# Genie-Kim/PintheMemory

Measured on AMD Instinct MI355X. Metric: train imgs/sec 768x768 bs=8 R50-DeepLabV3+ +mem, higher is better.
Workload: dtype f32

## Files before the change

include/pinmem_hip.h:

```cpp
#ifndef PINMEM_HIP_H
#define PINMEM_HIP_H
#include <stddef.h>
#include <stdint.h>

#ifdef __cplusplus
extern "C" {
#endif

typedef enum pm_status { PM_OK = 0, PM_EINVAL = -1, PM_EWORKSPACE = -2, PM_ELAUNCH = -3, PM_EUNSUPPORTED = -4 } pm_status;

typedef enum pm_dtype { PM_F32 = 0, PM_BF16 = 1 } pm_dtype;
#define PM_TF_ZERO_PAD64 1

typedef struct pm_tensor {
  void* ptr;
  int32_t n, h, w, c;
  int64_t pitch;
  int32_t dtype;
  int32_t flags;
} pm_tensor;

#define PM_ABI_VERSION 400

typedef struct pm_conv_params {
  int32_t struct_size;
  int32_t kh, kw, stride, pad, dil;
  int32_t prec;
  void* wino_v;
  int64_t wino_v_bytes;
  void* wxf;
  int64_t wxf_bytes;
  int32_t wxf_valid;
} pm_conv_params;

typedef struct pm_conv_epilogue {
  int64_t struct_size;
  const float* bias;
  const float* scale;
  const float* shift;
  const float* residual;
  int64_t residual_pitch;
  int32_t relu;
  float* bn_partials;
  int64_t bn_partials_bytes;
} pm_conv_epilogue;

const char* pm_last_error(void);
int pm_version(void);

size_t pm_conv_workspace(const pm_tensor* x, const pm_tensor* y, const pm_conv_params* p, int which );
size_t pm_conv_winograd_v_bytes(const pm_tensor* x, const pm_tensor* y, const pm_conv_params* p);
size_t pm_conv_wxf_bytes(const pm_tensor* x, const pm_tensor* y, const pm_conv_params* p);
size_t pm_conv_wxf_bytes_dgrad(const pm_tensor* dy, const pm_tensor* dx, const pm_conv_params* p);
typedef struct pm_wxf_job {
  const float* w;
  void* wxf;
  int64_t wxf_bytes;
  int32_t cout, kh, kw, cin;
  int32_t dgrad;
  int32_t reserved;
} pm_wxf_job;
int pm_conv_wxf_refresh_bf16(const pm_wxf_job* jobs, int n, void* stream);
int pm_conv_wxf_refresh_f32(const pm_wxf_job* jobs, int n, void* stream);
size_t pm_conv_bn_partials_bytes(const pm_tensor* x, const pm_tensor* y, const pm_conv_params* p);
int pm_conv_fwd(const pm_tensor* x, const float* w_krsc, const pm_tensor* y, const pm_conv_params* p,
                const pm_conv_epilogue* ep, void* ws, size_t ws_bytes, void* stream);
int pm_conv_bwd_data(const pm_tensor* dy, const float* w_krsc, const pm_tensor* dx, const pm_conv_params* p,
                     const pm_tensor* add, void* ws, size_t ws_bytes, void* stream);
int pm_conv_bwd_data_masked(const pm_tensor* dy, const float* w_krsc, const pm_tensor* dx, const pm_conv_params* p,
                            const pm_tensor* add, const uint8_t* add_mask, void* ws, size_t ws_bytes, void* stream);
int pm_conv_bwd_weight(const pm_tensor* x, const pm_tensor* dy, float* dw_krsc, float* dbias, const pm_conv_params* p,
                       void* ws, size_t ws_bytes, void* stream);

typedef struct pm_routing {
  int32_t struct_size;
  int32_t winograd;
  int32_t winograd_fused;
  int32_t conv16;
  int32_t conv16_wide;
  int32_t conv16_persistent;
  int32_t wgrad16;
  int32_t bf16_wgrad;
  int32_t split;
} pm_routing;
int pm_routing_get(pm_routing* out);
int pm_routing_set(const pm_routing* r);


int pm_set_winograd(int mode);
int pm_set_winograd_fused(int on);
int pm_set_conv16(int on);
int pm_set_bf16_wgrad(int on);
int pm_set_wgrad16(int on);
int pm_set_split(int on);

int pm_profile_enable(int on);
int pm_profile_dump(const char* csv_path);
int pm_profile_read(int mode, int bm, int bn, int km, int nst, double* total_ms, double* total_flops, int64_t* launches, int clear);
int pm_profile_read_prec(int mode, int bm, int bn, int km, int nst, int prec, double* total_ms, double* total_flops, int64_t* launches, int clear);
int pm_profile_read_bytes(int mode, int bm, int bn, int km, int nst, int prec, double* total_bytes);

size_t pm_bn_workspace(const pm_tensor* x);
int pm_bn_stats(const pm_tensor* x, float* moments, void* ws, size_t ws_bytes, void* stream);
int pm_bn_stats_finalize(const pm_tensor* x, float eps, float* mean, float* invstd, float* running_mean , float* running_var ,
                         float momentum, void* ws, size_t ws_bytes, void* stream);
int pm_bn_merge(const float* parts, int world, int c, float* moments, void* stream);
int pm_bn_merge_finalize(const float* parts, int world, int c, float eps, float* mean, float* invstd, float* running_mean ,
                         float* running_var , float momentum, void* stream);
int pm_bn_finalize(const float* moments, int c, float eps, float* mean, float* invstd,
                   float* running_mean, float* running_var, float momentum, void* stream);
int pm_bn_apply(const pm_tensor* x, const float* mean, const float* invstd, const float* gamma, const float* beta,
                const pm_tensor* residual , int relu, const pm_tensor* y, void* stream);
int pm_bn_apply_mask(const pm_tensor* x, const float* mean, const float* invstd, const float* gamma, const float* beta,
                     const pm_tensor* residual , int relu, const pm_tensor* y, uint8_t* mask , void* stream);
int pm_bn_bwd_reduce_mask(const pm_tensor* dy, const uint8_t* mask, const pm_tensor* x, const float* mean, const float* invstd,
                          const pm_tensor* gmask , float* sums, void* ws, size_t ws_bytes, void* stream);
int pm_bn_apply_mask_affine(const pm_tensor* x, const float* mean, const float* invstd, const float* gamma, const float* beta,
                            const pm_tensor* r, const float* r_mean, const float* r_invstd, const float* r_gamma, const float* r_beta,
                            int relu, const pm_tensor* y, uint8_t* mask , void* stream);
int pm_bn_bwd_apply_mask(const pm_tensor* dy, const uint8_t* mask, const pm_tensor* x, const float* mean, const float* invstd, const float* gamma,
                         const float* sums, float count, const pm_tensor* dx, void* stream);
int pm_bn_bwd_reduce(const pm_tensor* dy, const pm_tensor* y , const pm_tensor* x, const float* mean, const float* invstd,
                     const float* gamma , const float* beta , int relu, const pm_tensor* gmask ,
                     float* sums, void* ws, size_t ws_bytes, void* stream);
int pm_bn_bwd_apply(const pm_tensor* dy, const pm_tensor* y , const pm_tensor* x, const float* mean, const float* invstd,
                    const float* gamma, const float* beta , const float* sums, float count, int relu, const pm_tensor* dx,
                    const pm_tensor* dres , void* stream);
int pm_bn_partials_finalize(const float* partials, int64_t pixels, int c, float eps, float* mean, float* invstd, float* running_mean ,
                            float* running_var , float momentum, float* moments , void* stream);
int pm_bn_fold(const float* gamma, const float* beta, const float* running_mean, const float* running_var, const float* conv_bias,
               int c, float eps, float* scale, float* shift, void* stream);
int pm_bn_fold_multi(const void* table, const int* cs, const int* offs, int n, int max_c, int total, float eps, float* arena, void* stream);
int pm_relu_bwd(const pm_tensor* dy, const pm_tensor* y, const pm_tensor* dx, void* stream);
int pm_add(const pm_tensor* a, const pm_tensor* b, const pm_tensor* y, void* stream);
int pm_add_n(const pm_tensor* const* xs, int n, const pm_tensor* y, void* stream);
int pm_copy(const pm_tensor* src, const pm_tensor* dst, void* stream);
int pm_scale_shift_act(const pm_tensor* x, const float* scale, const float* shift, const pm_tensor* residual, int relu,
                       const pm_tensor* y, void* stream);

int pm_cast(const pm_tensor* x, const pm_tensor* y, void* stream);

int pm_maxpool3x3s2_fwd(const pm_tensor* x, const pm_tensor* y, uint8_t* argmax, void* stream);
int pm_maxpool3x3s2_bwd(const pm_tensor* dy, const uint8_t* argmax, const pm_tensor* dx, void* stream);
int pm_maxpool3x3s2_bn_relu_fwd(const pm_tensor* x, const float* mean, const float* invstd, const float* gamma, const float* beta, const pm_tensor* y,
                                uint8_t* argmax, void* stream);
int pm_bn_bwd_reduce_pool(const pm_tensor* dy_pooled, const uint8_t* argmax, const pm_tensor* x, const float* mean, const float* invstd, const float* gamma,
                          const float* beta, float* sums, void* ws, size_t ws_bytes, void* stream);
int pm_bn_bwd_apply_pool(const pm_tensor* dy_pooled, const uint8_t* argmax, const pm_tensor* x, const float* mean, const float* invstd, const float* gamma,
                         const float* beta, const float* sums, float count, const pm_tensor* dx, void* stream);
int pm_global_avgpool_fwd(const pm_tensor* x, const pm_tensor* y , void* stream);
int pm_global_avgpool_bwd(const pm_tensor* dy, const pm_tensor* dx, int accumulate, void* stream);

int pm_resize_bilinear_fwd(const pm_tensor* x, const pm_tensor* y, void* stream);
int pm_resize_bilinear_bwd(const pm_tensor* dy, const pm_tensor* dx, int accumulate, void* stream);
size_t pm_resize_bilinear_bwd_workspace(const pm_tensor* dy, const pm_tensor* dx);
// ... 79 lines not shown
```

pinthememory_amd/csrc/bn.hip:

```cpp
#include "pm_common.h"

namespace {

constexpr int CB = 64;
constexpr int RL = 16;

__device__ __forceinline__ float bn_affine(float v, float mu, float is, float ga, float be) { return pm_bn_affine(v, mu, is, ga, be); }

inline int chunk_rows(long P, int C) {
  const long colblocks = std::max<long>(1, (C + CB - 1) / CB);
  const long want = std::max<long>(512, 2048 / colblocks);
  long r = (P + want - 1) / want;
  r = std::max<long>(r, 64);
  return (int)((r + RL - 1) / RL * RL);
}

__global__ __launch_bounds__(256) void bn_stats_partial(const float* __restrict__ x, long pitch, long P, int C, int rows, float* __restrict__ part) {
  __shared__ float sm[RL][CB][2];
  const int g = threadIdx.x & 15, r = threadIdx.x >> 4;
  const int c = blockIdx.y * CB + g * 4;
  const long p0 = (long)blockIdx.x * rows, p1 = min(P, p0 + rows);
  float s1[4] = {0, 0, 0, 0}, s2[4] = {0, 0, 0, 0};
  if (c < C) {
    const float4 k = PM_LD4(x + c);
// ... 411 lines not shown
  if (int e = check_bn(dy, "bn_bwd_reduce")) return e;
  if (int e = check_bn(x, "bn_bwd_reduce")) return e;
  PM_REQUIRE(pm_same_shape(dy, x) && mean && invstd && sums, PM_EINVAL, "bn_bwd_reduce: bad args");
  PM_REQUIRE(relu >= 0 && relu <= 2, PM_EINVAL, "bn_bwd_reduce: relu mode %d (0 none, 1 mask from y, 2 mask rebuilt from x)", relu);
  PM_REQUIRE(relu != 1 || (y && pm_vec4(y) && pm_same_shape(y, x)), PM_EINVAL, "bn_bwd_reduce: relu mode 1 needs the forward output");
  PM_REQUIRE(relu != 2 || (gamma && beta), PM_EINVAL, "bn_bwd_reduce: relu mode 2 needs gamma and beta");
  PM_REQUIRE(!gmask || (relu != 0 && pm_vec4(gmask) && pm_same_shape(gmask, x)), PM_EINVAL, "bn_bwd_reduce: gmask needs a ReLU mode and the shape of x");
  PM_REQUIRE(ws && ws_bytes >= pm_bn_workspace(x), PM_EWORKSPACE, "bn_bwd_reduce: workspace too small");
  const long P = pm_pixels(x);
  const int rows = chunk_rows(P, x->c), nb = pm_cdiv(P, rows);
  hipStream_t st = (hipStream_t)stream;
  dim3 grid(nb, pm_cdiv(x->c, CB));
  const float *pdy = (const float*)dy->ptr, *py = relu == 1 ? (const float*)y->ptr : nullptr, *px = (const float*)x->ptr;
  const long yp = relu == 1 ? y->pitch : 0;
  float* pg = gmask ? (float*)gmask->ptr : nullptr;
  const long gp = gmask ? gmask->pitch : 0;
#define PM_BN_BWD_PARTIAL(R, G)                                                                                                                         \
  hipLaunchKernelGGL((bn_bwd_partial<R, G>), grid, dim3(256), 0, st, pdy, (long)dy->pitch, py, yp, px, (long)x->pitch, mean, invstd, gamma, beta, pg, gp, P, \
                     x->c, rows, (float*)ws)
  if (relu == 0) PM_BN_BWD_PARTIAL(0, false);
  else if (relu == 1 && gmask) PM_BN_BWD_PARTIAL(1, true);
  else if (relu == 1) PM_BN_BWD_PARTIAL(1, false);
  else if (gmask) PM_BN_BWD_PARTIAL(2, true);
  else PM_BN_BWD_PARTIAL(2, false);
#undef PM_BN_BWD_PARTIAL
  hipLaunchKernelGGL(bn_bwd_final, dim3(pm_cdiv(x->c, FC)), dim3(256), 0, st, (const float*)ws, nb, x->c, sums);
  return pm_check_launch("bn_bwd_reduce");
}

extern "C" int pm_bn_bwd_reduce_mask(const pm_tensor* dy, const uint8_t* mask, const pm_tensor* x, const float* mean, const float* invstd,
                                     const pm_tensor* gmask, float* sums, void* ws, size_t ws_bytes, void* stream) {
  PM_REQUIRE(dy && x && mask, PM_EINVAL, "bn_bwd_reduce_mask: null");
  if (pm_is_bf16(x)) return pm16_bn_bwd_reduce(dy, nullptr, mask, x, mean, invstd, nullptr, nullptr, 3, gmask, sums, ws, ws_bytes, (hipStream_t)stream);
  if (int e = check_bn(dy, "bn_bwd_reduce_mask")) return e;
  if (int e = check_bn(x, "bn_bwd_reduce_mask")) return e;
  PM_REQUIRE(pm_same_shape(dy, x) && mean && invstd && sums && mask, PM_EINVAL, "bn_bwd_reduce_mask: bad args");
  PM_REQUIRE(!gmask || (pm_vec4(gmask) && pm_same_shape(gmask, x)), PM_EINVAL, "bn_bwd_reduce_mask: gmask must have the shape of x");
  PM_REQUIRE(ws && ws_bytes >= pm_bn_workspace(x), PM_EWORKSPACE, "bn_bwd_reduce_mask: workspace too small");
  const long P = pm_pixels(x);
  const int rows = chunk_rows(P, x->c), nb = pm_cdiv(P, rows);
  hipStream_t st = (hipStream_t)stream;
  dim3 grid(nb, pm_cdiv(x->c, CB));
  float* pg = gmask ? (float*)gmask->ptr : nullptr;
  const long gp = gmask ? gmask->pitch : 0;
  if (gmask)
    hipLaunchKernelGGL((bn_bwd_partial<3, true>), grid, dim3(256), 0, st, (const float*)dy->ptr, (long)dy->pitch, reinterpret_cast<const float*>(mask), 0l,
                       (const float*)x->ptr, (long)x->pitch, mean, invstd, (const float*)nullptr, (const float*)nullptr, pg, gp, P, x->c, rows, (float*)ws);
  else
    hipLaunchKernelGGL((bn_bwd_partial<3, false>), grid, dim3(256), 0, st, (const float*)dy->ptr, (long)dy->pitch, reinterpret_cast<const float*>(mask), 0l,
                       (const float*)x->ptr, (long)x->pitch, mean, invstd, (const float*)nullptr, (const float*)nullptr, pg, gp, P, x->c, rows, (float*)ws);
  hipLaunchKernelGGL(bn_bwd_final, dim3(pm_cdiv(x->c, FC)), dim3(256), 0, st, (const float*)ws, nb, x->c, sums);
  return pm_check_launch("bn_bwd_reduce_mask");
}

extern "C" int pm_bn_bwd_apply(const pm_tensor* dy, const pm_tensor* y, const pm_tensor* x, const float* mean, const float* invstd, const float* gamma,
                               const float* beta, const float* sums, float count, int relu, const pm_tensor* dx, const pm_tensor* dres, void* stream) {
  PM_REQUIRE(dy && x && dx, PM_EINVAL, "bn_bwd_apply: null");
  if (pm_is_bf16(x)) return pm16_bn_bwd_apply(dy, y, x, mean, invstd, gamma, beta, sums, count, relu, dx, dres, (hipStream_t)stream);
  if (int e = check_bn(dy, "bn_bwd_apply")) return e;
  if (int e = check_bn(x, "bn_bwd_apply")) return e;
  if (int e = check_bn(dx, "bn_bwd_apply")) return e;
  PM_REQUIRE(pm_same_shape(dy, x) && pm_same_shape(dx, x) && mean && invstd && gamma && sums, PM_EINVAL, "bn_bwd_apply: bad args");
  PM_REQUIRE(relu >= 0 && relu <= 2, PM_EINVAL, "bn_bwd_apply: relu mode %d (0 none, 1 mask from y, 2 mask rebuilt from x)", relu);
  PM_REQUIRE(relu != 1 || (y && pm_vec4(y) && pm_same_shape(y, x)), PM_EINVAL, "bn_bwd_apply: relu mode 1 needs the forward output");
  PM_REQUIRE(relu != 2 || beta, PM_EINVAL, "bn_bwd_apply: relu mode 2 needs beta");
  PM_REQUIRE(!dres || (pm_vec4(dres) && pm_same_shape(dres, x)), PM_EINVAL, "bn_bwd_apply: dres shape mismatch");
  const float *pd = (const float*)dy->ptr, *po = relu == 1 ? (const float*)y->ptr : nullptr, *px = (const float*)x->ptr;
  float *pdx = (float*)dx->ptr, *pdr = dres ? (float*)dres->ptr : nullptr;
  const long a = dy->pitch, b = relu == 1 ? y->pitch : 0, c = x->pitch, d = dx->pitch, e2 = dres ? dres->pitch : 0;
  const bool from_x = relu == 2;
  const int C = x->c;
  const bool dev_count = !(count > 0.f);
  const float host_inv_n = dev_count ? 0.f : 1.f / count;
  return pm_ew_launch(true, pm_pixels(x), C, (hipStream_t)stream, "bn_bwd_apply", [=] __device__(long p, int ch) {
    const float inv_n = dev_count ? 1.f / sums[2 * C] : host_inv_n;
    float4 g = PM_LD4(pd + p * a + ch);
    if (po) {
      const float4 o = PM_LD4(po + p * b + ch);
      g.x = o.x > 0.f ? g.x : 0.f, g.y = o.y > 0.f ? g.y : 0.f, g.z = o.z > 0.f ? g.z : 0.f, g.w = o.w > 0.f ? g.w : 0.f;
    }
    const float4 v = PM_LD4(px + p * c + ch), mu = PM_LD4(mean + ch), is = PM_LD4(invstd + ch), ga = PM_LD4(gamma + ch);
    if (from_x) {
      const float4 be = PM_LD4(beta + ch);
      g.x = bn_affine(v.x, mu.x, is.x, ga.x, be.x) > 0.f ? g.x : 0.f, g.y = bn_affine(v.y, mu.y, is.y, ga.y, be.y) > 0.f ? g.y : 0.f;
      g.z = bn_affine(v.z, mu.z, is.z, ga.z, be.z) > 0.f ? g.z : 0.f, g.w = bn_affine(v.w, mu.w, is.w, ga.w, be.w) > 0.f ? g.w : 0.f;
    }
    if (pdr) PM_ST4(pdr + p * e2 + ch, g);
    const float4 s1 = PM_LD4(sums + ch), s2 = PM_LD4(sums + C + ch);
    float4 r;
    r.x = (g.x - s1.x * inv_n - (v.x - mu.x) * is.x * (s2.x * inv_n)) * (is.x * ga.x);
    r.y = (g.y - s1.y * inv_n - (v.y - mu.y) * is.y * (s2.y * inv_n)) * (is.y * ga.y);
    r.z = (g.z - s1.z * inv_n - (v.z - mu.z) * is.z * (s2.z * inv_n)) * (is.z * ga.z);
    r.w = (g.w - s1.w * inv_n - (v.w - mu.w) * is.w * (s2.w * inv_n)) * (is.w * ga.w);
    PM_ST4(pdx + p * d + ch, r);
  });
}

extern "C" int pm_bn_bwd_apply_mask(const pm_tensor* dy, const uint8_t* mask, const pm_tensor* x, const float* mean, const float* invstd, const float* gamma,
                                    const float* sums, float count, const pm_tensor* dx, void* stream) {
  PM_REQUIRE(dy && x && dx && mask, PM_EINVAL, "bn_bwd_apply_mask: null");
  if (int e = check_bn(dy, "bn_bwd_apply_mask")) return e;
  if (int e = check_bn(x, "bn_bwd_apply_mask")) return e;
  if (int e = check_bn(dx, "bn_bwd_apply_mask")) return e;
  PM_REQUIRE(pm_same_shape(dy, x) && pm_same_shape(dx, x) && mean && invstd && gamma && sums, PM_EINVAL, "bn_bwd_apply_mask: bad args");
  const float *pd = (const float*)dy->ptr, *px = (const float*)x->ptr;
  float* pdx = (float*)dx->ptr;
  const long a = dy->pitch, c = x->pitch, d = dx->pitch;
  const int C = x->c, cq = C >> 2;
  const bool dev_count = !(count > 0.f);
  const float host_inv_n = dev_count ? 0.f : 1.f / count;
  return pm_ew_launch(true, pm_pixels(x), C, (hipStream_t)stream, "bn_bwd_apply_mask", [=] __device__(long p, int ch) {
    const float inv_n = dev_count ? 1.f / sums[2 * C] : host_inv_n;
    float4 g = PM_LD4(pd + p * a + ch);
    const unsigned mb = mask[p * cq + (ch >> 2)];
    g.x = (mb & 1u) ? g.x : 0.f, g.y = (mb & 2u) ? g.y : 0.f, g.z = (mb & 4u) ? g.z : 0.f, g.w = (mb & 8u) ? g.w : 0.f;
    const float4 v = PM_LD4(px + p * c + ch), mu = PM_LD4(mean + ch), is = PM_LD4(invstd + ch), ga = PM_LD4(gamma + ch);
    const float4 s1 = PM_LD4(sums + ch), s2 = PM_LD4(sums + C + ch);
    float4 r;
    r.x = (g.x - s1.x * inv_n - (v.x - mu.x) * is.x * (s2.x * inv_n)) * (is.x * ga.x);
    r.y = (g.y - s1.y * inv_n - (v.y - mu.y) * is.y * (s2.y * inv_n)) * (is.y * ga.y);
    r.z = (g.z - s1.z * inv_n - (v.z - mu.z) * is.z * (s2.z * inv_n)) * (is.z * ga.z);
    r.w = (g.w - s1.w * inv_n - (v.w - mu.w) * is.w * (s2.w * inv_n)) * (is.w * ga.w);
    PM_ST4(pdx + p * d + ch, r);
  });
}

namespace {
int check_pool_bn(const pm_tensor* dyp, const uint8_t* argmax, const pm_tensor* x, const char* who) {
  PM_REQUIRE(dyp && argmax && x, PM_EINVAL, "%s: null", who);
  if (int e = check_bn(dyp, who)) return e;
  if (int e = check_bn(x, who)) return e;
  PM_REQUIRE(dyp->n == x->n && dyp->c == x->c && dyp->h == (x->h + 2 - 3) / 2 + 1 && dyp->w == (x->w + 2 - 3) / 2 + 1, PM_EINVAL,
             "%s: dy is the gradient of the 3x3 / s2 / p1 max pool of a tensor shaped like x", who);
  return PM_OK;
}
}

extern "C" int pm_bn_bwd_reduce_pool(const pm_tensor* dyp, const uint8_t* argmax, const pm_tensor* x, const float* mean, const float* invstd, const float* gamma,
                                     const float* beta, float* sums, void* ws, size_t ws_bytes, void* stream) {
  if (int e = check_pool_bn(dyp, argmax, x, "bn_bwd_reduce_pool")) return e;
  PM_REQUIRE(mean && invstd && gamma && beta && sums, PM_EINVAL, "bn_bwd_reduce_pool: bad args");
  PM_REQUIRE(ws && ws_bytes >= pm_bn_workspace(x), PM_EWORKSPACE, "bn_bwd_reduce_pool: workspace too small");
  const long P = pm_pixels(x);
  const int rows = chunk_rows(P, x->c), nb = pm_cdiv(P, rows);
  hipStream_t st = (hipStream_t)stream;
  hipLaunchKernelGGL(bn_bwd_partial_pool, dim3(nb, pm_cdiv(x->c, CB)), dim3(256), 0, st, (const float*)dyp->ptr, (long)dyp->pitch, dyp->h, dyp->w, argmax, x->h, x->w,
                     (const float*)x->ptr, (long)x->pitch, mean, invstd, gamma, beta, P, x->c, rows, (float*)ws);
  hipLaunchKernelGGL(bn_bwd_final, dim3(pm_cdiv(x->c, FC)), dim3(256), 0, st, (const float*)ws, nb, x->c, sums);
  return pm_check_launch("bn_bwd_reduce_pool");
}

extern "C" int pm_bn_bwd_apply_pool(const pm_tensor* dyp, const uint8_t* argmax, const pm_tensor* x, const float* mean, const float* invstd, const float* gamma,
                                    const float* beta, const float* sums, float count, const pm_tensor* dx, void* stream) {
  if (int e = check_pool_bn(dyp, argmax, x, "bn_bwd_apply_pool")) return e;
  PM_REQUIRE(dx, PM_EINVAL, "bn_bwd_apply_pool: null");
  if (int e = check_bn(dx, "bn_bwd_apply_pool")) return e;
  PM_REQUIRE(pm_same_shape(dx, x) && mean && invstd && gamma && beta && sums, PM_EINVAL, "bn_bwd_apply_pool: bad args");
  const float *pd = (const float*)dyp->ptr, *px = (const float*)x->ptr;
  float* pdx = (float*)dx->ptr;
  const long a = dyp->pitch, c = x->pitch, d = dx->pitch;
  const int C = x->c, H = x->h, W = x->w, Ho = dyp->h, Wo = dyp->w;
  const bool dev_count = !(count > 0.f);
  const float host_inv_n = dev_count ? 0.f : 1.f / count;
  return pm_ew_launch(true, pm_pixels(x), C, (hipStream_t)stream, "bn_bwd_apply_pool", [=] __device__(long p, int ch) {
    const float inv_n = dev_count ? 1.f / sums[2 * C] : host_inv_n;
    float4 g = pm_maxpool_gather4(pd, a, Ho, Wo, argmax, H, W, C, p, ch);
    const float4 v = PM_LD4(px + p * c + ch), mu = PM_LD4(mean + ch), is = PM_LD4(invstd + ch), ga = PM_LD4(gamma + ch), be = PM_LD4(beta + ch);
    g.x = bn_affine(v.x, mu.x, is.x, ga.x, be.x) > 0.f ? g.x : 0.f, g.y = bn_affine(v.y, mu.y, is.y, ga.y, be.y) > 0.f ? g.y : 0.f;
    g.z = bn_affine(v.z, mu.z, is.z, ga.z, be.z) > 0.f ? g.z : 0.f, g.w = bn_affine(v.w, mu.w, is.w, ga.w, be.w) > 0.f ? g.w : 0.f;
    const float4 s1 = PM_LD4(sums + ch), s2 = PM_LD4(sums + C + ch);
    float4 r;
    r.x = (g.x - s1.x * inv_n - (v.x - mu.x) * is.x * (s2.x * inv_n)) * (is.x * ga.x);
    r.y = (g.y - s1.y * inv_n - (v.y - mu.y) * is.y * (s2.y * inv_n)) * (is.y * ga.y);
    r.z = (g.z - s1.z * inv_n - (v.z - mu.z) * is.z * (s2.z * inv_n)) * (is.z * ga.z);
    r.w = (g.w - s1.w * inv_n - (v.w - mu.w) * is.w * (s2.w * inv_n)) * (is.w * ga.w);
    PM_ST4(pdx + p * d + ch, r);
  });
}
```

pinthememory_amd/csrc/conv_igemm.hip:

```cpp
#include <stdlib.h>
#include <algorithm>
#include <type_traits>
#include <vector>

#include "pm_common.h"

#include "conv_igemm_kernel.h"

namespace {

template <int ZL, bool O16 = false>
__global__ __launch_bounds__(256) void splitk_reduce_vec_kernel(const float* __restrict__ ws, int ksplit, long slab, int M, int Nn,
                                                                float* __restrict__ C, long c_pitch, const float* bias,
                                                                const float* scale, const float* shift, const float* residual,
                                                                long res_pitch, int relu, const unsigned char* res_mask) {
  constexpr int GP = 256 / ZL;
  __shared__ float4 red[ZL > 1 ? ZL : 1][GP];
  const int gl = threadIdx.x % GP, zl = threadIdx.x / GP;
  const long groups = (long)M * Nn / 4;
  for (long g0 = (long)blockIdx.x * GP; g0 < groups; g0 += (long)gridDim.x * GP) {
    const long grp = g0 + gl;
    float4 v = make_float4(0.f, 0.f, 0.f, 0.f);
    if (grp < groups)
#pragma unroll 8
// ... 394 lines not shown
  prof.done();
  return pm_check_launch("conv_igemm");
}

int check_common(const pm_tensor* x, const pm_tensor* y, const pm_conv_params* p) {
  PM_REQUIRE(x && y && p && x->ptr && y->ptr, PM_EINVAL, "conv: null tensor");
  PM_REQUIRE(p->struct_size == (int32_t)sizeof(pm_conv_params), PM_EINVAL, "conv: pm_conv_params.struct_size %d != %zu -- caller built against another pinmem_hip.h (library ABI %d)",
             p->struct_size, sizeof(pm_conv_params), PM_ABI_VERSION);
  PM_REQUIRE(p->kh >= 1 && p->kw >= 1 && p->dil >= 1 && p->pad >= 0, PM_EINVAL, "conv: bad geometry");
  PM_REQUIRE(p->stride == 1 || p->stride == 2, PM_EUNSUPPORTED, "conv: stride %d unsupported (1 or 2)", p->stride);
  const int ho = (x->h + 2 * p->pad - p->dil * (p->kh - 1) - 1) / p->stride + 1;
  const int wo = (x->w + 2 * p->pad - p->dil * (p->kw - 1) - 1) / p->stride + 1;
  PM_REQUIRE(ho == y->h && wo == y->w && x->n == y->n, PM_EINVAL, "conv: output %dx%d does not match geometry (%dx%d)", y->h, y->w, ho, wo);
  PM_REQUIRE((x->dtype == PM_F32 || x->dtype == PM_BF16) && (y->dtype == PM_F32 || y->dtype == PM_BF16), PM_EUNSUPPORTED, "conv: dtype %d / %d", x->dtype, y->dtype);
  for (const pm_tensor* t : {x, y}) {
    if (pm_is_bf16(t)) PM_REQUIRE(pm_vec8(t), PM_EINVAL, "conv: bf16 tensors must be 16B aligned with pitch %% 8 == 0 and channels %% 8 == 0");
    else PM_REQUIRE(pm_vec_ok(t), PM_EINVAL, "conv: tensors must be 16B aligned with pitch %% 4 == 0");
  }
  PM_REQUIRE(x->c % 4 == 0, PM_EUNSUPPORTED, "conv: Cin %% 4 != 0 unsupported (pad the input channels)");
  PM_REQUIRE((y->c % 4 == 0) || (p->kh * p->kw == 1), PM_EUNSUPPORTED, "conv: Cout %% 4 != 0 only for 1x1");
  PM_REQUIRE(x->pitch >= x->c && y->pitch >= y->c, PM_EINVAL, "conv: pitch < channels");
  PM_REQUIRE(pm_pixels(x) * x->pitch < (1ll << 29) && pm_pixels(y) * y->pitch < (1ll << 29) && (int64_t)y->c * x->c * p->kh * p->kw < (1ll << 29),
             PM_EUNSUPPORTED, "conv: tensor too large for 32-bit byte offsets (2 GiB per tensor)");
  return PM_OK;
}

void fill_geom(ConvK& k, const pm_tensor* x, const pm_tensor* y, const pm_conv_params* p) {
  k.N = x->n, k.H = x->h, k.W = x->w, k.Cin = x->c, k.x_pitch = x->pitch;
  k.Ho = y->h, k.Wo = y->w, k.Cout = y->c, k.y_pitch = y->pitch;
  k.kh = p->kh, k.kw = p->kw, k.stride = p->stride, k.pad = p->pad, k.dil = p->dil;
  k.sshift = p->stride == 2 ? 1 : 0;
  k.prec = p->prec != 0 ? 1 : 0;
  k.T_eff = p->kh * p->kw, k.tk_w = p->kw, k.ky0 = k.kx0 = 0, k.ksy = k.ksx = 1;
  k.sub = k.sub_cy = k.sub_cx = 0, k.Hc = x->h, k.Wc = x->w;
  k.bias = k.scale = k.shift = k.residual = nullptr;
  k.res_pitch = 0, k.res_mask = nullptr, k.relu = 0, k.stats = nullptr, k.io16 = 0;
  k.stage_ep = 1;
  k.spl_prio = 1;
  k.n_group = 8;
  k.batch_xcd = 0;
  k.a_bs = k.b_bs = k.c_bs = 0;
}

struct WinoPlan {
  bool use;
  pm_wino_geom g;
  int Kp, P;
  size_t v_bytes, m_bytes, u_bytes;
  Plan pl;
};
inline bool wino_wgrad_pays(int cin, int cout) { return (long)cin * cout >= 256 * 256; }
WinoPlan wino_plan(const pm_tensor* xin, int cout, const pm_conv_params* p, bool wgrad = false) {
  WinoPlan wp{};
  if (wgrad && !wino_wgrad_pays(xin->c, cout)) return wp;
  if (pm_route.winograd == 0 || p->kh != 3 || p->kw != 3 || p->stride != 1 || p->pad != p->dil || p->prec != 0) return wp;
  const int cin = xin->c;
  if (cin < 128 || cout < 128 || (cout & 3) || (cin & 3)) return wp;
  int m = 0;
  double best_ratio = 0.6;
  for (int cand = pm_route.winograd; cand >= 2; cand -= 2) {
    const pm_wino_geom g = pm_wino_make_geom(xin->n, xin->h, xin->w, p->dil, cand);
    const double cover = (double)(cand * g.TY * p->dil) * (double)(cand * g.TX * p->dil) / ((double)xin->h * xin->w);
    const double ratio = cover * (cand + 2) * (cand + 2) / (9.0 * cand * cand);
    if (ratio <= best_ratio) best_ratio = ratio, m = cand, wp.g = g;
  }
  if (!m) return wp;
  wp.P = (m + 2) * (m + 2);
  wp.Kp = (cin + BK - 1) / BK * BK;
  if (wp.g.tiles * (long)std::max(wp.Kp, cout) * 4 >= (1ll << 31)) return wp;
  wp.v_bytes = pm_align_up((size_t)wp.P * wp.g.tiles * wp.Kp * sizeof(float), 256);
  wp.m_bytes = pm_align_up((size_t)wp.P * wp.g.tiles * cout * sizeof(float), 256);
  wp.u_bytes = pm_align_up((size_t)wp.P * cout * wp.Kp * sizeof(float), 256);
  wp.pl.bm = 128, wp.pl.bn = 128;
  if (pm_cdiv(cout, 128) * 128 > cout * 1.12 && pm_cdiv(cout, 64) * 64 < pm_cdiv(cout, 128) * 128) wp.pl.bn = 64;
  if (wp.g.tiles <= 4608 && !pm_route.split) wp.pl.bm = 64;
  wp.pl.tiles_m = pm_cdiv(wp.g.tiles, wp.pl.bm), wp.pl.tiles_n = pm_cdiv(cout, wp.pl.bn);
  wp.pl.ksplit = 1, wp.pl.kper = wp.Kp, wp.pl.ws_bytes = 0;
  wp.use = true;
  return wp;
}
inline size_t wino_ws(const WinoPlan& wp) { return wp.v_bytes + wp.m_bytes + wp.u_bytes; }

int wino_conv(const pm_tensor* xin, const float* w, int w_cout, int w_cin, bool dgrad, const pm_tensor* yout, const WinoPlan& wp,
              const pm_conv_epilogue& ep, void* ws, hipStream_t st, float* v_keep = nullptr, float* u_ext = nullptr, bool u_valid = false) {
  float* V = v_keep ? v_keep : (float*)ws;
  float* Mo = (float*)((char*)ws + wp.v_bytes);
  float* U = u_ext ? u_ext : (float*)((char*)ws + wp.v_bytes + wp.m_bytes);
  const int cout = yout->c;
  if (int e = pm_wino_input_xf((const float*)xin->ptr, xin->pitch, xin->c, wp.Kp, wp.g, V, st)) return e;
  if (!(u_ext && u_valid))
    if (int e = pm_wino_filter_xf(w, w_cout, w_cin, wp.Kp, dgrad, wp.g.m, U, st)) return e;
  const pm_tensor xv = {V, 1, 1, (int32_t)wp.g.tiles, wp.Kp, wp.Kp};
  const pm_tensor yv = {Mo, 1, 1, (int32_t)wp.g.tiles, cout, cout};
  const pm_conv_params p1 = {(int32_t)sizeof(pm_conv_params), 1, 1, 1, 0, 1, 0};
  ConvK k;
  fill_geom(k, &xv, &yv, &p1);
  k.A = V, k.B = U, k.C = Mo;
  k.M = (int)wp.g.tiles, k.Nn = cout, k.K = wp.Kp;
  k.a_bytes = (unsigned)(wp.g.tiles * wp.Kp * 4), k.b_bytes = (unsigned)((long)cout * wp.Kp * 4), k.kmode = K_FAST;
  k.c_pitch = cout, k.c_split = 0;
  k.a_bs = wp.g.tiles * wp.Kp, k.b_bs = (long)cout * wp.Kp, k.c_bs = wp.g.tiles * cout;
  if (pm_route.winograd_fused && wp.g.m == 4 && wp.Kp % 16 == 0) {
    ProfScope prof(st, 3, 32, 32, 0, 0, 1, wp.g.tiles, cout, wp.Kp, wp.P, 1, 2.0 * wp.P * (double)wp.g.tiles * cout * xin->c);
    const int e = pm_wino_fused_f4(V, U, cout, wp.Kp, wp.g, (float*)yout->ptr, yout->pitch, ep.bias, ep.scale, ep.shift, ep.residual, ep.residual_pitch, ep.relu, st);
    prof.done();
    return e;
  }
  if (int e = launch<MODE_FWD>(k, wp.pl, st, wp.P, 2.0 * wp.P * (double)wp.g.tiles * cout * xin->c)) return e;
  return pm_wino_output_xf(Mo, cout, wp.g, (float*)yout->ptr, yout->pitch, ep.bias, ep.scale, ep.shift, ep.residual, ep.residual_pitch, ep.relu, st);
}

struct WinoWgradPlan {
  Plan pl;
  size_t slab_bytes;
};
WinoWgradPlan wino_wgrad_plan(const WinoPlan& wp, int cout) {
  WinoWgradPlan q{};
  q.pl.bm = 128, q.pl.bn = 128;
  if (pm_cdiv(wp.Kp, 128) * 128 > wp.Kp * 1.12 && pm_cdiv(wp.Kp, 64) * 64 < pm_cdiv(wp.Kp, 128) * 128) q.pl.bn = 64;
  q.pl.tiles_m = pm_cdiv(cout, 128), q.pl.tiles_n = pm_cdiv(wp.Kp, q.pl.bn);
  const long ksteps = (wp.g.tiles + BK - 1) / BK;
  const long per_split = (long)q.pl.tiles_m * q.pl.tiles_n * wp.P;
  long ks = std::max<long>(1, std::min<long>((768 + per_split / 2) / per_split, ksteps / 8));
  const long steps_per = (ksteps + ks - 1) / ks;
  ks = (ksteps + steps_per - 1) / steps_per;
  q.pl.ksplit = (int)ks, q.pl.kper = (int)(steps_per * BK), q.pl.ws_bytes = 0;
  q.slab_bytes = pm_align_up((size_t)ks * wp.P * cout * wp.Kp * sizeof(float), 256);
  return q;
}
inline size_t wino_wgrad_ws(const WinoPlan& wp, const WinoWgradPlan& q) { return wp.v_bytes + wp.m_bytes + q.slab_bytes; }

int wino_wgrad(const pm_tensor* x, const pm_tensor* dy, float* dw, const WinoPlan& wp, const WinoWgradPlan& q, void* ws, hipStream_t st,
               float* v_kept = nullptr) {
  float* V = v_kept ? v_kept : (float*)ws;
  float* Z = (float*)((char*)ws + wp.v_bytes);
  float* slab = (float*)((char*)ws + wp.v_bytes + wp.m_bytes);
  const int cout = dy->c;
  if (!v_kept)
    if (int e = pm_wino_input_xf((const float*)x->ptr, x->pitch, x->c, wp.Kp, wp.g, V, st)) return e;
  if (int e = pm_wino_dy_xf((const float*)dy->ptr, dy->pitch, cout, wp.g, Z, st)) return e;
  const pm_tensor xv = {V, 1, 1, (int32_t)wp.g.tiles, wp.Kp, wp.Kp};
  const pm_tensor zv = {Z, 1, 1, (int32_t)wp.g.tiles, cout, cout};
  const pm_conv_params p1 = {(int32_t)sizeof(pm_conv_params), 1, 1, 1, 0, 1, 0};
  ConvK k;
  fill_geom(k, &xv, &zv, &p1);
  k.A = Z, k.B = V, k.C = slab;
  k.M = cout, k.Nn = wp.Kp, k.K = (int)wp.g.tiles;
  k.a_bytes = (unsigned)(wp.g.tiles * cout * 4), k.b_bytes = (unsigned)(wp.g.tiles * wp.Kp * 4), k.kmode = K_MID;
  k.c_pitch = wp.Kp, k.c_split = (long)wp.P * cout * wp.Kp;
  k.a_bs = wp.g.tiles * cout, k.b_bs = wp.g.tiles * wp.Kp, k.c_bs = (long)cout * wp.Kp;
  if (int e = launch<MODE_WGRAD>(k, q.pl, st, wp.P, 2.0 * wp.P * (double)wp.g.tiles * cout * x->c)) return e;
  return pm_wino_dw_xf(slab, q.pl.ksplit, cout, x->c, wp.Kp, wp.g.m, dw, st);
}

struct Bf16Plan {
  bool use;
  bool c16;
  pm_conv16 k16;
  bool inplace;
  int Cp;
  long M, Nn, Kf;
  size_t xb_bytes, wb_bytes;
  Plan pl;
};
Bf16Plan bf16_plan(const pm_tensor* xin, const pm_tensor* yout, const pm_conv_params* p) {
  Bf16Plan b{};
  if ((p->prec != 2 && !pm_is_bf16(xin) && !pm_is_bf16(yout)) || xin->c < 32) return b;
  b.Cp = (xin->c + 63) / 64 * 64;
  const long T = (long)p->kh * p->kw;
  b.M = pm_pixels(yout), b.Nn = yout->c, b.Kf = T * b.Cp / 2;
  b.inplace = pm_is_bf16(xin) && (xin->c % 64 == 0 || ((xin->flags & PM_TF_ZERO_PAD64) && xin->pitch >= b.Cp));
  const size_t xb = b.inplace ? (size_t)pm_pixels(xin) * xin->pitch * 2 : (size_t)pm_pixels(xin) * b.Cp * 2, wb = (size_t)yout->c * T * b.Cp * 2;
  if (xb >= (1ull << 31) || wb >= (1ull << 31)) return b;
  b.xb_bytes = b.inplace ? 0 : pm_align_up(xb, 256), b.wb_bytes = pm_align_up(wb, 256);
  b.pl = make_plan(MODE_FWD, b.M, b.Nn, b.Kf, true);
  if (b.pl.bn < 64) return b;
  b.use = true;
  constexpr long C16_MIN_M = 256;
  b.c16 = false;
  if (pm_route.conv16 && b.M >= C16_MIN_M && p->stride >= 1) {
    pm_conv16& k = b.k16;
    k = pm_conv16{};
    k.N = xin->n, k.H = xin->h, k.W = xin->w, k.Ho = yout->h, k.Wo = yout->w;
    k.a_pitch = b.inplace ? xin->pitch : b.Cp, k.Cp = b.Cp;
    k.kh = p->kh, k.kw = p->kw, k.stride = p->stride, k.pad = p->pad, k.dil = p->dil;
    k.M = (int)b.M, k.Nn = (int)b.Nn, k.K = (int)(T * b.Cp), k.ksteps = k.K / 64;
    k.c_pitch = yout->pitch, k.c_f32 = pm_is_bf16(yout) ? 0 : 1;
    pm_conv16_plan(&k);
    b.c16 = pm_route.conv16 == 2 || k.wide || k.bm == 64 || k.ksteps_per == 1 || (b.pl.bm == 64 && k.ksteps >= 16);
  }
  return b;
}
inline size_t bf16_ws(const Bf16Plan& b) {
  return b.xb_bytes + b.wb_bytes + std::max(pm_align_up(b.pl.ws_bytes, 256), b.c16 ? pm_conv16_slab_bytes(&b.k16) : (size_t)0);
}

int conv_bf16(const pm_tensor* xin, const float* w, int w_cout, int w_cin, bool rotate, const pm_tensor* yout, const pm_conv_params* pe, const Bf16Plan& b,
              const pm_conv_epilogue& e0, void* ws, hipStream_t st, char* wb_ext = nullptr, bool wb_valid = false) {
  char* xb = b.inplace ? (char*)xin->ptr : (char*)ws;
  char* wb = wb_ext ? wb_ext : (char*)ws + b.xb_bytes;
  float* slab = (float*)((char*)ws + b.xb_bytes + b.wb_bytes);
  const int T = pe->kh * pe->kw;
  if (!b.inplace) {
    if (pm_is_bf16(xin)) {
      if (int e = pm16_pad_rows((const pm_bf16*)xin->ptr, xin->pitch, xin->c, b.Cp, pm_pixels(xin), (pm_bf16*)xb, st)) return e;
    } else if (int e = pm_bf16_cast_rows((const float*)xin->ptr, xin->pitch, xin->c, b.Cp, pm_pixels(xin), xb, st)) return e;
  }
  if (!(wb_ext && wb_valid))
    if (int e = pm_bf16_cast_weights(w, w_cout, T, w_cin, b.Cp, rotate, wb, st)) return e;
  const long xpitch16 = b.inplace ? xin->pitch : b.Cp;
  if (b.c16) {
    const bool o16 = pm_is_bf16(yout);
    const bool ok = (!e0.bn_partials || o16) &&
                    (o16 ? ((yout->c | yout->pitch | (e0.residual ? e0.residual_pitch : 0)) & 7) == 0 && pm_aligned16(yout->ptr) && pm_aligned16(e0.residual)
                         : !(e0.scale || e0.residual || e0.relu));
    if (ok) {
      pm_conv16 k = b.k16;
      k.A = (const pm_bf16*)xb, k.B = (const pm_bf16*)wb;
      const double fl = 2.0 * (double)b.M * (double)b.Nn * (double)T * (double)xin->c * (g_prof_on ? pm_conv16_executed_fraction(&k) : 1.0);
      ProfScope prof(st, k.wide ? 5 : 4, k.bm, k.bn, pm_conv16w_persistent(&k), 5, k.wide ? 3 : (k.ksteps_per == 1 ? 1 : 2), k.M, k.Nn, k.K / 2, 1, k.ksplit, fl);
      int e;
      if (k.ksplit > 1) {
        k.C = slab;
// ... 165 lines not shown
  const long T = (long)p->kh * p->kw;
  if (which == MODE_FWD) M = pm_pixels(y), Nn = y->c, K = T * x->c;
  else if (which == MODE_DGRAD) M = pm_pixels(x), Nn = x->c, K = T * y->c;
  else M = y->c, Nn = T * x->c, K = pm_pixels(y);
}

struct S2ParityPlan {
  S2Class c[4];
  Plan pl[4];
  bool valid[4];
  size_t tmp_bytes, slab_bytes;
};
S2ParityPlan s2_parity_plan(const pm_tensor* dy, const pm_tensor* dx, const pm_conv_params* p) {
  S2ParityPlan s{};
  for (int cls = 0; cls < 4; ++cls) {
    const S2Class& c = s.c[cls] = s2_class(cls, dx, p);
    s.tmp_bytes = std::max(s.tmp_bytes, (size_t)c.M * dx->c * sizeof(float));
    s.valid[cls] = c.M > 0 && c.nky * c.nkx > 0;
    if (!s.valid[cls]) continue;
    s.pl[cls] = make_plan(MODE_DGRAD, c.M, dx->c, (long)c.nky * c.nkx * dy->c, p->prec != 0);
    s.slab_bytes = std::max(s.slab_bytes, s.pl[cls].ws_bytes);
  }
  s.tmp_bytes = pm_align_up(s.tmp_bytes, 256);
  return s;
}

struct W16Plan {
  bool use;
  pm_wgrad16 k;
};
W16Plan wgrad16_plan(const pm_tensor* x, const pm_tensor* dy, const pm_conv_params* p, long M, long Nn, long K, int max_ksplit) {
  W16Plan q{};
  pm_wgrad16& w16 = q.k;
  w16.X = (const pm_bf16*)x->ptr, w16.DY = (const pm_bf16*)dy->ptr;
  w16.N = x->n, w16.H = x->h, w16.W = x->w, w16.Ho = dy->h, w16.Wo = dy->w;
  w16.x_pitch = x->pitch, w16.dy_pitch = dy->pitch, w16.Cin = x->c, w16.Cout = dy->c;
  w16.kh = p->kh, w16.kw = p->kw, w16.stride = p->stride, w16.pad = p->pad, w16.dil = p->dil;
  w16.M = (int)M, w16.Nn = (int)Nn, w16.P = (int)K, w16.kper = 64, w16.c_split = M * Nn;
  q.use = K < (1l << 30) && pm_wgrad16_plan(&w16);
  if (!q.use) return q;
  const long tiles = (long)w16.tiles_m * w16.tiles_n, steps = (K + 63) / 64;
  int best_ks = 1;
  double best = 1e30;
  for (int ks = 1; ks <= max_ksplit; ++ks) {
    const long per = (steps + ks - 1) / ks, kse = (steps + per - 1) / per;
    const long rounds = (tiles * kse + 255) / 256;
    const double cost = (double)rounds * (per + 6) + (kse > 1 ? (double)kse * M * Nn * 8.0 / 4e12 / 1.0e-6 : 0.0);
    if (cost < best) best = cost, best_ks = (int)kse;
  }
  const long per = (steps + best_ks - 1) / best_ks;
  w16.kper = (int)per * 64, w16.ksplit = (int)((steps + per - 1) / per);
  return q;
}

enum RouteKind {
  R_DIRECT,
  R_WINO,
  R_BF16,
  R_S2_NATIVE,
  R_S2_PARITY,
  R_WINO_WGRAD,
  R_BF16_WGRAD,
  R_DIRECT_WGRAD,
};
struct ConvRoute {
  RouteKind kind;
  Plan pl;
  WinoPlan wino;
  WinoWgradPlan wino_w;
  Bf16Plan b16;
  pm_conv_params pe;
  S2Native s2n;
  S2ParityPlan s2p;
  Bf16WgradPlan b16w;
  W16Plan w16;
  bool native16;
  size_t ws_bytes;
  size_t class_off, slab_off;
  size_t bias_off;
  size_t x32_off, dy32_off;
  size_t v_keep_bytes;
  size_t wxf_bytes;
  size_t bn_bytes;
};

ConvRoute route_conv(int which, const pm_tensor* x, const pm_tensor* y, const pm_conv_params* p) {
  ConvRoute r{};
  long M, Nn, K;
  gemm_dims(which, x, y, p, M, Nn, K);
  if (which == MODE_FWD) {
    if ((r.wino = wino_plan(x, y->c, p)).use) {
      r.kind = R_WINO, r.ws_bytes = wino_ws(r.wino), r.wxf_bytes = r.wino.u_bytes;
      r.v_keep_bytes = wino_wgrad_pays(x->c, y->c) ? r.wino.v_bytes : 0;
    } else if (p->prec == 2 && (r.b16 = bf16_plan(x, y, p)).use) {
      r.kind = R_BF16, r.pe = *p, r.ws_bytes = bf16_ws(r.b16), r.wxf_bytes = r.b16.wb_bytes;
    } else {
      r.kind = R_DIRECT, r.pl = make_plan(MODE_FWD, M, Nn, K, p->prec != 0), r.ws_bytes = pm_align_up(r.pl.ws_bytes, 256);
    }
    bool bn;
    if (pm_is_bf16(y)) bn = pm_vec8(y) && r.kind == R_BF16 && (r.b16.c16 ? (r.b16.k16.ksplit == 1 && !r.b16.k16.wide) : r.b16.pl.ksplit == 1);
    else if (pm_is_bf16(x) || (y->c & 3) || (y->pitch & 3) || !pm_aligned16(y->ptr)) bn = false;
    else bn = r.kind == R_BF16 ? r.b16.pl.ksplit == 1 : (r.kind == R_DIRECT && p->prec == 0 && r.pl.ksplit == 1 && r.pl.bn >= 64);
    r.bn_bytes = bn ? pm_align_up((size_t)pm_cdiv(pm_pixels(y), 32) * y->c * 2 * sizeof(float), 256) : 0;
  } else if (which == MODE_DGRAD) {
    if (p->stride == 2) {
      if ((r.s2n = s2_native_plan(y, x, p)).ok) {
        r.kind = R_S2_NATIVE, r.ws_bytes = r.s2n.total;
      } else {
        r.kind = R_S2_PARITY, r.s2p = s2_parity_plan(y, x, p);
        r.class_off = 0, r.slab_off = 4 * r.s2p.tmp_bytes;
        r.dy32_off = pm_align_up(r.slab_off + r.s2p.slab_bytes + 256, 256);
        r.ws_bytes = r.dy32_off + upcast_bytes(y);
      }
    } else if (dgrad_bf16_ok(p) && (r.pe = dgrad_as_fwd(p), r.b16 = bf16_plan(y, x, &r.pe)).use) {
      r.kind = R_BF16, r.ws_bytes = bf16_ws(r.b16), r.wxf_bytes = r.b16.wb_bytes;
    } else if ((r.wino = wino_plan(y, x->c, p)).use) {
      r.kind = R_WINO, r.ws_bytes = wino_ws(r.wino);
    } else {
      r.kind = R_DIRECT, r.pl = make_plan(MODE_DGRAD, M, Nn, K, p->prec != 0), r.ws_bytes = pm_align_up(r.pl.ws_bytes, 256);
    }
  } else {
    const bool tier = pm_is_bf16(x) || pm_is_bf16(y);
    r.native16 = pm_is_bf16(x) && pm_is_bf16(y) && y->c >= 32;
    size_t own;
    if (!tier && (r.b16w = bf16_wgrad_plan(x, y, p)).use) {
      r.kind = R_BF16_WGRAD, own = bf16_wgrad_ws(r.b16w);
    } else if (!tier && (r.wino = wino_plan(x, y->c, p, true)).use) {
      r.kind = R_WINO_WGRAD, r.wino_w = wino_wgrad_plan(r.wino, y->c), own = wino_wgrad_ws(r.wino, r.wino_w);
    } else {
      r.kind = R_DIRECT_WGRAD, r.pl = make_plan(MODE_WGRAD, M, Nn, K, p->prec != 0), own = r.pl.ws_bytes;
      if (r.native16) {
        r.pl.kper = (r.pl.kper + 63) / 64 * 64;
        r.pl.ksplit = (int)((K + r.pl.kper - 1) / r.pl.kper);
        r.w16 = wgrad16_plan(x, y, p, M, Nn, K, r.pl.ksplit);
      }
    }
    r.bias_off = pm_align_up(own, 256);
    r.ws_bytes = r.bias_off + pm_align_up((size_t)pm_cdiv(pm_pixels(y), colsum_rows(pm_pixels(y), y->c)) * y->c * sizeof(float), 256) + upcast_bytes(x) + upcast_bytes(y);
    r.x32_off = r.dy32_off = r.ws_bytes;
    if (!r.native16) r.x32_off -= upcast_bytes(x);
    r.dy32_off = r.x32_off - upcast_bytes(y);
  }
  return r;
}

int dgrad_s2_parity(const pm_tensor* dy0, const float* w, const pm_tensor* dx, const pm_conv_params* p, const pm_tensor* add, const ConvRoute& r, void* ws, hipStream_t st) {
  pm_tensor dy32;
  if (int e = upcast(dy0, (char*)ws + r.dy32_off, &dy32, st)) return e;
  const pm_tensor* dy = &dy32;
  float* tmp = (float*)((char*)ws + r.class_off);
  float* slab = (float*)((char*)ws + r.slab_off);
  for (int cls = 0; cls < 4; ++cls) {
    if (!r.s2p.valid[cls]) continue;
    const S2Class& c = r.s2p.c[cls];
    const Plan& pl = r.s2p.pl[cls];
    ConvK k;
    fill_geom(k, dx, dy, p);
    k.A = (const float*)dy->ptr, k.B = w;
    k.M = (int)c.M, k.Nn = dx->c, k.K = c.nky * c.nkx * dy->c;
    k.a_bytes = (unsigned)(pm_pixels(dy) * dy->pitch * 4), k.b_bytes = (unsigned)((long)dy->c * p->kh * p->kw * dx->c * 4);
    k.kmode = dy->c >= BK ? K_MID : K_SMALL;
    k.T_eff = c.nky * c.nkx, k.tk_w = c.nkx, k.ky0 = c.ky0, k.kx0 = c.kx0, k.ksy = c.ksy, k.ksx = c.ksx;
    k.sub = 1, k.sub_cy = c.cy, k.sub_cx = c.cx, k.Hc = c.Hc, k.Wc = c.Wc;
    float* out = (float*)((char*)tmp + cls * r.s2p.tmp_bytes);
    if (pl.ksplit > 1) {
      k.C = slab, k.c_pitch = dx->c, k.c_split = c.M * dx->c;
      if (int e = launch<MODE_DGRAD>(k, pl, st)) return e;
      if (int e = splitk_reduce(slab, pl.ksplit, c.M, dx->c, out, (long)dx->c, nullptr, nullptr, nullptr, nullptr, 0l, 0, st)) return e;
    } else {
      k.C = out, k.c_pitch = dx->c, k.c_split = 0;
      if (int e = launch<MODE_DGRAD>(k, pl, st)) return e;
    }
  }
  return s2_interleave(tmp, (long)(r.s2p.tmp_bytes / sizeof(float)), r.s2p.valid, dx, add, st, "dgrad_s2_interleave");
}

template <int MODE>
int conv_direct(const pm_tensor* x, const pm_tensor* y, const float* w, const pm_conv_params* p, const Plan& pl, const pm_conv_epilogue& e, void* ws, hipStream_t st,
                const unsigned char* res_mask = nullptr) {
  const pm_tensor *xin = MODE == MODE_FWD ? x : y, *out = MODE == MODE_FWD ? y : x;
  long M, Nn, K;
  gemm_dims(MODE, x, y, p, M, Nn, K);
  ConvK k;
  fill_geom(k, x, y, p);
  k.io16 = pm_is_bf16(out) ? 1 : 0;
  k.A = (const float*)xin->ptr, k.B = w;
  k.M = (int)M, k.Nn = (int)Nn, k.K = (int)K;
  k.a_bytes = (unsigned)(pm_pixels(xin) * xin->pitch * 4), k.b_bytes = (unsigned)((long)y->c * p->kh * p->kw * x->c * 4);
  k.kmode = (xin->c % BK == 0 && (MODE == MODE_FWD || p->stride == 1)) ? 0 : (xin->c >= BK ? 1 : 2);
  if (pl.ksplit > 1) {
    k.C = (float*)ws, k.c_pitch = Nn, k.c_split = M * Nn;
    if (int err = launch<MODE>(k, pl, st)) return err;
    return splitk_reduce((const float*)ws, pl.ksplit, M, Nn, (float*)out->ptr, (long)out->pitch, e.bias, e.scale, e.shift, e.residual, (long)e.residual_pitch, e.relu, st, k.io16 != 0,
                         res_mask);
  }
  k.C = (float*)out->ptr, k.c_pitch = out->pitch, k.c_split = 0;
  k.bias = e.bias, k.scale = e.scale, k.shift = e.shift, k.residual = e.residual, k.res_pitch = e.residual_pitch, k.res_mask = res_mask, k.relu = e.relu;
  k.stats = e.bn_partials;
  return launch<MODE>(k, pl, st);
}

int conv_wgrad_direct(const pm_tensor* x, const pm_tensor* dy, float* dw, const pm_conv_params* p, const ConvRoute& r, void* ws, hipStream_t st) {
  long M, Nn, K;
  gemm_dims(MODE_WGRAD, x, dy, p, M, Nn, K);
  if (r.w16.use) {
    pm_wgrad16 w16 = r.w16.k;
    w16.C = w16.ksplit > 1 ? (float*)ws : dw;
    ProfScope prof(st, MODE_WGRAD, w16.bm, w16.bn, 2, 4, 3, M, Nn, K, 1, w16.ksplit, 2.0 * (double)M * (double)Nn * (double)K);
    const int e = pm_wgrad16_launch(&w16, st);
    prof.done();
    if (e || w16.ksplit == 1) return e;
// ... 146 lines not shown
  if (!x || !y || !p0) return 0;
  const pm_conv_params tp = tier_params(p0, x, y);
  return route_conv(MODE_FWD, x, y, &tp).wxf_bytes;
}
extern "C" size_t pm_conv_wxf_bytes_dgrad(const pm_tensor* dy, const pm_tensor* dx, const pm_conv_params* p0) {
  if (!dy || !dx || !p0) return 0;
  const pm_conv_params tp = tier_params(p0, dy, dx);
  return route_conv(MODE_DGRAD, dx, dy, &tp).wxf_bytes;
}
extern "C" size_t pm_conv_bn_partials_bytes(const pm_tensor* x, const pm_tensor* y, const pm_conv_params* p0) {
  if (!x || !y || !p0 || check_common(x, y, p0) != PM_OK) return 0;
  const pm_conv_params tp = tier_params(p0, x, y);
  return route_conv(MODE_FWD, x, y, &tp).bn_bytes;
}

extern "C" int pm_conv_wxf_refresh_f32(const pm_wxf_job* jobs, int n, void* stream) {
  PM_REQUIRE(n >= 0 && (jobs || n == 0), PM_EINVAL, "conv_wxf_refresh_f32: bad job table");
  std::vector<const float*> w(n);
  std::vector<float*> U(n);
  std::vector<int> cout(n), cin(n), kp(n), m(n);
  for (int i = 0; i < n; ++i) {
    const pm_wxf_job& q = jobs[i];
    PM_REQUIRE(q.w && q.wxf && q.cout > 0 && q.cin > 0 && q.kh == 3 && q.kw == 3 && q.dgrad == 0, PM_EINVAL,
               "conv_wxf_refresh_f32: job %d: forward transforms of 3x3 filters only", i);
    PM_REQUIRE(pm_aligned16(q.wxf), PM_EINVAL, "conv_wxf_refresh_f32: job %d: buffer must be 16-byte aligned", i);
    const int Kp = (q.cin + BK - 1) / BK * BK;
    const size_t u4 = pm_align_up((size_t)36 * q.cout * Kp * sizeof(float), 256), u2 = pm_align_up((size_t)16 * q.cout * Kp * sizeof(float), 256);
    PM_REQUIRE((size_t)q.wxf_bytes == u4 || (size_t)q.wxf_bytes == u2, PM_EINVAL, "conv_wxf_refresh_f32: job %d: %ld bytes is neither the F(4x4) nor the F(2x2) transform of %d x %d",
               i, (long)q.wxf_bytes, q.cout, q.cin);
    w[i] = q.w, U[i] = (float*)q.wxf, cout[i] = q.cout, cin[i] = q.cin, kp[i] = Kp, m[i] = (size_t)q.wxf_bytes == u4 ? 4 : 2;
  }
  return pm_wino_filter_xf_multi(w.data(), U.data(), cout.data(), cin.data(), kp.data(), m.data(), n, (hipStream_t)stream);
}

extern "C" int pm_conv_fwd(const pm_tensor* x, const float* w, const pm_tensor* y, const pm_conv_params* p0,
                           const pm_conv_epilogue* ep, void* ws, size_t ws_bytes, void* stream) {
  if (int e = check_common(x, y, p0)) return e;
  const pm_conv_params tp = tier_params(p0, x, y);
  const pm_conv_params* p = &tp;
  PM_REQUIRE(!ep || ep->struct_size == (int64_t)sizeof(pm_conv_epilogue), PM_EINVAL,
             "conv_fwd: pm_conv_epilogue.struct_size %ld != %zu -- caller built against another pinmem_hip.h (library ABI %d)", ep ? (long)ep->struct_size : 0l,
             sizeof(pm_conv_epilogue), PM_ABI_VERSION);
  PM_REQUIRE(w && pm_aligned16(w), PM_EINVAL, "conv_fwd: weight null or unaligned");
  pm_conv_epilogue e0 = {(int64_t)sizeof(pm_conv_epilogue), nullptr, nullptr, nullptr, nullptr, 0, 0};
  if (ep) e0 = *ep;
  PM_REQUIRE((e0.scale == nullptr) == (e0.shift == nullptr), PM_EINVAL, "conv_fwd: scale and shift go together");
  const ConvRoute r = route_conv(MODE_FWD, x, y, p);
  if (e0.bn_partials) {
    PM_REQUIRE(!e0.relu && !e0.residual, PM_EINVAL, "conv_fwd: bn_partials are the statistics of the convolution output (no residual / ReLU)");
    PM_REQUIRE(r.bn_bytes != 0 && (size_t)e0.bn_partials_bytes >= r.bn_bytes, PM_EINVAL, "conv_fwd: this call cannot emit bn_partials (ask pm_conv_bn_partials_bytes): %zu needed", r.bn_bytes);
  }
  PM_REQUIRE(ws_bytes >= r.ws_bytes && (ws || r.ws_bytes == 0), PM_EWORKSPACE, "conv_fwd: workspace %zu < %zu", ws_bytes, r.ws_bytes);
  hipStream_t st = (hipStream_t)stream;
  switch (r.kind) {
    case R_WINO: {
      float* keep = (p->wino_v && (size_t)p->wino_v_bytes >= r.wino.v_bytes) ? (float*)p->wino_v : nullptr;
      float* uext = (p->wxf && (size_t)p->wxf_bytes >= r.wino.u_bytes) ? (float*)p->wxf : nullptr;
      return wino_conv(x, w, y->c, x->c, false, y, r.wino, e0, ws, st, keep, uext, p->wxf_valid != 0);
    }
    case R_BF16: {
      char* wext = (p->wxf && (size_t)p->wxf_bytes >= r.b16.wb_bytes) ? (char*)p->wxf : nullptr;
      return conv_bf16(x, w, y->c, x->c, false, y, &r.pe, r.b16, e0, ws, st, wext, p->wxf_valid != 0);
    }
    default:
      PM_REQUIRE(pm_is_f32(x), PM_EUNSUPPORTED, "conv_fwd: a bf16 input needs at least 32 channels (got %d)", x->c);
      return conv_direct<MODE_FWD>(x, y, w, p, r.pl, e0, ws, st);
  }
}

extern "C" int pm_conv_bwd_data(const pm_tensor* dy, const float* w, const pm_tensor* dx, const pm_conv_params* p0, const pm_tensor* add,
                                void* ws, size_t ws_bytes, void* stream) {
  return pm_conv_bwd_data_masked(dy, w, dx, p0, add, nullptr, ws, ws_bytes, stream);
}

extern "C" int pm_conv_bwd_data_masked(const pm_tensor* dy, const float* w, const pm_tensor* dx, const pm_conv_params* p0, const pm_tensor* add,
                                       const uint8_t* add_mask, void* ws, size_t ws_bytes, void* stream) {
  if (int e = check_common(dx, dy, p0)) return e;
  const pm_conv_params tp = tier_params(p0, dy, dx);
  const pm_conv_params* p = &tp;
  PM_REQUIRE(!add || (add->ptr && pm_same_shape(add, dx) && add->dtype == dx->dtype), PM_EINVAL, "conv_bwd_data: `add` must match dx (shape and dtype)");
  PM_REQUIRE(!add || !pm_is_bf16(add) || pm_vec8(add), PM_EINVAL, "conv_bwd_data: bf16 `add` must be 16B aligned with pitch %% 8 == 0");
  PM_REQUIRE(w && pm_aligned16(w), PM_EINVAL, "conv_bwd_data: weight null or unaligned");
  const ConvRoute r = route_conv(MODE_DGRAD, dx, dy, p);
  PM_REQUIRE(ws_bytes >= r.ws_bytes && (ws || r.ws_bytes == 0), PM_EWORKSPACE, "conv_bwd_data: workspace %zu < %zu", ws_bytes, r.ws_bytes);
  if (add_mask) {
    PM_REQUIRE(add && pm_is_f32(add) && pm_is_f32(dy) && pm_vec4(add) && pm_vec4(dx), PM_EINVAL, "conv_bwd_data: a masked `add` is an fp32 tensor with 16-byte rows and c %% 4 == 0");
    PM_REQUIRE(r.kind == R_DIRECT, PM_EUNSUPPORTED,
               "conv_bwd_data: a masked `add` is served by the fp32 implicit-GEMM route only (this call routes to %s)",
               r.kind == R_WINO ? "Winograd" : (r.kind == R_BF16 ? "the bf16 kernels" : "the stride-2 class kernels"));
  }
  hipStream_t st = (hipStream_t)stream;
  const pm_conv_epilogue e1 = {(int64_t)sizeof(pm_conv_epilogue), nullptr, nullptr, nullptr, add ? (const float*)add->ptr : nullptr, add ? add->pitch : 0, 0};
  switch (r.kind) {
    case R_S2_NATIVE: return dgrad_s2_bf16(dy, w, dx, p, add, r.s2n, ws, st);
    case R_S2_PARITY: return dgrad_s2_parity(dy, w, dx, p, add, r, ws, st);
    case R_BF16: {
      char* wext = (p->wxf && (size_t)p->wxf_bytes >= r.b16.wb_bytes) ? (char*)p->wxf : nullptr;
      return conv_bf16(dy, w, dy->c, dx->c, true, dx, &r.pe, r.b16, e1, ws, st, wext, p->wxf_valid != 0);
    }
    case R_WINO: return wino_conv(dy, w, dy->c, dx->c, true, dx, r.wino, e1, ws, st);
    default:
      PM_REQUIRE(pm_is_f32(dy), PM_EUNSUPPORTED, "conv_bwd_data: a bf16 dy needs at least 32 channels and a stride-1 geometry the forward form covers");
      return conv_direct<MODE_DGRAD>(dx, dy, w, p, r.pl, e1, ws, st, add_mask);
  }
}

extern "C" int pm_conv_bwd_weight(const pm_tensor* x0, const pm_tensor* dy0, float* dw, float* dbias, const pm_conv_params* p0, void* ws,
                                  size_t ws_bytes, void* stream) {
  if (int e = check_common(x0, dy0, p0)) return e;
  const pm_conv_params tp = tier_params(p0, x0, dy0);
  const pm_conv_params* p = &tp;
  PM_REQUIRE(dw && pm_aligned16(dw), PM_EINVAL, "conv_bwd_weight: dw null or unaligned");
  const ConvRoute r = route_conv(MODE_WGRAD, x0, dy0, p);
  PM_REQUIRE(ws && ws_bytes >= r.ws_bytes, PM_EWORKSPACE, "conv_bwd_weight: workspace %zu < %zu", ws_bytes, r.ws_bytes);
  hipStream_t st = (hipStream_t)stream;
  const pm_tensor *x = x0, *dy = dy0;
  pm_tensor x32, dy32;
  if (!r.native16 && pm_is_bf16(x0)) {
    if (int e = upcast(x0, (char*)ws + r.x32_off, &x32, st)) return e;
    x = &x32;
  }
  if (pm_is_bf16(dy0) && (!r.native16 || dbias)) {
    if (int e = upcast(dy0, (char*)ws + r.dy32_off, &dy32, st)) return e;
    if (!r.native16) dy = &dy32;
  }
  int e;
  switch (r.kind) {
    case R_BF16_WGRAD: e = conv_wgrad_bf16(x, dy, dw, p, r.b16w, ws, st); break;
    case R_WINO_WGRAD: e = wino_wgrad(x, dy, dw, r.wino, r.wino_w, ws, st, (p->wino_v && (size_t)p->wino_v_bytes >= r.wino.v_bytes) ? (float*)p->wino_v : nullptr); break;
    default: e = conv_wgrad_direct(x, dy, dw, p, r, ws, st);
  }
  if (e || !dbias) return e;
  const pm_tensor* dyb = pm_is_bf16(dy0) ? &dy32 : dy0;
  const long P = pm_pixels(dyb);
  const int rpb = colsum_rows(P, dyb->c), nb = pm_cdiv(P, rpb);
  float* part = (float*)((char*)ws + r.bias_off);
  if (dyb->pitch == ((dyb->c + 3) & ~3) && dyb->pitch <= 64 && pm_aligned16(dyb->ptr))
    hipLaunchKernelGGL(colsum_partial_narrow_kernel, dim3(nb), dim3(256), 0, st, (const float*)dyb->ptr, (int)(dyb->pitch / 4), P, dyb->c, rpb, part);
  else
    hipLaunchKernelGGL(colsum_partial_kernel, dim3(nb, pm_cdiv(dyb->c, 64)), dim3(256), 0, st, (const float*)dyb->ptr, (long)dyb->pitch, P, dyb->c, rpb, part);
  hipLaunchKernelGGL(colsum_final_kernel, dim3(pm_cdiv(dyb->c, 64)), dim3(1024), 0, st, (const float*)part, nb, dyb->c, dbias);
  return pm_check_launch("conv_bias_grad");
}
```

pinthememory_amd/csrc/pm_common.h:

```cpp
#pragma once
#include <hip/hip_runtime.h>
#include <algorithm>
#include <atomic>
#include <stdarg.h>
#include <stdint.h>
#include <stdio.h>

#include "../../include/pinmem_hip.h"

void pm_set_error(const char* fmt, ...);

#define PM_REQUIRE(cond, code, ...)      \
  do {                                   \
    if (!(cond)) {                       \
      pm_set_error(__VA_ARGS__);         \
      return (code);                     \
    }                                    \
  } while (0)

static inline int pm_check_launch(const char* what) {
  hipError_t e = hipGetLastError();
  if (e != hipSuccess) {
    pm_set_error("%s: launch failed: %s", what, hipGetErrorString(e));
    return PM_ELAUNCH;
  }
  return PM_OK;
}

static inline bool pm_aligned16(const void* p) { return (reinterpret_cast<uintptr_t>(p) & 15u) == 0; }
static inline int64_t pm_pixels(const pm_tensor* t) { return (int64_t)t->n * t->h * t->w; }
static inline int pm_cdiv(int64_t a, int64_t b) { return (int)((a + b - 1) / b); }
static inline size_t pm_align_up(size_t v, size_t a) { return (v + a - 1) / a * a; }

static inline bool pm_vec_ok(const pm_tensor* t) { return pm_aligned16(t->ptr) && (t->pitch % 4) == 0; }
static inline bool pm_is_f32(const pm_tensor* t) { return t->dtype == PM_F32; }
static inline bool pm_is_bf16(const pm_tensor* t) { return t->dtype == PM_BF16; }
#define PM_REQUIRE_F32(t, who) PM_REQUIRE(!(t) || pm_is_f32(t), PM_EUNSUPPORTED, "%s: fp32 tensors only (got dtype %d)", who, (t)->dtype)
static inline bool pm_vec8(const pm_tensor* t) { return pm_is_bf16(t) && pm_aligned16(t->ptr) && (t->pitch % 8) == 0 && (t->c % 8) == 0; }

struct pm_wino_geom {
  int N, H, W, d, m, TY, TX;
  long tiles;
};
pm_wino_geom pm_wino_make_geom(int n, int h, int w, int d, int m);
int pm_wino_input_xf(const float* x, long pitch, int C, int Kp, const pm_wino_geom& g, float* V, hipStream_t st);
int pm_wino_filter_xf(const float* w, int Cout, int Cin, int Kp, bool dgrad, int m, float* U, hipStream_t st);
int pm_wino_filter_xf_multi(const float* const* w, float* const* U, const int* cout, const int* cin, const int* kp, const int* m, int n, hipStream_t st);
int pm_wino_output_xf(const float* M, int Cout, const pm_wino_geom& g, float* y, long ypitch, const float* bias, const float* scale, const float* shift,
                      const float* residual, long res_pitch, int relu, hipStream_t st);
int pm_wino_fused_f4(const float* V, const float* U, int Cout, int Kp, const pm_wino_geom& g, float* y, long ypitch, const float* bias, const float* scale,
                     const float* shift, const float* residual, long res_pitch, int relu, hipStream_t st);
int pm_wino_dy_xf(const float* dy, long pitch, int Cout, const pm_wino_geom& g, float* Z, hipStream_t st);
int pm_wino_dw_xf(const float* slab, int ks, int Cout, int Cin, int Kp, int m, float* dw, hipStream_t st);

int pm_bf16_cast_rows(const float* x, long pitch, int C, int Cp, long P, void* out, hipStream_t st);
int pm_bf16_cast_weights(const float* w, int Cout, int T, int Cin, int Cp, bool rotate, void* out, hipStream_t st);
struct PmS2Classes {
  int ky0[4], nky[4], kx0[4], nkx[4];
  void* out[4];
};
int pm_bf16_cast_weights_s2(const float* w, int Cout, int kh, int kw, int Cin, int Cp, const PmS2Classes* cl, hipStream_t st);
int pm_bf16_transpose_taps(const float* x, long pitch, int C, int N, int H, int W, int Ho, int Wo, int kh, int kw, int stride, int pad, int dil, void* out,
                           hipStream_t st);

typedef unsigned short pm_bf16;
int pm16_bn_stats(const pm_tensor* x, float* moments, float eps, float* mean, float* invstd, float* running_mean, float* running_var, float momentum, void* ws,
                  size_t ws_bytes, hipStream_t st);
size_t pm16_bn_workspace(const pm_tensor* x);
int pm16_bn_apply_mask(const pm_tensor* x, const float* mean, const float* invstd, const float* gamma, const float* beta, const pm_tensor* res, int relu,
                       const pm_tensor* y, uint8_t* mask, hipStream_t st);
int pm16_bn_bwd_reduce(const pm_tensor* dy, const pm_tensor* y, const uint8_t* mask, const pm_tensor* x, const float* mean, const float* invstd, const float* gamma,
                       const float* beta, int relu, const pm_tensor* gmask, float* sums, void* ws, size_t ws_bytes, hipStream_t st);
int pm16_bn_bwd_apply(const pm_tensor* dy, const pm_tensor* y, const pm_tensor* x, const float* mean, const float* invstd, const float* gamma, const float* beta,
                      const float* sums, float count, int relu, const pm_tensor* dx, const pm_tensor* dres, hipStream_t st);
int pm16_add_n(const pm_tensor* const* xs, int n, const pm_tensor* y, hipStream_t st);
int pm16_copy(const pm_tensor* x, const pm_tensor* y, hipStream_t st);
int pm16_maxpool_fwd(const pm_tensor* x, const pm_tensor* y, uint8_t* argmax, hipStream_t st);
int pm16_maxpool_bwd(const pm_tensor* dy, const uint8_t* argmax, const pm_tensor* dx, hipStream_t st);
int pm16_gap_fwd(const pm_tensor* x, const pm_tensor* y, hipStream_t st);
int pm16_gap_bwd(const pm_tensor* dy, const pm_tensor* dx, int accumulate, hipStream_t st);
int pm16_resize_fwd(const pm_tensor* x, const pm_tensor* y, hipStream_t st);
int pm16_resize_bwd(const pm_tensor* dy, const pm_tensor* dx, int accumulate, hipStream_t st);
size_t pm16_resize_bwd_workspace(const pm_tensor* dy, const pm_tensor* dx);
int pm16_resize_bwd_separable(const pm_tensor* dy, const pm_tensor* dx, int accumulate, void* ws, size_t ws_bytes, hipStream_t st);
int pm16_to_f32(const pm_bf16* x, long pitch, int C, long P, float* out, long out_pitch, hipStream_t st);
int pm16_pad_rows(const pm_bf16* x, long pitch, int C, int Cp, long P, pm_bf16* out, hipStream_t st);

struct pm_conv16 {
  const pm_bf16* A;
  const pm_bf16* B;
  void* C;
  int N, H, W, Ho, Wo;
  long a_pitch;
  int Cp;
  int kh, kw, stride, pad, dil;
  int M, Nn, K, ksteps;
  long c_pitch;
  int c_f32;
  const float *bias, *scale, *shift;
  const void* residual;
  long res_pitch;
  int relu;
  float* stats;
  int bm, bn, tiles_m, tiles_n, ksplit, ksteps_per;
  long c_split;
  int wide;
};
void pm_conv16_plan(pm_conv16* k);
int pm_conv16w_launch(const pm_conv16* k, hipStream_t st);
int pm_conv16w_persistent(const pm_conv16* k);
size_t pm_conv16_slab_bytes(const pm_conv16* k);
double pm_conv16_executed_fraction(const pm_conv16* k);
int pm_conv16_launch(const pm_conv16* k, hipStream_t st);

struct pm_wgrad16 {
  const pm_bf16* X;
  const pm_bf16* DY;
  float* C;
  int N, H, W, Ho, Wo;
  long x_pitch, dy_pitch;
  int Cin, Cout, kh, kw, stride, pad, dil;
  int M, Nn, P;
  int kper, ksplit;
  long c_split;
  int bm, bn, tiles_m, tiles_n;
};
bool pm_wgrad16_plan(pm_wgrad16* k);
int pm_wgrad16_launch(const pm_wgrad16* k, hipStream_t st);

struct pm_gemm_pw {
  const float* A;
  const float* B;
  float* C;
  const float *bias, *scale, *shift, *residual;
  const unsigned char* res_mask;
  long a_pitch, c_pitch, res_pitch;
// ... 23 lines not shown
    if (!keep || !done[dev].load(std::memory_order_acquire)) {
      if (hipFuncSetAttribute(kernel, hipFuncAttributeMaxDynamicSharedMemorySize, lds_bytes) != hipSuccess) (void)hipGetLastError();
      else if (keep) done[dev].store(true, std::memory_order_release);
    }
    return pm_device_cus(dev);
  }
};

extern pm_routing pm_route;


__device__ __forceinline__ void pm_ld8(const pm_bf16* p, float* v) {
  const uint4 q = *reinterpret_cast<const uint4*>(p);
  v[0] = __uint_as_float(q.x << 16), v[1] = __uint_as_float(q.x & 0xffff0000u), v[2] = __uint_as_float(q.y << 16), v[3] = __uint_as_float(q.y & 0xffff0000u);
  v[4] = __uint_as_float(q.z << 16), v[5] = __uint_as_float(q.z & 0xffff0000u), v[6] = __uint_as_float(q.w << 16), v[7] = __uint_as_float(q.w & 0xffff0000u);
}
__device__ __forceinline__ unsigned pm_pack_bf16(float a, float b) {
  typedef __bf16 bf16x2_t __attribute__((ext_vector_type(2)));
  bf16x2_t o;
  o[0] = (__bf16)a, o[1] = (__bf16)b;
  return __builtin_bit_cast(unsigned, o);
}
__device__ __forceinline__ void pm_st8(pm_bf16* p, const float* v) {
  uint4 q;
  q.x = pm_pack_bf16(v[0], v[1]), q.y = pm_pack_bf16(v[2], v[3]), q.z = pm_pack_bf16(v[4], v[5]), q.w = pm_pack_bf16(v[6], v[7]);
  *reinterpret_cast<uint4*>(p) = q;
}
__device__ __forceinline__ float pm_bf16_to_f32(pm_bf16 h) { return __uint_as_float((unsigned)h << 16); }
__device__ __forceinline__ pm_bf16 pm_f32_to_bf16(float f) { return __builtin_bit_cast(unsigned short, (__bf16)f); }

template <int LDC, int LPR, int RPI>
__device__ __forceinline__ void pm_slab_stats16(const float* Ws, int rr0, int cc, long slab_row0, long M, long Nn, int col, bool cok, const float* bi, const float* sc,
                                                const float* sh, float* stats) {
  const float cnt = (float)max(0l, min(32l, M - slab_row0));
  float s1[8], mu[8], m2[8];
#pragma unroll
  for (int e = 0; e < 8; ++e) s1[e] = 0.f, m2[e] = 0.f;
  auto slab_row = [&](int r0, float* v) {
    const float4 v0 = *reinterpret_cast<const float4*>(Ws + (r0 + rr0) * LDC + cc), v1 = *reinterpret_cast<const float4*>(Ws + (r0 + rr0) * LDC + cc + 4);
    const float t[8] = {v0.x, v0.y, v0.z, v0.w, v1.x, v1.y, v1.z, v1.w};
#pragma unroll
    for (int e = 0; e < 8; ++e) v[e] = pm_bf16_to_f32(pm_f32_to_bf16((t[e] + bi[e]) * sc[e] + sh[e]));
    return slab_row0 + r0 + rr0 < M;
  };
#pragma unroll
  for (int r0 = 0; r0 < 32; r0 += RPI) {
    float v[8];
    const bool rok = slab_row(r0, v);
#pragma unroll
    for (int e = 0; e < 8; ++e) s1[e] += rok ? v[e] : 0.f;
  }
#pragma unroll
  for (int o = LPR; o < 64; o <<= 1)
#pragma unroll
    for (int e = 0; e < 8; ++e) s1[e] += __shfl_xor(s1[e], o, 64);
#pragma unroll
  for (int e = 0; e < 8; ++e) mu[e] = cnt > 0.f ? s1[e] / cnt : 0.f;
#pragma unroll
  for (int r0 = 0; r0 < 32; r0 += RPI) {
    float v[8];
    const bool rok = slab_row(r0, v);
#pragma unroll
    for (int e = 0; e < 8; ++e) {
      const float d = v[e] - mu[e];
      m2[e] += rok ? d * d : 0.f;
    }
  }
#pragma unroll
  for (int o = LPR; o < 64; o <<= 1)
#pragma unroll
    for (int e = 0; e < 8; ++e) m2[e] += __shfl_xor(m2[e], o, 64);
  if (rr0 == 0 && cok && cnt > 0.f) {
    float* dst = stats + ((slab_row0 >> 5) * Nn + col) * 2;
#pragma unroll
    for (int e = 0; e < 8; e += 2) *reinterpret_cast<float4*>(dst + 2 * e) = make_float4(mu[e], m2[e], mu[e + 1], m2[e + 1]);
  }
}

__device__ __forceinline__ float pm_bn_affine(float v, float mu, float is, float ga, float be) {
  const float s = is * ga;
  return fmaf(v, s, fmaf(-mu, s, be));
}

__device__ __forceinline__ float4 pm_maxpool_gather4(const float* __restrict__ dy, long dp, int Ho, int Wo, const uint8_t* __restrict__ arg, int H, int W, int C, long ip,
                                                     int ch) {
  const int ix = (int)(ip % W), iy = (int)((ip / W) % H), n = (int)(ip / ((long)W * H));
  float4 g = make_float4(0.f, 0.f, 0.f, 0.f);
  const int oy_hi = min((iy + 1) >> 1, Ho - 1), ox_hi = min((ix + 1) >> 1, Wo - 1);
  for (int oy = iy >> 1; oy <= oy_hi; ++oy) {
    const int ky = iy + 1 - 2 * oy;
    if (ky < 0 || ky > 2) continue;
    for (int ox = ix >> 1; ox <= ox_hi; ++ox) {
      const int kx = ix + 1 - 2 * ox;
      if (kx < 0 || kx > 2) continue;
      const long op = (long)(n * Ho + oy) * Wo + ox;
      const unsigned a = *reinterpret_cast<const unsigned*>(arg + op * C + ch), want = (unsigned)(ky * 3 + kx);
      const float4 d = *reinterpret_cast<const float4*>(dy + op * dp + ch);
      g.x += (a & 255u) == want ? d.x : 0.f;
      g.y += ((a >> 8) & 255u) == want ? d.y : 0.f;
      g.z += ((a >> 16) & 255u) == want ? d.z : 0.f;
      g.w += (a >> 24) == want ? d.w : 0.f;
    }
  }
  return g;
}

__device__ __forceinline__ float pm_wave_sum(float v) {
#pragma unroll
  for (int o = 32; o > 0; o >>= 1) v += __shfl_xor(v, o, 64);
  return v;
}
__device__ __forceinline__ float pm_wave_max(float v) {
#pragma unroll
  for (int o = 32; o > 0; o >>= 1) v = fmaxf(v, __shfl_xor(v, o, 64));
  return v;
}

struct pm_lerp {
  int i0, i1;
  float w0, w1;
};
__host__ __device__ __forceinline__ float pm_ac_scale(int in, int out) {
  return out > 1 ? (float)(in - 1) / (float)(out - 1) : 0.f;
}
__device__ __forceinline__ pm_lerp pm_ac_lerp(float scale, int dst, int in) {
  float src = scale * (float)dst;
  int i0 = (int)src;
  if (i0 > in - 1) i0 = in - 1;
  int i1 = i0 + (i0 < in - 1 ? 1 : 0);
  float l1 = src - (float)i0;
  if (l1 < 0.f) l1 = 0.f;
  if (l1 > 1.f) l1 = 1.f;
  pm_lerp r;
  r.i0 = i0;
  r.i1 = i1;
  r.w1 = l1;
  r.w0 = 1.f - l1;
  return r;
}

template <bool VEC, typename F>
__global__ __launch_bounds__(256) void pm_ew_kernel(long pixels, int c, F f) {
  const int cg = VEC ? c / 4 : c;
  const long total = pixels * cg;
  for (long i = (long)blockIdx.x * 256 + threadIdx.x; i < total; i += (long)gridDim.x * 256) {
    const long p = i / cg;
    const int ch = (int)(i - p * cg) * (VEC ? 4 : 1);
    f(p, ch);
  }
}
static inline int pm_ew_grid(long work) { return (int)std::min<long>((work + 255) / 256, 256 * 16); }
template <typename F>
static inline int pm_ew_launch(bool vec, long pixels, int c, hipStream_t st, const char* name, F f) {
  if (pixels * c == 0) return PM_OK;
  if (vec) hipLaunchKernelGGL((pm_ew_kernel<true, F>), dim3(pm_ew_grid(pixels * c / 4)), dim3(256), 0, st, pixels, c, f);
  else hipLaunchKernelGGL((pm_ew_kernel<false, F>), dim3(pm_ew_grid(pixels * c)), dim3(256), 0, st, pixels, c, f);
  return pm_check_launch(name);
}
static inline bool pm_same_shape(const pm_tensor* a, const pm_tensor* b) { return a->n == b->n && a->h == b->h && a->w == b->w && a->c == b->c; }
static inline bool pm_vec4(const pm_tensor* t) { return pm_vec_ok(t) && t->c % 4 == 0; }
#define PM_LD4(ptr) (*reinterpret_cast<const float4*>(ptr))
#define PM_ST4(ptr, v) (*reinterpret_cast<float4*>(ptr) = (v))
```

pinthememory_amd/csrc/winograd.hip:

```cpp
#include "pm_common.h"

namespace {

enum { W_BT = 0, W_AT = 1, W_G = 2, W_A = 3, W_GT = 4 };

template <int MT>
__host__ __device__ constexpr float wino_bt(int i, int j) {
  if (MT == 2) {
    constexpr float t[4][4] = {{1, 0, -1, 0}, {0, 1, 1, 0}, {0, -1, 1, 0}, {0, 1, 0, -1}};
    return t[i & 3][j & 3];
  }
  constexpr float t[6][6] = {{4, 0, -5, 0, 1, 0}, {0, -4, -4, 1, 1, 0}, {0, 4, -4, -1, 1, 0}, {0, -2, -1, 2, 1, 0}, {0, 2, -1, -2, 1, 0}, {0, 4, 0, -5, 0, 1}};
  return t[i][j];
}
template <int MT>
__host__ __device__ constexpr float wino_at(int i, int j) {
  if (MT == 2) {
    constexpr float t[2][4] = {{1, 1, 1, 0}, {0, 1, -1, -1}};
    return t[i & 1][j & 3];
  }
  constexpr float t[4][6] = {{1, 1, 1, 1, 1, 0}, {0, 1, -1, 2, -2, 0}, {0, 1, 1, 4, 4, 0}, {0, 1, -1, 8, -8, 1}};
  return t[i][j];
}
template <int MT>
// ... 205 lines not shown
    Vec<4> col[3], o[A];
#pragma unroll
    for (int ky = 0; ky < 3; ++ky)
#pragma unroll
      for (int e = 0; e < 4; ++e) col[ky].v[e] = DGRAD ? sg[(2 - ky) * 3 + (2 - kx)][4 * q + e][j] : sg[ky * 3 + kx][j][4 * q + e];
    mat_apply<MT, W_G>(col, o);
#pragma unroll
    for (int a = 0; a < A; ++a) gg[a][kx] = o[a];
  }
  float* out = U + (long)row * Kp + k;
#pragma unroll
  for (int a = 0; a < A; ++a) {
    Vec<4> o[A];
    mat_apply<MT, W_G>(gg[a], o);
#pragma unroll
    for (int b = 0; b < A; ++b) {
#pragma unroll
      for (int e = 0; e < 4; ++e)
        if (k + e >= Kr) o[b].v[e] = 0.f;
      vstore<4>(out + (a * A + b) * plane, o[b]);
    }
  }
}
template <int MT, bool DGRAD>
__global__ __launch_bounds__(256) void wino_filter_kernel(const float* __restrict__ w, int Cout, int Cin, int Kp, float* __restrict__ U) {
  __shared__ float sg[9][32][33];
  wino_filter_block<MT, DGRAD>(w, Cout, Cin, Kp, U, blockIdx.x, blockIdx.y, sg);
}

constexpr int WR_BATCH = 48;
struct WinoRefreshJobs {
  const float* w[WR_BATCH];
  float* U[WR_BATCH];
  int cout[WR_BATCH], cin[WR_BATCH], kp[WR_BATCH], m[WR_BATCH];
  int start[WR_BATCH + 1];
  int n;
};
__global__ __launch_bounds__(256) void wino_filter_multi_kernel(const WinoRefreshJobs t) {
  __shared__ float sg[9][32][33];
  int j = 0;
  while (j + 1 < t.n && (int)blockIdx.x >= t.start[j + 1]) ++j;
  const int local = (int)blockIdx.x - t.start[j];
  const int nbx = t.kp[j] / 32;
  const int bx = local % nbx, by = local / nbx;
  if (t.m[j] == 4) wino_filter_block<4, false>(t.w[j], t.cout[j], t.cin[j], t.kp[j], t.U[j], bx, by, sg);
  else wino_filter_block<2, false>(t.w[j], t.cout[j], t.cin[j], t.kp[j], t.U[j], bx, by, sg);
}

template <int MT, int W>
__global__ __launch_bounds__(256) void wino_dy_kernel(const float* __restrict__ dy, long yp, int Cout, const pm_wino_geom g, float* __restrict__ Z) {
  constexpr int A = MT + 2;
  const unsigned cg = Cout / W;
  const unsigned total = (unsigned)g.tiles * cg;
  const long plane = g.tiles * (long)Cout;
  for (unsigned i = blockIdx.x * 256u + threadIdx.x; i < total; i += gridDim.x * 256u) {
    const unsigned tile = i / cg;
    const int c = (int)(i - tile * cg) * W;
    const TileId t = decode_tile(tile, g);
    Vec<W> r[A][MT];
#pragma unroll
    for (int b = 0; b < MT; ++b) {
      const int xx = t.rx + g.d * (MT * t.tx + b);
      Vec<W> col[MT], o[A];
#pragma unroll
      for (int a = 0; a < MT; ++a) {
        const int yy = t.ry + g.d * (MT * t.ty + a);
        col[a] = (yy < g.H && xx < g.W) ? vload<W>(dy + ((long)(t.n * g.H + yy) * g.W + xx) * yp + c) : vzero<W>();
      }
      mat_apply<MT, W_A>(col, o);
#pragma unroll
      for (int a = 0; a < A; ++a) r[a][b] = o[a];
    }
    float* out = Z + (long)tile * Cout + c;
#pragma unroll
    for (int a = 0; a < A; ++a) {
      Vec<W> o[A];
      mat_apply<MT, W_A>(r[a], o);
#pragma unroll
      for (int b = 0; b < A; ++b) vstore<W>(out + (a * A + b) * plane, o[b]);
    }
  }
}

template <int MT>
__global__ __launch_bounds__(256) void wino_dw_kernel(const float* __restrict__ slab, int ks, int Cout, int Cin, int Kp, float* __restrict__ dw) {
  constexpr int A = MT + 2, P = A * A;
  const long total = (long)Cout * Cin, plane = (long)Cout * Kp;
  for (long i = (long)blockIdx.x * 256 + threadIdx.x; i < total; i += (long)gridDim.x * 256) {
    const int co = (int)(i / Cin), ci = (int)(i - (long)co * Cin);
    const float* in = slab + (long)co * Kp + ci;
    float du[P];
#pragma unroll
    for (int q = 0; q < P; ++q) du[q] = 0.f;
    for (int z = 0; z < ks; ++z) {
      float ld[P];
#pragma unroll
      for (int q = 0; q < P; ++q) ld[q] = in[((long)z * P + q) * plane];
#pragma unroll
      for (int q = 0; q < P; ++q) du[q] += ld[q];
    }
    Vec<1> h[3][A];
#pragma unroll
    for (int b = 0; b < A; ++b) {
      Vec<1> col[A], o[3];
#pragma unroll
      for (int a = 0; a < A; ++a) col[a].v[0] = du[a * A + b];
      mat_apply<MT, W_GT>(col, o);
#pragma unroll
      for (int k = 0; k < 3; ++k) h[k][b] = o[k];
    }
    float* out = dw + (long)co * 9 * Cin + ci;
#pragma unroll
    for (int k = 0; k < 3; ++k) {
      Vec<1> o[3];
      mat_apply<MT, W_GT>(h[k], o);
#pragma unroll
      for (int l = 0; l < 3; ++l) out[(k * 3 + l) * (long)Cin] = o[l].v[0];
    }
  }
}

typedef float f32x16 __attribute__((ext_vector_type(16)));

struct WinoFusedArgs {
  const float* V;
  const float* U;
  float* y;
  long yp;
  int Cout, Kp;
  pm_wino_geom g;
  const float* bias;
  const float* scale;
  const float* shift;
  const float* residual;
  long rp;
  int relu;
  int ncb;
};

constexpr int WF_THREADS = 768, WF_TB = 32, WF_CB = 32, WF_BK = 16, WF_P = 36;
constexpr size_t WF_LDS = (size_t)WF_P * WF_TB * (WF_CB + 1) * sizeof(float);

__device__ __forceinline__ int wf_xcd_remap(int bid, int nwg) {
  const int q = nwg >> 3, r = nwg & 7, xcd = bid & 7, idx = bid >> 3;
  const int base = xcd < r ? xcd * (q + 1) : r * (q + 1) + (xcd - r) * q;
  return base + idx;
}

__global__ __launch_bounds__(WF_THREADS) void wino_fused_f4_kernel(const WinoFusedArgs a) {
  extern __shared__ __align__(16) float4 lds4[];
  const int tid = threadIdx.x, lane = tid & 63, wave = tid >> 6;
  const int lid = wf_xcd_remap(blockIdx.x, gridDim.x);
  const int tb = lid / a.ncb, cb = lid - tb * a.ncb;
  const long tile0 = (long)tb * WF_TB;
  const int co0 = cb * WF_CB;

  const int rem = tid & 255, row = rem >> 2, chunk = rem & 3, pgrp = tid >> 8;
  const bool is_a = row < WF_TB;
  bool valid;
  const float* gp;
  long plane;
  if (is_a) {
    const long tile = tile0 + row;
    valid = tile < a.g.tiles;
    gp = a.V + (valid ? tile : 0) * a.Kp + chunk * 4;
    plane = a.g.tiles * (long)a.Kp;
// ... 88 lines not shown
      mat_apply<MT, W_AT>(sv[aa], o);
#pragma unroll
      for (int b = 0; b < MT; ++b) {
        const int xx = ti.rx + a.g.d * (MT * ti.tx + b);
        if (yy >= a.g.H || xx >= a.g.W) continue;
        const long pix = (long)(ti.n * a.g.H + yy) * a.g.W + xx;
        float v = o[b].v[0];
        if (a.bias) v += bi;
        if (a.scale) v = v * sc + sh;
        if (a.residual) v += a.residual[pix * a.rp + co];
        if (a.relu) v = fmaxf(v, 0.f);
        a.y[pix * a.yp + co] = v;
      }
    }
  }
}

inline unsigned nblocks(long total) { return (unsigned)std::min<long>((total + 255) / 256, 1 << 20); }

}

pm_wino_geom pm_wino_make_geom(int n, int h, int w, int d, int m) {
  pm_wino_geom g;
  g.N = n, g.H = h, g.W = w, g.d = d, g.m = m;
  g.TY = (pm_cdiv(h, d) + m - 1) / m, g.TX = (pm_cdiv(w, d) + m - 1) / m;
  g.tiles = (long)n * d * d * g.TY * g.TX;
  return g;
}

int pm_wino_input_xf(const float* x, long pitch, int C, int Kp, const pm_wino_geom& g, float* V, hipStream_t st) {
  if (g.m == 4) hipLaunchKernelGGL((wino_input_kernel<4, 2>), dim3(nblocks(g.tiles * (Kp / 2))), dim3(256), 0, st, x, pitch, C, Kp, g, V);
  else hipLaunchKernelGGL((wino_input_kernel<2, 4>), dim3(nblocks(g.tiles * (Kp / 4))), dim3(256), 0, st, x, pitch, C, Kp, g, V);
  return pm_check_launch("wino_input");
}

int pm_wino_filter_xf(const float* w, int Cout, int Cin, int Kp, bool dgrad, int m, float* U, hipStream_t st) {
  const int R = dgrad ? Cin : Cout;
  dim3 grid(Kp / 32, pm_cdiv(R, 32));
  if (m == 4) {
    if (dgrad) hipLaunchKernelGGL((wino_filter_kernel<4, true>), grid, dim3(256), 0, st, w, Cout, Cin, Kp, U);
    else hipLaunchKernelGGL((wino_filter_kernel<4, false>), grid, dim3(256), 0, st, w, Cout, Cin, Kp, U);
  } else {
    if (dgrad) hipLaunchKernelGGL((wino_filter_kernel<2, true>), grid, dim3(256), 0, st, w, Cout, Cin, Kp, U);
    else hipLaunchKernelGGL((wino_filter_kernel<2, false>), grid, dim3(256), 0, st, w, Cout, Cin, Kp, U);
  }
  return pm_check_launch("wino_filter");
}

int pm_wino_filter_xf_multi(const float* const* w, float* const* U, const int* cout, const int* cin, const int* kp, const int* m, int n, hipStream_t st) {
  for (int i0 = 0; i0 < n; i0 += WR_BATCH) {
    WinoRefreshJobs t;
    t.n = std::min(WR_BATCH, n - i0);
    long blocks = 0;
    for (int i = 0; i < t.n; ++i) {
      t.w[i] = w[i0 + i], t.U[i] = U[i0 + i], t.cout[i] = cout[i0 + i], t.cin[i] = cin[i0 + i], t.kp[i] = kp[i0 + i], t.m[i] = m[i0 + i];
      t.start[i] = (int)blocks;
      blocks += (long)(kp[i0 + i] / 32) * pm_cdiv(cout[i0 + i], 32);
    }
    t.start[t.n] = (int)blocks;
    if (blocks == 0) continue;
    hipLaunchKernelGGL(wino_filter_multi_kernel, dim3((unsigned)blocks), dim3(256), 0, st, t);
    if (int e = pm_check_launch("wino_filter_multi")) return e;
  }
  return PM_OK;
}

int pm_wino_output_xf(const float* M, int Cout, const pm_wino_geom& g, float* y, long ypitch, const float* bias, const float* scale, const float* shift,
                      const float* residual, long res_pitch, int relu, hipStream_t st) {
  if (g.m == 4)
    hipLaunchKernelGGL((wino_output_kernel<4, 2>), dim3(nblocks(g.tiles * (Cout / 2))), dim3(256), 0, st, M, Cout, g, y, ypitch, bias, scale, shift, residual,
                       res_pitch, relu);
  else
    hipLaunchKernelGGL((wino_output_kernel<2, 4>), dim3(nblocks(g.tiles * (Cout / 4))), dim3(256), 0, st, M, Cout, g, y, ypitch, bias, scale, shift, residual,
                       res_pitch, relu);
  return pm_check_launch("wino_output");
}

int pm_wino_dy_xf(const float* dy, long pitch, int Cout, const pm_wino_geom& g, float* Z, hipStream_t st) {
  if (g.m == 4) hipLaunchKernelGGL((wino_dy_kernel<4, 2>), dim3(nblocks(g.tiles * (Cout / 2))), dim3(256), 0, st, dy, pitch, Cout, g, Z);
  else hipLaunchKernelGGL((wino_dy_kernel<2, 4>), dim3(nblocks(g.tiles * (Cout / 4))), dim3(256), 0, st, dy, pitch, Cout, g, Z);
  return pm_check_launch("wino_dy");
}

int pm_wino_dw_xf(const float* slab, int ks, int Cout, int Cin, int Kp, int m, float* dw, hipStream_t st) {
  const unsigned nb = (unsigned)std::min<long>(((long)Cout * Cin + 255) / 256, 1 << 16);
  if (m == 4) hipLaunchKernelGGL(wino_dw_kernel<4>, dim3(nb), dim3(256), 0, st, slab, ks, Cout, Cin, Kp, dw);
  else hipLaunchKernelGGL(wino_dw_kernel<2>, dim3(nb), dim3(256), 0, st, slab, ks, Cout, Cin, Kp, dw);
  return pm_check_launch("wino_dw");
}

int pm_wino_fused_f4(const float* V, const float* U, int Cout, int Kp, const pm_wino_geom& g, float* y, long ypitch, const float* bias, const float* scale,
                     const float* shift, const float* residual, long res_pitch, int relu, hipStream_t st) {
  static pm_lds_optin optin;
  (void)optin(reinterpret_cast<const void*>(&wino_fused_f4_kernel), (int)WF_LDS);
  WinoFusedArgs a;
  a.V = V, a.U = U, a.y = y, a.yp = ypitch, a.Cout = Cout, a.Kp = Kp, a.g = g;
  a.bias = bias, a.scale = scale, a.shift = shift, a.residual = residual, a.rp = res_pitch, a.relu = relu;
  a.ncb = (Cout + WF_CB - 1) / WF_CB;
  const long ntb = (g.tiles + WF_TB - 1) / WF_TB;
  hipLaunchKernelGGL(wino_fused_f4_kernel, dim3((unsigned)(ntb * a.ncb)), dim3(WF_THREADS), WF_LDS, st, a);
  return pm_check_launch("wino_fused_f4");
}
```

pinthememory_amd/hip/kernels.py:

```python
import ctypes
from ctypes import byref

import os

import torch

from . import lib as L
from .lib import PmConvEpilogue, PmConvParams, check, ptr, stream, tdesc, workspace


def _lib():
    return L.load()


CONV_PREC = 0
ACT_DTYPE = torch.float32


def set_conv_precision(name):
    global CONV_PREC, ACT_DTYPE
    CONV_PREC = {'f32': 0, 'fp32': 0, 'bf16': 2, 'bf16_operands': 2, 'bf16_staged': 1}[name]
    ACT_DTYPE = torch.bfloat16 if name == 'bf16' else torch.float32


# ... 146 lines not shown
    for j, (key, ent, owner) in zip(jobs, todo):
        cout, kh, kw, cin = key[1]
        j.w, j.wxf, j.wxf_bytes, j.cout, j.kh, j.kw, j.cin, j.dgrad = key[0], ent[2].data_ptr(), key[2], cout, kh, kw, cin, 1 if key[5] else 0
        ent[1] = -1
    check(_lib().pm_conv_wxf_refresh_bf16(jobs, len(todo), stream()), 'pm_conv_wxf_refresh_bf16')
    cur = L.stream_obj()
    raw = cur.cuda_stream
    if raw not in _U_STREAMS:
        _U_STREAMS[raw] = cur
    ev = cur.record_event()
    for key, ent, owner in todo:
        ent[1], ent[3], ent[4] = owner._version, ev, raw
    return len(todo)


_SIZES = {}
_GEN = [0]


def _sizes(key, fn):
    v = _SIZES.get(key)
    if v is None:
        if len(_SIZES) > 8192:
            _SIZES.clear()
        v = _SIZES[key] = fn()
    return v


_XFORM_COUNT = [0, False]


def filter_transform_count(enable=None):
    if enable is not None:
        _XFORM_COUNT[1] = bool(enable)
    return _XFORM_COUNT[0]


def conv_fwd(x, w_krsc, stride, pad, dil, bias=None, scale=None, shift=None, residual=None, relu=False, out=None, keep_v=None, bn_partials=None, out_dtype=None):
    cout, kh, kw, cin = w_krsc.shape
    n, h, w_, c = x.shape
    assert c == cin, 'conv: Cin mismatch %d vs %d' % (c, cin)
    ho, wo = conv_out_hw(h, w_, kh, stride, pad, dil)
    y = out if out is not None else new((n, ho, wo, cout), x, pitch_pad=True, dtype=out_dtype if out_dtype is not None else ACT_DTYPE)
    assert residual is None or residual.dtype == y.dtype, 'conv_fwd: the fused residual has the dtype of the output'
    xd, yd = tdesc(x), tdesc(y)
    p = L.conv_params(kh, kw, stride, pad, dil, CONV_PREC)
    lib = _lib()
    nbv, nbu, nb, npb = _sizes(('f', x.shape, x.stride(), x.dtype, xd.flags, w_krsc.shape, y.stride(), y.dtype, stride, pad, dil, CONV_PREC, _GEN[0]),
                               lambda: (lib.pm_conv_winograd_v_bytes(byref(xd), byref(yd), byref(p)), lib.pm_conv_wxf_bytes(byref(xd), byref(yd), byref(p)),
                                        lib.pm_conv_workspace(byref(xd), byref(yd), byref(p), 0), lib.pm_conv_bn_partials_bytes(byref(xd), byref(yd), byref(p))))
    if keep_v is not None:
        nbv = nbv if KEEP_WINOGRAD_V else 0
        v = torch.empty(nbv // 4, dtype=torch.float32, device=x.device) if nbv else None
        keep_v.append(v)
        if v is not None:
            p.wino_v, p.wino_v_bytes = v.data_ptr(), nbv
    u_ent = None
    if (kh == 3 and CONV_PREC == 0) or CONV_PREC == 2:
        u_ent = _wino_u(p, w_krsc, nbu)
    if _XFORM_COUNT[1] and p.wxf_valid == 0 and nbu:
        _XFORM_COUNT[0] += 1
    ws = workspace(nb, x.device) if nb else None
    part = None
    if bn_partials is not None:
        ep16 = BN_EPILOGUE16 or (BN_EP16_MIN_BYTES > 0 and y.numel() * 2 >= BN_EP16_MIN_BYTES)
        ep32 = BN_EPILOGUE or (BN_EP_MIN_BYTES > 0 and y.numel() * 4 >= BN_EP_MIN_BYTES)
        npb = npb if ((ep16 if y.dtype == torch.bfloat16 else ep32) and residual is None and not relu and scale is None) else 0
        part = torch.empty(npb // 4, dtype=torch.float32, device=x.device) if npb else None
        bn_partials.append(part)
    ep = None
    if bias is not None or scale is not None or residual is not None or relu or part is not None:
        rd = tdesc(residual) if residual is not None else None
        ep = L.conv_epilogue(ptr(bias), ptr(scale), ptr(shift), rd.ptr if rd else None, rd.pitch if rd else 0, 1 if relu else 0, ptr(part),
                            part.numel() * 4 if part is not None else 0)
    check(lib.pm_conv_fwd(byref(xd), w_krsc.data_ptr(), byref(yd), byref(p), byref(ep) if ep else None, ptr(ws), nb, stream()), 'pm_conv_fwd')
    if u_ent is not None:
        ent, version = u_ent
        cur = L.stream_obj()
        ent[3], ent[4] = cur.record_event(), cur.cuda_stream
        ent[1] = version
    return y


def conv_bwd_data(dy, w_krsc, x_shape, stride, pad, dil, add=None, dtype=None, add_mask=None):
    cout, kh, kw, cin = w_krsc.shape
    dx = new(x_shape, dy, dtype=dtype)
    dyd, dxd = tdesc(dy), tdesc(dx)
    p = L.conv_params(kh, kw, stride, pad, dil, CONV_PREC)
    lib = _lib()
    nb, nbu = _sizes(('d', dy.shape, dy.stride(), dy.dtype, dyd.flags, w_krsc.shape, dx.shape, dx.stride(), dx.dtype, stride, pad, dil, CONV_PREC, _GEN[0]),
                     lambda: (lib.pm_conv_workspace(byref(dxd), byref(dyd), byref(p), 1), lib.pm_conv_wxf_bytes_dgrad(byref(dyd), byref(dxd), byref(p))))
    ws = workspace(nb, dy.device) if nb else None
    ad = tdesc(add) if add is not None else None
    u_ent = _wino_u(p, w_krsc, nbu, dgrad=True) if CONV_PREC == 2 else None
    if add_mask is not None:
        check(lib.pm_conv_bwd_data_masked(byref(dyd), w_krsc.data_ptr(), byref(dxd), byref(p), byref(ad), add_mask.data_ptr(), ptr(ws), nb, stream()), 'pm_conv_bwd_data_masked')
    else:
        check(lib.pm_conv_bwd_data(byref(dyd), w_krsc.data_ptr(), byref(dxd), byref(p), byref(ad) if ad else None, ptr(ws), nb, stream()), 'pm_conv_bwd_data')
    if u_ent is not None:
        ent, version = u_ent
        cur = L.stream_obj()
        ent[3], ent[4] = cur.record_event(), cur.cuda_stream
        ent[1] = version
    return dx


def conv_bwd_weight(x, dy, w_shape_krsc, stride, pad, dil, want_bias=False, wino_v=None, on_stream=None):
    cout, kh, kw, cin = w_shape_krsc
    dw = torch.empty(w_shape_krsc, dtype=torch.float32, device=x.device)
    db = torch.empty(cout, dtype=torch.float32, device=x.device) if want_bias else None
    xd, dyd = tdesc(x), tdesc(dy)
    p = L.conv_params(kh, kw, stride, pad, dil, CONV_PREC)
    if wino_v is not None:
        p.wino_v, p.wino_v_bytes = wino_v.data_ptr(), wino_v.numel() * 4
    lib = _lib()
    nb = _sizes(('w', x.shape, x.stride(), x.dtype, dy.shape, dy.stride(), dy.dtype, w_shape_krsc, stride, pad, dil, CONV_PREC, wino_v is not None, _GEN[0]),
                lambda: lib.pm_conv_workspace(byref(xd), byref(dyd), byref(p), 2))
    raw = stream() if on_stream is None else on_stream.cuda_stream
    ws = workspace(nb, x.device, on_stream)
    check(lib.pm_conv_bwd_weight(byref(xd), byref(dyd), dw.data_ptr(), ptr(db), byref(p), ptr(ws), nb, raw), 'pm_conv_bwd_weight')
    return dw, db


def bn_stats(x):
    c = x.shape[3]
    mom = torch.empty(3 * c, dtype=torch.float32, device=x.device)
    xd = tdesc(x)
    lib = _lib()
    nb = _sizes(('bn', x.shape, x.dtype), lambda: lib.pm_bn_workspace(byref(xd)))
    ws = workspace(nb, x.device)
    check(lib.pm_bn_stats(byref(xd), mom.data_ptr(), ptr(ws), nb, stream()), 'pm_bn_stats')
    return mom


def bn_stats_finalize(x, eps, running_mean=None, running_var=None, momentum=0.1):
    c = x.shape[3]
    mean = torch.empty(c, dtype=torch.float32, device=x.device)
    invstd = torch.empty_like(mean)
    xd = tdesc(x)
    lib = _lib()
    nb = _sizes(('bn', x.shape, x.dtype), lambda: lib.pm_bn_workspace(byref(xd)))
    ws = workspace(nb, x.device)
    check(lib.pm_bn_stats_finalize(byref(xd), eps, mean.data_ptr(), invstd.data_ptr(), ptr(running_mean), ptr(running_var), momentum, ptr(ws), nb, stream()),
          'pm_bn_stats_finalize')
    return mean, invstd


def bn_partials_finalize(part, pixels, c, eps, running_mean=None, running_var=None, momentum=0.1):
    mean = torch.empty(c, dtype=torch.float32, device=part.device)
    invstd = torch.empty_like(mean)
    check(_lib().pm_bn_partials_finalize(part.data_ptr(), pixels, c, eps, mean.data_ptr(), invstd.data_ptr(), ptr(running_mean), ptr(running_var), momentum, None,
                                         stream()), 'pm_bn_partials_finalize')
    return mean, invstd


def bn_partials_moments(part, pixels, c):
    mom = torch.empty(3 * c, dtype=torch.float32, device=part.device)
    check(_lib().pm_bn_partials_finalize(part.data_ptr(), pixels, c, 0.0, None, None, None, None, 0.0, mom.data_ptr(), stream()), 'pm_bn_partials_finalize')
    return mom


def bn_merge(parts, world, c):
    out = torch.empty(3 * c, dtype=torch.float32, device=parts.device)
    check(_lib().pm_bn_merge(parts.data_ptr(), world, c, out.data_ptr(), stream()), 'pm_bn_merge')
    return out


def bn_merge_finalize(parts, world, c, eps, running_mean=None, running_var=None, momentum=0.1):
    mean = torch.empty(c, dtype=torch.float32, device=parts.device)
    invstd = torch.empty_like(mean)
    check(_lib().pm_bn_merge_finalize(parts.data_ptr(), world, c, eps, mean.data_ptr(), invstd.data_ptr(), ptr(running_mean), ptr(running_var), momentum,
                                      stream()), 'pm_bn_merge_finalize')
    return mean, invstd


def bn_finalize(moments, c, eps, running_mean=None, running_var=None, momentum=0.1):
    mean = torch.empty(c, dtype=torch.float32, device=moments.device)
    invstd = torch.empty_like(mean)
    check(_lib().pm_bn_finalize(moments.data_ptr(), c, eps, mean.data_ptr(), invstd.data_ptr(), ptr(running_mean), ptr(running_var), momentum, stream()),
          'pm_bn_finalize')
    return mean, invstd


def bn_fold_multi(table, cs, offs, n, max_c, total, eps):
    arena = torch.empty(2 * total, dtype=torch.float32, device=table.device)
    check(_lib().pm_bn_fold_multi(table.data_ptr(), cs.data_ptr(), offs.data_ptr(), n, max_c, total, eps, arena.data_ptr(), stream()), 'pm_bn_fold_multi')
    return arena


def bn_fold(gamma, beta, running_mean, running_var, eps, conv_bias=None):
    c = gamma.numel()
    scale = torch.empty(c, dtype=torch.float32, device=gamma.device)
    shift = torch.empty_like(scale)
    check(_lib().pm_bn_fold(gamma.data_ptr(), beta.data_ptr(), running_mean.data_ptr(), running_var.data_ptr(), ptr(conv_bias), c, eps, scale.data_ptr(),
                            shift.data_ptr(), stream()), 'pm_bn_fold')
    return scale, shift


def bn_apply(x, mean, invstd, gamma, beta, residual=None, relu=False, out=None, want_mask=False):
    y = out if out is not None else torch.empty_like(x, memory_format=torch.contiguous_format)
    rd = tdesc(residual) if residual is not None else None
    grp = 8 if x.dtype == torch.bfloat16 else 4
    mask = torch.empty((x.shape[0] * x.shape[1] * x.shape[2], x.shape[3] // grp), dtype=torch.uint8, device=x.device) if want_mask else None
    check(_lib().pm_bn_apply_mask(byref(tdesc(x)), mean.data_ptr(), invstd.data_ptr(), gamma.data_ptr(), beta.data_ptr(), byref(rd) if rd else None,
# ... 560 lines not shown
```

pinthememory_amd/hip/lib.py:

```python
import ctypes
import os
from ctypes import POINTER, byref, c_char_p, c_float, c_int, c_int32, c_int64, c_size_t, c_void_p

import torch

_HERE = os.path.dirname(os.path.dirname(os.path.abspath(__file__)))
LIB_PATH = os.environ.get('PM_LIB') or os.path.join(_HERE, 'libpinmem_hip.so')


class PmTensor(ctypes.Structure):
    _fields_ = [('ptr', c_void_p), ('n', c_int32), ('h', c_int32), ('w', c_int32), ('c', c_int32), ('pitch', c_int64), ('dtype', c_int32), ('flags', c_int32)]


PM_F32, PM_BF16 = 0, 1
PM_TF_ZERO_PAD64 = 1


class PmSgdEntry(ctypes.Structure):
    _fields_ = [('param', c_void_p), ('grad', c_void_p), ('momentum_buffer', c_void_p), ('numel', c_int64)]


class PmWxfJob(ctypes.Structure):
    _fields_ = [('w', c_void_p), ('wxf', c_void_p), ('wxf_bytes', c_int64), ('cout', c_int32), ('kh', c_int32), ('kw', c_int32), ('cin', c_int32),
                ('dgrad', c_int32), ('reserved', c_int32)]


class PmConvParams(ctypes.Structure):
    _fields_ = [('struct_size', c_int32), ('kh', c_int32), ('kw', c_int32), ('stride', c_int32), ('pad', c_int32), ('dil', c_int32), ('prec', c_int32),
                ('wino_v', c_void_p), ('wino_v_bytes', c_int64),
                ('wxf', c_void_p), ('wxf_bytes', c_int64), ('wxf_valid', c_int32)]


class PmRouting(ctypes.Structure):
    _fields_ = [('struct_size', c_int32), ('winograd', c_int32), ('winograd_fused', c_int32), ('conv16', c_int32), ('conv16_wide', c_int32),
                ('conv16_persistent', c_int32), ('wgrad16', c_int32), ('bf16_wgrad', c_int32), ('split', c_int32)]


class PmConvEpilogue(ctypes.Structure):
    _fields_ = [('struct_size', c_int64), ('bias', c_void_p), ('scale', c_void_p), ('shift', c_void_p), ('residual', c_void_p),
                ('residual_pitch', c_int64), ('relu', c_int32), ('bn_partials', c_void_p), ('bn_partials_bytes', c_int64)]


def conv_params(kh, kw, stride, pad, dil, prec=0):
    return PmConvParams(ctypes.sizeof(PmConvParams), kh, kw, stride, pad, dil, prec)


def conv_epilogue(*fields):
    return PmConvEpilogue(ctypes.sizeof(PmConvEpilogue), *fields)


ABI_VERSION = 400


class PinmemError(RuntimeError):
    pass


_T, _P, _E = POINTER(PmTensor), POINTER(PmConvParams), POINTER(PmConvEpilogue)
_vp, _sz, _i, _f, _i64 = c_void_p, c_size_t, c_int, c_float, c_int64

SIGNATURES = {
    'pm_last_error': (c_char_p, []),
    'pm_version': (c_int, []),
    'pm_conv_winograd_v_bytes': (_sz, [_T, _T, _P]),
    'pm_conv_wxf_bytes': (_sz, [_T, _T, _P]),
    'pm_conv_wxf_bytes_dgrad': (_sz, [_T, _T, _P]),
    'pm_conv_wxf_refresh_bf16': (_i, [_vp, _i, _vp]),
    'pm_conv_wxf_refresh_f32': (_i, [_vp, _i, _vp]),
    'pm_conv_workspace': (_sz, [_T, _T, _P, _i]),
    'pm_conv_fwd': (_i, [_T, _vp, _T, _P, _E, _vp, _sz, _vp]),
    'pm_conv_bwd_data': (_i, [_T, _vp, _T, _P, _T, _vp, _sz, _vp]),
    'pm_conv_bwd_data_masked': (_i, [_T, _vp, _T, _P, _T, _vp, _vp, _sz, _vp]),
    'pm_conv_bwd_weight': (_i, [_T, _T, _vp, _vp, _P, _vp, _sz, _vp]),
    'pm_set_winograd': (_i, [_i]),
    'pm_set_winograd_fused': (_i, [_i]),
    'pm_set_conv16': (_i, [_i]),
    'pm_profile_enable': (_i, [_i]),
    'pm_profile_dump': (_i, [ctypes.c_char_p]),
    'pm_profile_read': (_i, [_i, _i, _i, _i, _i, POINTER(ctypes.c_double), POINTER(ctypes.c_double), POINTER(c_int64), _i]),
    'pm_profile_read_prec': (_i, [_i, _i, _i, _i, _i, _i, POINTER(ctypes.c_double), POINTER(ctypes.c_double), POINTER(c_int64), _i]),
    'pm_profile_read_bytes': (_i, [_i, _i, _i, _i, _i, _i, POINTER(ctypes.c_double)]),
    'pm_bn_workspace': (_sz, [_T]),
    'pm_bn_stats': (_i, [_T, _vp, _vp, _sz, _vp]),
    'pm_bn_merge': (_i, [_vp, _i, _i, _vp, _vp]),
    'pm_bn_merge_finalize': (_i, [_vp, _i, _i, _f, _vp, _vp, _vp, _vp, _f, _vp]),
    'pm_bn_finalize': (_i, [_vp, _i, _f, _vp, _vp, _vp, _vp, _f, _vp]),
    'pm_bn_stats_finalize': (_i, [_T, _f, _vp, _vp, _vp, _vp, _f, _vp, _sz, _vp]),
    'pm_bn_fold': (_i, [_vp, _vp, _vp, _vp, _vp, _i, _f, _vp, _vp, _vp]),
    'pm_bn_fold_multi': (_i, [_vp, _vp, _vp, _i, _i, _i, _f, _vp, _vp]),
    'pm_bn_apply': (_i, [_T, _vp, _vp, _vp, _vp, _T, _i, _T, _vp]),
    'pm_bn_apply_mask': (_i, [_T, _vp, _vp, _vp, _vp, _T, _i, _T, _vp, _vp]),
    'pm_bn_bwd_reduce_mask': (_i, [_T, _vp, _T, _vp, _vp, _T, _vp, _vp, _sz, _vp]),
    'pm_bn_apply_mask_affine': (_i, [_T, _vp, _vp, _vp, _vp, _T, _vp, _vp, _vp, _vp, _i, _T, _vp, _vp]),
    'pm_bn_bwd_apply_mask': (_i, [_T, _vp, _T, _vp, _vp, _vp, _vp, _f, _T, _vp]),
    'pm_bn_bwd_reduce': (_i, [_T, _T, _T, _vp, _vp, _vp, _vp, _i, _T, _vp, _vp, _sz, _vp]),
    'pm_bn_bwd_apply': (_i, [_T, _T, _T, _vp, _vp, _vp, _vp, _vp, _f, _i, _T, _T, _vp]),
    'pm_relu_bwd': (_i, [_T, _T, _T, _vp]),
    'pm_add': (_i, [_T, _T, _T, _vp]),
    'pm_add_n': (_i, [POINTER(_T), _i, _T, _vp]),
    'pm_copy': (_i, [_T, _T, _vp]),
    'pm_scale_shift_act': (_i, [_T, _vp, _vp, _T, _i, _T, _vp]),
    'pm_maxpool3x3s2_fwd': (_i, [_T, _T, _vp, _vp]),
    'pm_maxpool3x3s2_bwd': (_i, [_T, _vp, _T, _vp]),
    'pm_maxpool3x3s2_bn_relu_fwd': (_i, [_T, _vp, _vp, _vp, _vp, _T, _vp, _vp]),
    'pm_bn_bwd_reduce_pool': (_i, [_T, _vp, _T, _vp, _vp, _vp, _vp, _vp, _vp, _sz, _vp]),
    'pm_bn_bwd_apply_pool': (_i, [_T, _vp, _T, _vp, _vp, _vp, _vp, _vp, _f, _T, _vp]),
    'pm_global_avgpool_fwd': (_i, [_T, _T, _vp]),
    'pm_global_avgpool_bwd': (_i, [_T, _T, _i, _vp]),
    'pm_resize_bilinear_fwd': (_i, [_T, _T, _vp]),
    'pm_resize_bilinear_bwd': (_i, [_T, _T, _i, _vp]),
    'pm_resize_bilinear_bwd_workspace': (_sz, [_T, _T]),
    'pm_resize_bilinear_bwd_separable': (_i, [_T, _T, _i, _vp, _sz, _vp]),
    'pm_resize_bilinear_hp_fwd': (_i, [_T, _T, _i, _vp]),
    'pm_softmax_mean_update': (_i, [_T, _vp, _i, _vp]),
    'pm_sliding_stitch': (_i, [_T, _vp, _i, _i, _i, _i, _vp, _i, _vp]),
    'pm_argmax_f64': (_i, [_vp, _i, _i, _i, _i, _vp, _vp, _vp]),
    'pm_image_u8_to_nhwc4': (_i, [_vp, _i64, POINTER(c_float), POINTER(c_float), _vp, _vp]),
    'pm_labels_u8_to_i64': (_i, [_vp, _i64, _vp, _vp]),
    'pm_nchw_to_nhwc': (_i, [_vp, _i, _T, _vp]),
    'pm_nhwc_to_nchw': (_i, [_T, _vp, _vp]),
    'pm_label_nearest': (_i, [_vp, _i, _i, _i, _vp, _i, _i, _vp]),
    'pm_upsample_ce_workspace': (_sz, [_i, _i, _i]),
    'pm_upsample_ce_fwd': (_i, [_T, _f, _vp, _i, _i, _vp, _vp, _sz, _vp]),
    'pm_upsample_ce_bwd_workspace': (_sz, [_T, _i, _i]),
    'pm_upsample_ce_bwd': (_i, [_T, _f, _vp, _i, _i, _vp, _vp, _T, _vp, _sz, _vp]),
    'pm_upsample_ce_field_bytes': (_sz, [_T, _i, _i]),
    'pm_upsample_ce_fwd_field': (_i, [_T, _f, _vp, _i, _i, _vp, _vp, _vp, _sz, _vp]),
    'pm_upsample_ce_bwd_field': (_i, [_T, _f, _i, _i, _vp, _vp, _vp, _T, _vp]),
    'pm_upsample_wce_loss_floats': (_sz, [_i]),
    'pm_upsample_wce_workspace': (_sz, [_i, _i, _i]),
    'pm_upsample_wce_fwd': (_i, [_T, _f, _vp, _i, _i, _vp, _i64, _i, _vp, _vp, _sz, _vp]),
    'pm_upsample_wce_fwd_field': (_i, [_T, _f, _vp, _i, _i, _vp, _i64, _i, _vp, _vp, _vp, _sz, _vp]),
    'pm_upsample_wce_bwd_field': (_i, [_T, _f, _i, _i, _i, _vp, _vp, _vp, _T, _vp]),
    'pm_label_class_weights_workspace': (_sz, [_i]),
    'pm_label_class_weights': (_i, [_vp, _i, _i, _i, _i, ctypes.c_double, _i, _i, _vp, _vp, _sz, _vp]),
    'pm_mem_read_fwd': (_i, [_T, _vp, _i, _vp, _T, _vp, _vp, _vp]),
    'pm_mem_read_fwd_pq_workspace': (_sz, [_i64, _i]),
    'pm_mem_read_fwd_pq': (_i, [_T, _vp, _i, _vp, _vp, _T, _vp, _vp, _vp, _vp, _sz, _vp]),
    'pm_mem_colsoftmax_workspace': (_sz, [_i64, _i]),
    'pm_mem_colsoftmax': (_i, [_vp, _vp, _i64, _i, _vp, _vp, _sz, _vp]),
    'pm_mem_read_bwd_workspace': (_sz, [_i64, _i, _i]),
    'pm_mem_read_bwd': (_i, [_T, _vp, _i, _vp, _T, _vp, _T, _vp, _vp, _sz, _vp]),
    'pm_mem_write_accum_workspace': (_sz, [_T, _i]),
    'pm_mem_write_accum': (_i, [_T, _vp, _i, _i, _i, _i, _vp, _vp, _sz, _vp]),
    'pm_mem_write_accum_bwd': (_i, [_T, _vp, _i, _i, _i, _i, _vp, _T, _vp]),
    'pm_mem_write_update': (_i, [_vp, _vp, _i, _i, _f, _vp, _vp, _vp]),
    'pm_mem_write_update_bwd': (_i, [_vp, _vp, _i, _i, _f, _vp, _vp, _vp, _vp]),
    'pm_sgd_momentum': (_i, [_vp, _vp, _vp, _i64, _f, _f, _f, _i, _vp]),
    'pm_set_bf16_wgrad': (_i, [_i]),
    'pm_set_wgrad16': (_i, [_i]),
    'pm_set_split': (_i, [_i]),
    'pm_routing_get': (_i, [POINTER(PmRouting)]),
    'pm_routing_set': (_i, [POINTER(PmRouting)]),
    'pm_conv_bn_partials_bytes': (_sz, [_T, _T, POINTER(PmConvParams)]),
    'pm_bn_partials_finalize': (_i, [_vp, _i64, _i, _f, _vp, _vp, _vp, _vp, _f, _vp, _vp]),
    'pm_sgd_momentum_multi': (_i, [_vp, _i, _f, _f, _f, _vp]),
    'pm_sgd_momentum_multi_dev': (_i, [_vp, _i, _f, _vp, _f, _f, _vp]),
    'pm_cast': (_i, [_T, _T, _vp]),
}

_lib = None


def load():
    global _lib
    if _lib is not None:
        return _lib
    if not os.environ.get('PM_LIB'):
        from .. import build as _build
        _build.build()
    lib = ctypes.CDLL(LIB_PATH)
    for name, (res, args) in SIGNATURES.items():
        fn = getattr(lib, name)
        fn.restype, fn.argtypes = res, args
    if lib.pm_version() != ABI_VERSION:
        raise PinmemError('%s reports ABI %d, this binding is written against %d (include/pinmem_hip.h)' % (LIB_PATH, lib.pm_version(), ABI_VERSION))
    _lib = lib
    return lib


def check(code, what=''):
    if code != 0:
        raise PinmemError('%s failed (%d): %s' % (what, code, load().pm_last_error().decode()))


_raw_stream = torch._C._cuda_getCurrentRawStream
_cur_device = torch._C._cuda_getDevice


def stream():
    return _raw_stream(_cur_device())


_ZERO_PAD = {}


def register_zero_pad(base, c, pitch):
    import weakref
    if len(_ZERO_PAD) > 64:
        for k in [k for k, v in _ZERO_PAD.items() if v[0]() is None]:
            del _ZERO_PAD[k]
    _ZERO_PAD[base.data_ptr()] = (weakref.ref(base), c, pitch)


_TD = {}


def tdesc(t):
    key = (t.shape, t.stride(), t.dtype)
    m = _TD.get(key)
    if m is None:
        assert t.dim() == 4 and t.dtype in (torch.float32, torch.bfloat16) and t.is_cuda, 'expected a CUDA fp32 / bf16 NHWC tensor, got %s %s' % (tuple(t.shape), t.dtype)
        n, h, w, c = t.shape
        sn, sh, sw, sc = t.stride()
        pitch = sw if w > 1 else (sh if h > 1 else (sn if n > 1 else c))
        assert (sc == 1 or c == 1) and pitch >= c, 'channels must be innermost: shape %s stride %s' % (tuple(t.shape), t.stride())
        assert (h == 1 or w == 1 or sh == w * pitch) and (n == 1 or h * w == 1 or sn == h * w * pitch), \
            'not an NHWC view: shape %s stride %s' % (tuple(t.shape), t.stride())
        if len(_TD) > 4096:
            _TD.clear()
        m = _TD[key] = (n, h, w, c, pitch, PM_F32 if t.dtype == torch.float32 else PM_BF16)
    assert t.is_cuda
    if m[5] == PM_F32 or m[3] % 64 == 0:
        return PmTensor(t.data_ptr(), m[0], m[1], m[2], m[3], m[4], m[5], 0)
    flags = 0
    z = _ZERO_PAD.get(t.data_ptr())
    if z is not None and z[0]() is not None and z[1] == m[3] and z[2] == m[4]:
        flags = PM_TF_ZERO_PAD64
    return PmTensor(t.data_ptr(), m[0], m[1], m[2], m[3], m[4], m[5], flags)


_ws = {}


def workspace(nbytes, device, on_stream=None):
    key = (device.index, stream() if on_stream is None else on_stream.cuda_stream)
    buf = _ws.get(key)
    if buf is None or buf.numel() < nbytes:
        buf = torch.empty(max(int(nbytes), 1 << 20), dtype=torch.uint8, device=device)
        if on_stream is not None:
            buf.record_stream(on_stream)
# ... 18 lines not shown
```

pinthememory_amd/hip/ops.py:

```python
import os as _os

import torch

from . import kernels as K
from . import lib as L
from .. import dist as D


def nhwc(t):
    v = t.permute(0, 2, 3, 1)
    n, h, w, c = v.shape
    sn, sh, sw, sc = v.stride()
    pitch = sw if w > 1 else (sh if h > 1 else (sn if n > 1 else c))
    ok = (sc == 1 or c == 1) and pitch >= c and (h == 1 or w == 1 or sh == w * pitch) and (n == 1 or h * w == 1 or sn == h * w * pitch)
    if ok and v.dtype == torch.float32:
        return v
    if v.dtype == torch.bfloat16:
        if ok and pitch % 8 == 0 and c % 8 == 0 and v.data_ptr() % 16 == 0:
            return v
        return v.contiguous()
    if h * w == 1:
        return v.contiguous().float()
    return K.nchw_to_nhwc(t.float())

# ... 24 lines not shown


_nbt_pending = []


def flush_bn_counters():
    if _nbt_pending:
        torch._foreach_add_(_nbt_pending, 1)
        _nbt_pending.clear()


_OVERLAP_ENV = _os.environ.get('PM_OVERLAP_WGRAD')
OVERLAP_WGRAD = True if _OVERLAP_ENV is None else _OVERLAP_ENV == '1'


def overlap_wgrad():
    if not OVERLAP_WGRAD:
        return False
    return not (_OVERLAP_ENV is None and K.CONV_PREC == 2 and K.ACT_DTYPE == torch.bfloat16)


_side = {}
_proxy = {}


def masked_stream(n_cus, device=None, first=0):
    import ctypes
    dev = torch.cuda.current_device() if device is None else device
    total = torch.cuda.get_device_properties(dev).multi_processor_count
    n_cus = max(1, min(int(n_cus), total))
    words = (total + 31) // 32
    mask = (ctypes.c_uint32 * words)()
    picked = {(first + (i * total) // n_cus) % total for i in range(n_cus)}
    for cu in picked:
        mask[cu // 32] |= 1 << (cu % 32)
    hip = ctypes.CDLL('libamdhip64.so')
    st = ctypes.c_void_p()
    with torch.cuda.device(dev):
        err = hip.hipExtStreamCreateWithCUMask(ctypes.byref(st), ctypes.c_uint32(words), mask)
    if err != 0 or not st.value:
        raise RuntimeError('hipExtStreamCreateWithCUMask(%d CUs) failed: %d' % (n_cus, err))
    return torch.cuda.ExternalStream(st.value, device=dev)


WGRAD_CUS = int(_os.environ.get('PM_WGRAD_CUS', '0'))


def _side_stream():
    dev = torch.cuda.current_device()
    if dev not in _side:
        _side[dev] = masked_stream(WGRAD_CUS, dev) if WGRAD_CUS > 0 else torch.cuda.Stream(device=dev)
    return _side[dev]


class _Defer(torch.autograd.Function):
    @staticmethod
    def forward(ctx, w):
        return w.view_as(w)

    @staticmethod
    def backward(ctx, g):
        L.stream_obj().wait_stream(_side_stream())
        return g


def begin_forward():
    flush_bn_counters()
    _proxy.clear()


def defer_weights(module):
    if not (overlap_wgrad() and torch.is_grad_enabled()):
        return
    for m in module.modules():
        if isinstance(m, torch.nn.Conv2d) and m.bias is None and m.weight.requires_grad and id(m.weight) not in _proxy:
            _proxy[id(m.weight)] = _Defer.apply(m.weight)


def _w(weight):
    p = _proxy.get(id(weight))
    return (p, True) if p is not None else (weight, False)


def _wgrad(x, dy, wshape, geom, want_bias=False, deferred=False, wino_v=None):
    if not deferred:
        return K.conv_bwd_weight(x, dy, wshape, *geom, want_bias=want_bias, wino_v=wino_v)
    side, main = _side_stream(), L.stream_obj()
    ev = torch.cuda.Event()
    ev.record(main)
    side.wait_event(ev)
    out = K.conv_bwd_weight(x, dy, wshape, *geom, want_bias=want_bias, wino_v=wino_v, on_stream=side)
    if wino_v is not None:
        wino_v.record_stream(side)
    x.record_stream(side)
    dy.record_stream(side)
    for t in out:
        if t is not None:
            t.record_stream(side)
    return out


commit_done = {}


def wait_commit():
    if not commit_done or not torch.cuda.is_available():
        return
    ev = commit_done.pop(torch.cuda.current_device(), None)
    if ev is not None:
        torch.cuda.current_stream().wait_event(ev)


BN_FUSED_FINALIZE = _os.environ.get('PM_BN_FUSED', '1') == '1'


RELU_MASK_BYTES = _os.environ.get('PM_BN_MASK', '1') == '1'


MERGE_SYNCBN = _os.environ.get('PM_MERGE_SYNCBN', '1') == '1'


def _bn_train_stats_multi(ys, bns, partials):
    c = ys[0].shape[3]
    moms = []
    for y, part in zip(ys, partials):
        pixels = y.shape[0] * y.shape[1] * y.shape[2]
        moms.append(K.bn_partials_moments(part, pixels, c) if part is not None else K.bn_stats(y))
    n = len(ys)
    flat, world = D.gather_moments(torch.cat(moms), bns[0].group)
    parts = flat.view(world, n, 3 * c)
    return [K.bn_merge_finalize(parts[:, i].contiguous().view(-1), world, c, bn.eps, bn.running_mean, bn.running_var, bn.momentum) for i, bn in enumerate(bns)]


def _mergeable(bns, ys):
    return (MERGE_SYNCBN and BN_FUSED_FINALIZE and D.is_dist() and len(bns) > 1 and all(b.group is not None and b.group is bns[0].group for b in bns)
            and len({y.shape[3] for y in ys}) == 1)


def _bn_train_stats(y, bn, partials=None):
    c = y.shape[3]
    pixels = y.shape[0] * y.shape[1] * y.shape[2]
    if bn.group is None and BN_FUSED_FINALIZE:
        if partials is not None:
            mean, invstd = K.bn_partials_finalize(partials, pixels, c, bn.eps, bn.running_mean, bn.running_var, bn.momentum)
        else:
            mean, invstd = K.bn_stats_finalize(y, bn.eps, bn.running_mean, bn.running_var, bn.momentum)
    elif bn.group is not None and D.is_dist() and BN_FUSED_FINALIZE:
        mom = K.bn_partials_moments(partials, pixels, c) if partials is not None else K.bn_stats(y)
        flat, world = D.gather_moments(mom, bn.group)
        mean, invstd = K.bn_merge_finalize(flat, world, c, bn.eps, bn.running_mean, bn.running_var, bn.momentum)
    else:
        mom = K.bn_partials_moments(partials, pixels, c) if partials is not None else K.bn_stats(y)
        if bn.group is not None:
            mom = D.merge_moments(mom, c, bn.group)
        mean, invstd = K.bn_finalize(mom, c, bn.eps, bn.running_mean, bn.running_var, bn.momentum)
    return mean, invstd


def _bn_train_fwd(y, gamma, beta, bn, residual, relu, out=None, partials=None, want_mask=False):
    mean, invstd = _bn_train_stats(y, bn, partials)
    if want_mask:
        o, mask = K.bn_apply(y, mean, invstd, gamma, beta, residual=residual, relu=relu, out=out, want_mask=True)
        return o, mean, invstd, mask
    return K.bn_apply(y, mean, invstd, gamma, beta, residual=residual, relu=relu, out=out), mean, invstd


def _bn_train_bwd(dv, o, y, mean, invstd, gamma, beta, relu, group, want_dres, has_res, mask=None):
    c = y.shape[3]
    mode = 0 if not relu else (1 if has_res else 2)
    hand_over = mode == 1 and want_dres
    if hand_over and mask is not None:
        sums, gm = K.bn_bwd_reduce_mask(dv, mask, y, mean, invstd, want_gmask=True, with_count=group is not None)
    else:
        sums, gm = K.bn_bwd_reduce(dv, o, y, mean, invstd, mode, gamma, beta, want_gmask=hand_over, with_count=group is not None)
    local = sums
    if group is not None:
        sums = D.all_reduce_sum_copy(local, group)
    count = float(y.shape[0] * y.shape[1] * y.shape[2]) if group is None else -1.0
    if hand_over:
        dy, _ = K.bn_bwd_apply(gm, None, y, mean, invstd, gamma, sums, count, 0, False)
        dres = gm
    else:
        dy, dres = K.bn_bwd_apply(dv, o, y, mean, invstd, gamma, sums, count, mode, want_dres, beta)
    return dy, dres, local[c:2 * c], local[:c]


def _bn_bwd_masked(dv, mask, y, mean, invstd, gamma, group):
    c = y.shape[3]
    local, _ = K.bn_bwd_reduce_mask(dv, mask, y, mean, invstd, want_gmask=False, with_count=group is not None)
    sums = local if group is None else D.all_reduce_sum_copy(local, group)
    count = float(y.shape[0] * y.shape[1] * y.shape[2]) if group is None else -1.0
    return K.bn_bwd_apply_mask(dv, mask, y, mean, invstd, gamma, sums, count), local[c:2 * c], local[:c]


class _Bottleneck(torch.autograd.Function):

    @staticmethod
    def forward(ctx, x, w1, g1, b1, w2, g2, b2, w3, g3, b3, wd, gd, bd, geoms, bns, deferred):
        xv = nhwc(x)
        k1, k2, k3 = K.krsc(w1), K.krsc(w2), K.krsc(w3)
        ps = []
        y1 = K.conv_fwd(xv, k1, *geoms[0], bn_partials=ps)
        o1, m1, i1 = _bn_train_fwd(y1, g1, b1, bns[0], None, True, partials=ps[0])
        kv = []
        y2 = K.conv_fwd(o1, k2, *geoms[1], keep_v=kv, bn_partials=ps)
        o2, m2, i2 = _bn_train_fwd(y2, g2, b2, bns[1], None, True, partials=ps[1])
        y3 = K.conv_fwd(o2, k3, *geoms[2], bn_partials=ps)
        merged = False
        if wd is not None:
            kd = K.krsc(wd)
            yd = K.conv_fwd(xv, kd, *geoms[3], bn_partials=ps)
            merged = _mergeable([bns[3], bns[2]], [yd, y3])
            fold = y3.dtype == torch.float32 and yd.dtype == torch.float32
            if merged:
                (md, idd), (m3, i3) = _bn_train_stats_multi([yd, y3], [bns[3], bns[2]], [ps[3], ps[2]])
                res = None if fold else K.bn_apply(yd, md, idd, gd, bd, residual=None, relu=False)
            elif fold:
                md, idd = _bn_train_stats(yd, bns[3], ps[3])
                m3, i3 = _bn_train_stats(y3, bns[2], ps[2])
                res = None
            else:
                res, md, idd = _bn_train_fwd(yd, gd, bd, bns[3], None, False, partials=ps[3])
        else:
            kd = yd = md = idd = None
            res = xv
        if res is None:
            out, mask3 = K.bn_apply_res_affine(y3, m3, i3, g3, b3, yd, md, idd, gd, bd, relu=True, want_mask=True)
            if not RELU_MASK_BYTES:
                mask3 = None
        elif merged:
            out, mask3 = K.bn_apply(y3, m3, i3, g3, b3, residual=res, relu=True, want_mask=True) if RELU_MASK_BYTES else (K.bn_apply(y3, m3, i3, g3, b3, residual=res, relu=True), None)
        elif RELU_MASK_BYTES:
            out, m3, i3, mask3 = _bn_train_fwd(y3, g3, b3, bns[2], res, True, partials=ps[2], want_mask=True)
        else:
            (out, m3, i3), mask3 = _bn_train_fwd(y3, g3, b3, bns[2], res, True, partials=ps[2]), None
        ctx.geoms, ctx.groups, ctx.has_ds, ctx.deferred = geoms, [b.group for b in bns], wd is not None, deferred
        ctx.save_for_backward(xv, k1, k2, k3, kd, y1, o1, y2, o2, y3, yd, out, m1, i1, m2, i2, m3, i3, md, idd, g1, g2, g3, gd, b1, b2, b3, kv[0], mask3)
        return nchw(out)

    @staticmethod
    def backward(ctx, dout):
        xv, k1, k2, k3, kd, y1, o1, y2, o2, y3, yd, out, m1, i1, m2, i2, m3, i3, md, idd, g1, g2, g3, gd, b1, b2, b3, v2, mask3 = ctx.saved_tensors
        ge, gr, df = ctx.geoms, ctx.groups, ctx.deferred
        dv = _grad_view(dout)
        pair = None
        if ctx.has_ds and MERGE_SYNCBN and D.is_dist() and gr[2] is not None and gr[3] is gr[2] and y3.shape[3] == yd.shape[3]:
            c3 = y3.shape[3]
            if mask3 is not None:
                s3, gm = K.bn_bwd_reduce_mask(dv, mask3, y3, m3, i3, want_gmask=True, with_count=True)
            else:
                s3, gm = K.bn_bwd_reduce(dv, out, y3, m3, i3, 1, g3, b3, want_gmask=True, with_count=True)
            sd, _ = K.bn_bwd_reduce(gm, None, yd, md, idd, 0, gd, None, want_gmask=False, with_count=True)
            both = D.all_reduce_sum_copy(torch.cat([s3, sd]), gr[2])
            g3sum, gdsum = both[:s3.numel()], both[s3.numel():]
            dy3, _ = K.bn_bwd_apply(gm, None, y3, m3, i3, g3, g3sum, -1.0, 0, False)
            dres, dg3, db3 = gm, s3[c3:2 * c3], s3[:c3]
            dyd, _ = K.bn_bwd_apply(gm, None, yd, md, idd, gd, gdsum, -1.0, 0, False, None)
            pair = (dyd, sd[c3:2 * c3], sd[:c3])
        elif mask3 is not None and dv.dtype == torch.float32 and K.CONV_PREC != 2:
            dy3, dg3, db3 = _bn_bwd_masked(dv, mask3, y3, m3, i3, g3, gr[2])
            dres = None
        else:
            dy3, dres, dg3, db3 = _bn_train_bwd(dv, out, y3, m3, i3, g3, b3, True, gr[2], True, True, mask=mask3)
        dw3, _ = _wgrad(o2, dy3, tuple(k3.shape), ge[2], deferred=df[2])
        do2 = K.conv_bwd_data(dy3, k3, tuple(o2.shape), *ge[2])
        dy2, _, dg2, db2 = _bn_train_bwd(do2, o2, y2, m2, i2, g2, b2, True, gr[1], False, False)
        dw2, _ = _wgrad(o1, dy2, tuple(k2.shape), ge[1], deferred=df[1], wino_v=v2)
        do1 = K.conv_bwd_data(dy2, k2, tuple(o1.shape), *ge[1])
        dy1, _, dg1, db1 = _bn_train_bwd(do1, o1, y1, m1, i1, g1, b1, True, gr[0], False, False)
        dw1, _ = _wgrad(xv, dy1, tuple(k1.shape), ge[0], deferred=df[0])
        dwd = dgd = dbd = None
        skip, skip_mask = (dres, None) if dres is not None else (dv, mask3)
        if ctx.has_ds:
            if pair is not None:
                dyd, dgd, dbd = pair
            elif dres is None:
                dyd, dgd, dbd = _bn_bwd_masked(dv, mask3, yd, md, idd, gd, gr[3])
            else:
                dyd, _, dgd, dbd = _bn_train_bwd(dres, None, yd, md, idd, gd, None, False, gr[3], False, False)
            dwdk, _ = _wgrad(xv, dyd, tuple(kd.shape), ge[3], deferred=df[3])
            dwd = dwdk.permute(0, 3, 1, 2)
            skip, skip_mask = (K.conv_bwd_data(dyd, kd, tuple(xv.shape), *ge[3]) if ctx.needs_input_grad[0] else None), None
        dx = nchw(K.conv_bwd_data(dy1, k1, tuple(xv.shape), *ge[0], add=skip, add_mask=skip_mask)) if ctx.needs_input_grad[0] else None
        p = lambda d: d.permute(0, 3, 1, 2)
        return dx, p(dw1), dg1, db1, p(dw2), dg2, db2, p(dw3), dg3, db3, dwd, dgd, dbd, None, None, None


FOLD_BATCH = _os.environ.get('PM_FOLD_BATCH', '1') == '1'
_fold_cache = None
fold_misses = 0
last_prefold_event = None


class prefold:
    def __init__(self, model):
        self.model, self.active = model, False

    def __enter__(self):
        global _fold_cache, last_prefold_event
        last_prefold_event = None
        m = self.model
        if not FOLD_BATCH or m.training or torch.is_grad_enabled() or _fold_cache is not None:
            return self
        bns = getattr(m, '_pm_bn_list', None)
        if bns is None:
            bns = [b for b in m.modules() if isinstance(b, torch.nn.modules.batchnorm._BatchNorm)]
            m.__dict__['_pm_bn_list'] = bns
        bns = [b for b in bns if b.running_mean is not None and b.weight is not None and b.running_mean.is_cuda and not b.training]
        if not bns or len({b.eps for b in bns}) != 1:
            return self
        ptrs = tuple(t.data_ptr() for b in bns for t in (b.weight, b.bias, b.running_mean, b.running_var))
        plan = m.__dict__.get('_pm_fold_plan')
        if plan is None or plan[0] != ptrs:
            dev = bns[0].running_mean.device
            cs = [b.num_features for b in bns]
            offs, tot = [], 0
            for c in cs:
                offs.append(tot)
                tot += (c + 3) // 4 * 4
            as_i64 = [p - (1 << 64) if p >= (1 << 63) else p for p in ptrs]
            plan = (ptrs, torch.tensor(as_i64, dtype=torch.int64, device=dev), torch.tensor(cs, dtype=torch.int32, device=dev),
                    torch.tensor(offs, dtype=torch.int32, device=dev), cs, offs, tot)
            m.__dict__['_pm_fold_plan'] = plan
        _, table, dcs, doffs, cs, offs, tot = plan
        arena = K.bn_fold_multi(table, dcs, doffs, len(cs), max(cs), tot, bns[0].eps)
        _fold_cache = {b.running_mean.data_ptr(): (arena[o:o + c], arena[tot + o:tot + o + c]) for b, c, o in zip(bns, cs, offs)}
        self.active = True
        last_prefold_event = torch.cuda.current_stream().record_event() if len(bns) == len(m.__dict__['_pm_bn_list']) else None
        return self

    def __exit__(self, *exc):
        global _fold_cache
        if self.active:
            _fold_cache = None
        return False


class _ConvBnAct(torch.autograd.Function):

    @staticmethod
    def forward(ctx, x, w, bias, gamma, beta, residual, geom, bn, relu, out, deferred=False):
        stride, pad, dil = geom
        xv, wk = nhwc(x), K.krsc(w)
        rv = nhwc(residual) if residual is not None else None
        ov = nhwc(out) if out is not None else None
        ctx.geom, ctx.relu, ctx.train, ctx.deferred = geom, relu, bn.training, deferred and bias is None
        needs_grad = bn.grad_enabled and any(ctx.needs_input_grad[:6])
        if not bn.training and not needs_grad:
            hit = _fold_cache.get(bn.running_mean.data_ptr()) if (_fold_cache is not None and bias is None) else None
            if hit is None:
                global fold_misses
                fold_misses += 1
            scale, shift = hit if hit is not None else K.bn_fold(gamma, beta, bn.running_mean, bn.running_var, bn.eps, bias)
            o = K.conv_fwd(xv, wk, stride, pad, dil, scale=scale, shift=shift, residual=rv, relu=relu, out=ov)
            return nchw(o)
        kv, ps = [], []
        y = K.conv_fwd(xv, wk, stride, pad, dil, bias=bias, keep_v=kv if ctx.needs_input_grad[1] else None, bn_partials=ps if bn.training else None)
        if bn.training:
            o, mean, invstd = _bn_train_fwd(y, gamma, beta, bn, rv, relu, ov, partials=ps[0])
        else:
            mean, invstd = bn.running_mean, torch.rsqrt(bn.running_var + bn.eps)
            o = K.bn_apply(y, mean, invstd, gamma, beta, residual=rv, relu=relu, out=ov)
        ctx.group, ctx.has_bias, ctx.has_res = bn.group, bias is not None, residual is not None
        ctx.save_for_backward(xv, wk, y, o, mean, invstd, gamma, beta, kv[0] if kv else None)
        return nchw(o)

    @staticmethod
    def backward(ctx, dout):
        xv, wk, y, o, mean, invstd, gamma, beta, vk = ctx.saved_tensors
        stride, pad, dil = ctx.geom
        dv = _grad_view(dout)
        want_dres = ctx.has_res and ctx.needs_input_grad[5]
        if ctx.train:
            dy, dres, dgamma, dbeta = _bn_train_bwd(dv, o, y, mean, invstd, gamma, beta, ctx.relu, ctx.group, want_dres, ctx.has_res)
        else:
            c = y.shape[3]
            mode = 0 if not ctx.relu else (1 if ctx.has_res else 2)
            sums, g = K.bn_bwd_reduce(dv, o, y, mean, invstd, mode, gamma, beta, want_gmask=mode != 0)
            g = dv if g is None else g
            dy = K.scale_shift_act(g, gamma * invstd, torch.zeros_like(gamma))
            dres, dgamma, dbeta = (g if want_dres else None), sums[c:], sums[:c]
        dx = nchw(K.conv_bwd_data(dy, wk, tuple(xv.shape), stride, pad, dil, dtype=xv.dtype)) if ctx.needs_input_grad[0] else None
        dw = db = None
        if ctx.needs_input_grad[1] or (ctx.has_bias and ctx.needs_input_grad[2]):
            dwk, db = _wgrad(xv, dy, tuple(wk.shape), (stride, pad, dil), want_bias=ctx.has_bias, deferred=ctx.deferred, wino_v=vk)
            dw = dwk.permute(0, 3, 1, 2)
        return dx, dw, db, dgamma, dbeta, (nchw(dres) if dres is not None else None), None, None, None, None, None


class _Stem(torch.autograd.Function):

    @staticmethod
    def forward(ctx, x, w, gamma, beta, geom, bn):
        xv, wk = nhwc(x), K.krsc(w)
        kv, ps = [], []
        y = K.conv_fwd(xv, wk, *geom, keep_v=kv if ctx.needs_input_grad[1] else None, bn_partials=ps)
        mean, invstd = _bn_train_stats(y, bn, ps[0])
        out, arg = K.maxpool_bn_relu_fwd(y, mean, invstd, gamma, beta)
        ctx.geom, ctx.group = geom, bn.group
        ctx.save_for_backward(xv, wk, y, mean, invstd, gamma, beta, arg, kv[0] if kv else None)
        return nchw(out)

    @staticmethod
    def backward(ctx, dout):
        xv, wk, y, mean, invstd, gamma, beta, arg, vk = ctx.saved_tensors
        c = y.shape[3]
        grp = ctx.group
        dy, local = K.bn_relu_bwd_pool(_grad_view(dout), arg, y, mean, invstd, gamma, beta, with_count=grp is not None,
                                       reduce_sums=(lambda s: D.all_reduce_sum_copy(s, grp)) if grp is not None else None)
        dx = nchw(K.conv_bwd_data(dy, wk, tuple(xv.shape), *ctx.geom, dtype=xv.dtype)) if ctx.needs_input_grad[0] else None
        dw = None
        if ctx.needs_input_grad[1]:
            dwk, _ = _wgrad(xv, dy, tuple(wk.shape), ctx.geom, wino_v=vk)
            dw = dwk.permute(0, 3, 1, 2)
        return dx, dw, local[c:2 * c], local[:c], None, None


def stem_tail(x, w, conv, bn):
    st = BNState(bn)
    if st.training and torch.is_grad_enabled() and K.ACT_DTYPE == torch.float32 and x.dtype == torch.float32 and w.shape[0] % 4 == 0:
        return _Stem.apply(x, w, bn.weight, bn.bias, _geom(conv), st)
    return maxpool3x3s2(_ConvBnAct.apply(x, w, None, bn.weight, bn.bias, None, _geom(conv), st, True, None))


class _ConvBnActN(torch.autograd.Function):

    @staticmethod
    def forward(ctx, n, geoms, bns, outs, deferreds, *ts):
        xs, ws, gammas, betas = ts[0:n], ts[n:2 * n], ts[2 * n:3 * n], ts[3 * n:4 * n]
        xvs, wks = [nhwc(x) for x in xs], [K.krsc(w) for w in ws]
        ys, kvs, parts = [], [], []
        for i in range(n):
            kv, ps = [], []
            ys.append(K.conv_fwd(xvs[i], wks[i], *geoms[i], keep_v=kv if ctx.needs_input_grad[5 + n + i] else None, bn_partials=ps))
            kvs.append(kv[0] if kv else None)
            parts.append(ps[0])
        stats = _bn_train_stats_multi(ys, bns, parts)
        os_ = [K.bn_apply(ys[i], stats[i][0], stats[i][1], gammas[i], betas[i], residual=None, relu=True, out=nhwc(outs[i]) if outs[i] is not None else None) for i in range(n)]
        ctx.n, ctx.geoms, ctx.group, ctx.deferreds = n, geoms, bns[0].group, deferreds
        ctx.save_for_backward(*xvs, *wks, *ys, *os_, *[st[0] for st in stats], *[st[1] for st in stats], *gammas, *betas, *kvs)
        return tuple(nchw(o) for o in os_)

    @staticmethod
    def backward(ctx, *douts):
        n = ctx.n
        sv = ctx.saved_tensors
        xvs, wks, ys, os_, means, invs, gammas, betas, kvs = (sv[i * n:(i + 1) * n] for i in range(9))
        c = ys[0].shape[3]
        red = [K.bn_bwd_reduce(_grad_view(douts[i]), os_[i], ys[i], means[i], invs[i], 2, gammas[i], betas[i], want_gmask=False, with_count=True) for i in range(n)]
        tot = D.all_reduce_sum_copy(torch.cat([r[0] for r in red]), ctx.group)
        ln = red[0][0].numel()
        dxs, dws, dgs, dbs = [], [], [], []
        for i in range(n):
            dy, _ = K.bn_bwd_apply(_grad_view(douts[i]), os_[i], ys[i], means[i], invs[i], gammas[i], tot[i * ln:(i + 1) * ln], -1.0, 2, False, betas[i])
            dxs.append(nchw(K.conv_bwd_data(dy, wks[i], tuple(xvs[i].shape), *ctx.geoms[i], dtype=xvs[i].dtype)) if ctx.needs_input_grad[5 + i] else None)
            dwk, _ = _wgrad(xvs[i], dy, tuple(wks[i].shape), ctx.geoms[i], deferred=ctx.deferreds[i], wino_v=kvs[i])
            dws.append(dwk.permute(0, 3, 1, 2))
            dgs.append(red[i][0][c:2 * c]), dbs.append(red[i][0][:c])
        return (None, None, None, None, None, *dxs, *dws, *dgs, *dbs)


def conv_bn_act_n(xs, seqs, outs):
    convs, bns_m = [q[0] for q in seqs], [q[1] for q in seqs]
    ok = MERGE_SYNCBN and BN_FUSED_FINALIZE and D.is_dist() and torch.is_grad_enabled() and all(b.training for b in bns_m) and all(cv.bias is None for cv in convs)
    if ok:
        groups = [D.bn_group(b) for b in bns_m]
        ok = all(g is not None and g is groups[0] for g in groups) and len({cv.out_channels for cv in convs}) == 1
# ... 347 lines not shown
```

Baseline: 153.7.

## Fuse BN-backward apply into Winograd dy/input transforms for dgrad and wgrad

Adds a kernel that applies the batch-norm backward (ReLU gate and dx formula) and writes the Winograd-domain tensors for both the data-gradient input transform and the weight-gradient dy transform in a single pass. Downstream Winograd dgrad and wgrad accept a pre-transformed dy via a new tensor flag, which skips their own transforms and the intermediate dy tensor. This removes a full read/write of the BN-backward output plus two separate transform passes for 3x3 convs where both gradients take the Winograd route. It adds two transformed buffers held at once, more routing checks, and only applies for plain BN+ReLU layers without groups, bias or residual.

```diff
diff --git a/include/pinmem_hip.h b/include/pinmem_hip.h
--- a/include/pinmem_hip.h
+++ b/include/pinmem_hip.h
@@ -11,6 +11,7 @@
 
 typedef enum pm_dtype { PM_F32 = 0, PM_BF16 = 1 } pm_dtype;
 #define PM_TF_ZERO_PAD64 1
+#define PM_TF_WINO_XF 2
 
 typedef struct pm_tensor {
   void* ptr;
@@ -71,6 +72,10 @@
                             const pm_tensor* add, const uint8_t* add_mask, void* ws, size_t ws_bytes, void* stream);
 int pm_conv_bwd_weight(const pm_tensor* x, const pm_tensor* dy, float* dw_krsc, float* dbias, const pm_conv_params* p,
                        void* ws, size_t ws_bytes, void* stream);
+size_t pm_conv_bn_bwd_winograd_bytes(const pm_tensor* x, const pm_tensor* y, const pm_conv_params* p, int which );
+int pm_conv_bn_bwd_winograd(const pm_tensor* dout, const pm_tensor* y, const pm_tensor* x, const pm_conv_params* p, const float* mean, const float* invstd,
+                            const float* gamma, const float* beta, const float* sums, float count, float* vdy, size_t vdy_bytes, float* z, size_t z_bytes,
+                            void* stream);
 
 typedef struct pm_routing {
   int32_t struct_size;
diff --git a/pinthememory_amd/csrc/bn.hip b/pinthememory_amd/csrc/bn.hip
--- a/pinthememory_amd/csrc/bn.hip
+++ b/pinthememory_amd/csrc/bn.hip
@@ -517,16 +517,14 @@
     const float4 v = PM_LD4(px + p * c + ch), mu = PM_LD4(mean + ch), is = PM_LD4(invstd + ch), ga = PM_LD4(gamma + ch);
     if (from_x) {
       const float4 be = PM_LD4(beta + ch);
-      g.x = bn_affine(v.x, mu.x, is.x, ga.x, be.x) > 0.f ? g.x : 0.f, g.y = bn_affine(v.y, mu.y, is.y, ga.y, be.y) > 0.f ? g.y : 0.f;
-      g.z = bn_affine(v.z, mu.z, is.z, ga.z, be.z) > 0.f ? g.z : 0.f, g.w = bn_affine(v.w, mu.w, is.w, ga.w, be.w) > 0.f ? g.w : 0.f;
+      g.x = pm_bn_relu_gate(g.x, v.x, mu.x, is.x, ga.x, be.x), g.y = pm_bn_relu_gate(g.y, v.y, mu.y, is.y, ga.y, be.y);
+      g.z = pm_bn_relu_gate(g.z, v.z, mu.z, is.z, ga.z, be.z), g.w = pm_bn_relu_gate(g.w, v.w, mu.w, is.w, ga.w, be.w);
     }
     if (pdr) PM_ST4(pdr + p * e2 + ch, g);
     const float4 s1 = PM_LD4(sums + ch), s2 = PM_LD4(sums + C + ch);
     float4 r;
-    r.x = (g.x - s1.x * inv_n - (v.x - mu.x) * is.x * (s2.x * inv_n)) * (is.x * ga.x);
-    r.y = (g.y - s1.y * inv_n - (v.y - mu.y) * is.y * (s2.y * inv_n)) * (is.y * ga.y);
-    r.z = (g.z - s1.z * inv_n - (v.z - mu.z) * is.z * (s2.z * inv_n)) * (is.z * ga.z);
-    r.w = (g.w - s1.w * inv_n - (v.w - mu.w) * is.w * (s2.w * inv_n)) * (is.w * ga.w);
+    r.x = pm_bn_bwd_dx(g.x, v.x, mu.x, is.x, ga.x, s1.x, s2.x, inv_n), r.y = pm_bn_bwd_dx(g.y, v.y, mu.y, is.y, ga.y, s1.y, s2.y, inv_n);
+    r.z = pm_bn_bwd_dx(g.z, v.z, mu.z, is.z, ga.z, s1.z, s2.z, inv_n), r.w = pm_bn_bwd_dx(g.w, v.w, mu.w, is.w, ga.w, s1.w, s2.w, inv_n);
     PM_ST4(pdx + p * d + ch, r);
   });
 }
@@ -552,10 +550,8 @@
     const float4 v = PM_LD4(px + p * c + ch), mu = PM_LD4(mean + ch), is = PM_LD4(invstd + ch), ga = PM_LD4(gamma + ch);
     const float4 s1 = PM_LD4(sums + ch), s2 = PM_LD4(sums + C + ch);
     float4 r;
-    r.x = (g.x - s1.x * inv_n - (v.x - mu.x) * is.x * (s2.x * inv_n)) * (is.x * ga.x);
-    r.y = (g.y - s1.y * inv_n - (v.y - mu.y) * is.y * (s2.y * inv_n)) * (is.y * ga.y);
-    r.z = (g.z - s1.z * inv_n - (v.z - mu.z) * is.z * (s2.z * inv_n)) * (is.z * ga.z);
-    r.w = (g.w - s1.w * inv_n - (v.w - mu.w) * is.w * (s2.w * inv_n)) * (is.w * ga.w);
+    r.x = pm_bn_bwd_dx(g.x, v.x, mu.x, is.x, ga.x, s1.x, s2.x, inv_n), r.y = pm_bn_bwd_dx(g.y, v.y, mu.y, is.y, ga.y, s1.y, s2.y, inv_n);
+    r.z = pm_bn_bwd_dx(g.z, v.z, mu.z, is.z, ga.z, s1.z, s2.z, inv_n), r.w = pm_bn_bwd_dx(g.w, v.w, mu.w, is.w, ga.w, s1.w, s2.w, inv_n);
     PM_ST4(pdx + p * d + ch, r);
   });
 }
@@ -605,10 +601,8 @@
     g.z = bn_affine(v.z, mu.z, is.z, ga.z, be.z) > 0.f ? g.z : 0.f, g.w = bn_affine(v.w, mu.w, is.w, ga.w, be.w) > 0.f ? g.w : 0.f;
     const float4 s1 = PM_LD4(sums + ch), s2 = PM_LD4(sums + C + ch);
     float4 r;
-    r.x = (g.x - s1.x * inv_n - (v.x - mu.x) * is.x * (s2.x * inv_n)) * (is.x * ga.x);
-    r.y = (g.y - s1.y * inv_n - (v.y - mu.y) * is.y * (s2.y * inv_n)) * (is.y * ga.y);
-    r.z = (g.z - s1.z * inv_n - (v.z - mu.z) * is.z * (s2.z * inv_n)) * (is.z * ga.z);
-    r.w = (g.w - s1.w * inv_n - (v.w - mu.w) * is.w * (s2.w * inv_n)) * (is.w * ga.w);
+    r.x = pm_bn_bwd_dx(g.x, v.x, mu.x, is.x, ga.x, s1.x, s2.x, inv_n), r.y = pm_bn_bwd_dx(g.y, v.y, mu.y, is.y, ga.y, s1.y, s2.y, inv_n);
+    r.z = pm_bn_bwd_dx(g.z, v.z, mu.z, is.z, ga.z, s1.z, s2.z, inv_n), r.w = pm_bn_bwd_dx(g.w, v.w, mu.w, is.w, ga.w, s1.w, s2.w, inv_n);
     PM_ST4(pdx + p * d + ch, r);
   });
 }
diff --git a/pinthememory_amd/csrc/conv_igemm.hip b/pinthememory_amd/csrc/conv_igemm.hip
--- a/pinthememory_amd/csrc/conv_igemm.hip
+++ b/pinthememory_amd/csrc/conv_igemm.hip
@@ -500,12 +500,14 @@
 inline size_t wino_ws(const WinoPlan& wp) { return wp.v_bytes + wp.m_bytes + wp.u_bytes; }
 
 int wino_conv(const pm_tensor* xin, const float* w, int w_cout, int w_cin, bool dgrad, const pm_tensor* yout, const WinoPlan& wp,
-              const pm_conv_epilogue& ep, void* ws, hipStream_t st, float* v_keep = nullptr, float* u_ext = nullptr, bool u_valid = false) {
-  float* V = v_keep ? v_keep : (float*)ws;
-  float* Mo = (float*)((char*)ws + wp.v_bytes);
-  float* U = u_ext ? u_ext : (float*)((char*)ws + wp.v_bytes + wp.m_bytes);
+              const pm_conv_epilogue& ep, void* ws, hipStream_t st, float* v_keep = nullptr, float* u_ext = nullptr, bool u_valid = false, bool v_given = false) {
+  float* V = v_given ? (float*)xin->ptr : (v_keep ? v_keep : (float*)ws);
+  const size_t v_own = v_given ? 0 : wp.v_bytes;
+  float* Mo = (float*)((char*)ws + v_own);
+  float* U = u_ext ? u_ext : (float*)((char*)ws + v_own + wp.m_bytes);
   const int cout = yout->c;
-  if (int e = pm_wino_input_xf((const float*)xin->ptr, xin->pitch, xin->c, wp.Kp, wp.g, V, st)) return e;
+  if (!v_given)
+    if (int e = pm_wino_input_xf((const float*)xin->ptr, xin->pitch, xin->c, wp.Kp, wp.g, V, st)) return e;
   if (!(u_ext && u_valid))
     if (int e = pm_wino_filter_xf(w, w_cout, w_cin, wp.Kp, dgrad, wp.g.m, U, st)) return e;
   const pm_tensor xv = {V, 1, 1, (int32_t)wp.g.tiles, wp.Kp, wp.Kp};
@@ -549,14 +551,15 @@
 inline size_t wino_wgrad_ws(const WinoPlan& wp, const WinoWgradPlan& q) { return wp.v_bytes + wp.m_bytes + q.slab_bytes; }
 
 int wino_wgrad(const pm_tensor* x, const pm_tensor* dy, float* dw, const WinoPlan& wp, const WinoWgradPlan& q, void* ws, hipStream_t st,
-               float* v_kept = nullptr) {
+               float* v_kept = nullptr, bool z_given = false) {
   float* V = v_kept ? v_kept : (float*)ws;
-  float* Z = (float*)((char*)ws + wp.v_bytes);
-  float* slab = (float*)((char*)ws + wp.v_bytes + wp.m_bytes);
+  float* Z = z_given ? (float*)dy->ptr : (float*)((char*)ws + wp.v_bytes);
+  float* slab = (float*)((char*)ws + wp.v_bytes + (z_given ? 0 : wp.m_bytes));
   const int cout = dy->c;
   if (!v_kept)
     if (int e = pm_wino_input_xf((const float*)x->ptr, x->pitch, x->c, wp.Kp, wp.g, V, st)) return e;
-  if (int e = pm_wino_dy_xf((const float*)dy->ptr, dy->pitch, cout, wp.g, Z, st)) return e;
+  if (!z_given)
+    if (int e = pm_wino_dy_xf((const float*)dy->ptr, dy->pitch, cout, wp.g, Z, st)) return e;
   const pm_tensor xv = {V, 1, 1, (int32_t)wp.g.tiles, wp.Kp, wp.Kp};
   const pm_tensor zv = {Z, 1, 1, (int32_t)wp.g.tiles, cout, cout};
   const pm_conv_params p1 = {(int32_t)sizeof(pm_conv_params), 1, 1, 1, 0, 1, 0};
@@ -888,12 +891,14 @@
   size_t v_keep_bytes;
   size_t wxf_bytes;
   size_t bn_bytes;
+  bool pre;
 };
 
 ConvRoute route_conv(int which, const pm_tensor* x, const pm_tensor* y, const pm_conv_params* p) {
   ConvRoute r{};
   long M, Nn, K;
   gemm_dims(which, x, y, p, M, Nn, K);
+  r.pre = which != MODE_FWD && (y->flags & PM_TF_WINO_XF) != 0;
   if (which == MODE_FWD) {
     if ((r.wino = wino_plan(x, y->c, p)).use) {
       r.kind = R_WINO, r.ws_bytes = wino_ws(r.wino), r.wxf_bytes = r.wino.u_bytes;
@@ -921,7 +926,7 @@
     } else if (dgrad_bf16_ok(p) && (r.pe = dgrad_as_fwd(p), r.b16 = bf16_plan(y, x, &r.pe)).use) {
       r.kind = R_BF16, r.ws_bytes = bf16_ws(r.b16), r.wxf_bytes = r.b16.wb_bytes;
     } else if ((r.wino = wino_plan(y, x->c, p)).use) {
-      r.kind = R_WINO, r.ws_bytes = wino_ws(r.wino);
+      r.kind = R_WINO, r.ws_bytes = wino_ws(r.wino) - (r.pre ? r.wino.v_bytes : 0);
     } else {
       r.kind = R_DIRECT, r.pl = make_plan(MODE_DGRAD, M, Nn, K, p->prec != 0), r.ws_bytes = pm_align_up(r.pl.ws_bytes, 256);
     }
@@ -932,7 +937,7 @@
     if (!tier && (r.b16w = bf16_wgrad_plan(x, y, p)).use) {
       r.kind = R_BF16_WGRAD, own = bf16_wgrad_ws(r.b16w);
     } else if (!tier && (r.wino = wino_plan(x, y->c, p, true)).use) {
-      r.kind = R_WINO_WGRAD, r.wino_w = wino_wgrad_plan(r.wino, y->c), own = wino_wgrad_ws(r.wino, r.wino_w);
+      r.kind = R_WINO_WGRAD, r.wino_w = wino_wgrad_plan(r.wino, y->c), own = wino_wgrad_ws(r.wino, r.wino_w) - (r.pre ? r.wino.m_bytes : 0);
     } else {
       r.kind = R_DIRECT_WGRAD, r.pl = make_plan(MODE_WGRAD, M, Nn, K, p->prec != 0), own = r.pl.ws_bytes;
       if (r.native16) {
@@ -1245,6 +1250,7 @@
   PM_REQUIRE(!add || !pm_is_bf16(add) || pm_vec8(add), PM_EINVAL, "conv_bwd_data: bf16 `add` must be 16B aligned with pitch %% 8 == 0");
   PM_REQUIRE(w && pm_aligned16(w), PM_EINVAL, "conv_bwd_data: weight null or unaligned");
   const ConvRoute r = route_conv(MODE_DGRAD, dx, dy, p);
+  PM_REQUIRE(!r.pre || r.kind == R_WINO, PM_EUNSUPPORTED, "conv_bwd_data: a Winograd-transformed dy (PM_TF_WINO_XF) is served by the Winograd route only; this call routes elsewhere");
   PM_REQUIRE(ws_bytes >= r.ws_bytes && (ws || r.ws_bytes == 0), PM_EWORKSPACE, "conv_bwd_data: workspace %zu < %zu", ws_bytes, r.ws_bytes);
   if (add_mask) {
     PM_REQUIRE(add && pm_is_f32(add) && pm_is_f32(dy) && pm_vec4(add) && pm_vec4(dx), PM_EINVAL, "conv_bwd_data: a masked `add` is an fp32 tensor with 16-byte rows and c %% 4 == 0");
@@ -1261,11 +1267,57 @@
       char* wext = (p->wxf && (size_t)p->wxf_bytes >= r.b16.wb_bytes) ? (char*)p->wxf : nullptr;
       return conv_bf16(dy, w, dy->c, dx->c, true, dx, &r.pe, r.b16, e1, ws, st, wext, p->wxf_valid != 0);
     }
-    case R_WINO: return wino_conv(dy, w, dy->c, dx->c, true, dx, r.wino, e1, ws, st);
+    case R_WINO: return wino_conv(dy, w, dy->c, dx->c, true, dx, r.wino, e1, ws, st, nullptr, nullptr, false, r.pre);
     default:
       PM_REQUIRE(pm_is_f32(dy), PM_EUNSUPPORTED, "conv_bwd_data: a bf16 dy needs at least 32 channels and a stride-1 geometry the forward form covers");
       return conv_direct<MODE_DGRAD>(dx, dy, w, p, r.pl, e1, ws, st, add_mask);
   }
+}
+
+namespace {
+struct WinoBnBwdRoute {
+  bool ok;
+  WinoPlan d, w;
+};
+WinoBnBwdRoute wino_bn_bwd_route(const pm_tensor* x, const pm_tensor* y, const pm_conv_params* p0) {
+  WinoBnBwdRoute q{};
+  if (!x || !y || !p0 || !pm_is_f32(x) || !pm_is_f32(y) || check_common(x, y, p0) != PM_OK) return q;
+  const pm_conv_params tp = tier_params(p0, x, y);
+  pm_tensor yy = *y;
+  yy.flags &= ~PM_TF_WINO_XF;
+  const ConvRoute rd = route_conv(MODE_DGRAD, x, &yy, &tp), rw = route_conv(MODE_WGRAD, x, &yy, &tp);
+  if (rd.kind != R_WINO || rw.kind != R_WINO_WGRAD) return q;
+  q.d = rd.wino, q.w = rw.wino;
+  q.ok = q.d.g.m == q.w.g.m && q.d.g.tiles == q.w.g.tiles && q.d.g.TY == q.w.g.TY && q.d.g.TX == q.w.g.TX && q.d.g.d == q.w.g.d;
+  return q;
+}
+}
+
+extern "C" size_t pm_conv_bn_bwd_winograd_bytes(const pm_tensor* x, const pm_tensor* y, const pm_conv_params* p0, int which) {
+  const WinoBnBwdRoute q = wino_bn_bwd_route(x, y, p0);
+  if (!q.ok || which < 0 || which > 1) return 0;
+  return which == 0 ? q.d.v_bytes : q.w.m_bytes;
+}
+
+extern "C" int pm_conv_bn_bwd_winograd(const pm_tensor* dout, const pm_tensor* y, const pm_tensor* x, const pm_conv_params* p0, const float* mean, const float* invstd,
+                                       const float* gamma, const float* beta, const float* sums, float count, float* vdy, size_t vdy_bytes, float* z, size_t z_bytes,
+                                       void* stream) {
+  PM_REQUIRE(dout && y && x && p0 && dout->ptr && y->ptr, PM_EINVAL, "conv_bn_bwd_winograd: null tensor");
+  PM_REQUIRE_F32(dout, "conv_bn_bwd_winograd");
+  PM_REQUIRE_F32(y, "conv_bn_bwd_winograd");
+  PM_REQUIRE_F32(x, "conv_bn_bwd_winograd");
+  PM_REQUIRE(pm_same_shape(dout, y) && pm_vec4(dout) && pm_vec4(y) && dout->pitch >= dout->c && y->pitch >= y->c, PM_EINVAL,
+             "conv_bn_bwd_winograd: dout and y are fp32 tensors of one shape with 16-byte rows and c %% 4 == 0");
+  PM_REQUIRE(mean && invstd && gamma && beta && sums, PM_EINVAL, "conv_bn_bwd_winograd: statistics, parameters and sums are required");
+  pm_tensor xs = *x;
+  if (!xs.ptr) xs.ptr = y->ptr;
+  if (int e = check_common(&xs, y, p0)) return e;
+  const WinoBnBwdRoute q = wino_bn_bwd_route(&xs, y, p0);
+  PM_REQUIRE(q.ok, PM_EUNSUPPORTED, "conv_bn_bwd_winograd: the data and the weight gradient of this convolution do not both take the Winograd route (pm_conv_bn_bwd_winograd_bytes answers 0)");
+  PM_REQUIRE(vdy && z && pm_aligned16(vdy) && pm_aligned16(z) && vdy_bytes >= q.d.v_bytes && z_bytes >= q.w.m_bytes, PM_EWORKSPACE,
+             "conv_bn_bwd_winograd: vdy %zu < %zu or z %zu < %zu bytes (or null / unaligned)", vdy_bytes, q.d.v_bytes, z_bytes, q.w.m_bytes);
+  return pm_wino_bn_bwd_xf((const float*)dout->ptr, dout->pitch, (const float*)y->ptr, y->pitch, mean, invstd, gamma, beta, sums, count, y->c, q.d.Kp, q.d.g, vdy, z,
+                           (hipStream_t)stream);
 }
 
 extern "C" int pm_conv_bwd_weight(const pm_tensor* x0, const pm_tensor* dy0, float* dw, float* dbias, const pm_conv_params* p0, void* ws,
@@ -1275,6 +1327,9 @@
   const pm_conv_params* p = &tp;
   PM_REQUIRE(dw && pm_aligned16(dw), PM_EINVAL, "conv_bwd_weight: dw null or unaligned");
   const ConvRoute r = route_conv(MODE_WGRAD, x0, dy0, p);
+  PM_REQUIRE(!r.pre || (r.kind == R_WINO_WGRAD && !dbias), PM_EUNSUPPORTED,
+             "conv_bwd_weight: a Winograd-transformed dy (PM_TF_WINO_XF) is served by the Winograd route only, without a bias gradient; this call %s",
+             r.kind == R_WINO_WGRAD ? "asks for dbias" : "routes elsewhere");
   PM_REQUIRE(ws && ws_bytes >= r.ws_bytes, PM_EWORKSPACE, "conv_bwd_weight: workspace %zu < %zu", ws_bytes, r.ws_bytes);
   hipStream_t st = (hipStream_t)stream;
   const pm_tensor *x = x0, *dy = dy0;
@@ -1290,7 +1345,7 @@
   int e;
   switch (r.kind) {
     case R_BF16_WGRAD: e = conv_wgrad_bf16(x, dy, dw, p, r.b16w, ws, st); break;
-    case R_WINO_WGRAD: e = wino_wgrad(x, dy, dw, r.wino, r.wino_w, ws, st, (p->wino_v && (size_t)p->wino_v_bytes >= r.wino.v_bytes) ? (float*)p->wino_v : nullptr); break;
+    case R_WINO_WGRAD: e = wino_wgrad(x, dy, dw, r.wino, r.wino_w, ws, st, (p->wino_v && (size_t)p->wino_v_bytes >= r.wino.v_bytes) ? (float*)p->wino_v : nullptr, r.pre); break;
     default: e = conv_wgrad_direct(x, dy, dw, p, r, ws, st);
   }
   if (e || !dbias) return e;
diff --git a/pinthememory_amd/csrc/pm_common.h b/pinthememory_amd/csrc/pm_common.h
--- a/pinthememory_amd/csrc/pm_common.h
+++ b/pinthememory_amd/csrc/pm_common.h
@@ -52,6 +52,8 @@
                      const float* shift, const float* residual, long res_pitch, int relu, hipStream_t st);
 int pm_wino_dy_xf(const float* dy, long pitch, int Cout, const pm_wino_geom& g, float* Z, hipStream_t st);
 int pm_wino_dw_xf(const float* slab, int ks, int Cout, int Cin, int Kp, int m, float* dw, hipStream_t st);
+int pm_wino_bn_bwd_xf(const float* dout, long dpitch, const float* y, long ypitch, const float* mean, const float* invstd, const float* gamma, const float* beta,
+                      const float* sums, float count, int Cout, int Kp, const pm_wino_geom& g, float* V, float* Z, hipStream_t st);
 
 int pm_bf16_cast_rows(const float* x, long pitch, int C, int Cp, long P, void* out, hipStream_t st);
 int pm_bf16_cast_weights(const float* w, int Cout, int T, int Cin, int Cp, bool rotate, void* out, hipStream_t st);
@@ -241,6 +243,11 @@
   return fmaf(v, s, fmaf(-mu, s, be));
 }
 
+__device__ __forceinline__ float pm_bn_bwd_dx(float g, float v, float mu, float is, float ga, float s1, float s2, float inv_n) {
+  return fmaf(-((v - mu) * is), s2 * inv_n, fmaf(-s1, inv_n, g)) * (is * ga);
+}
+__device__ __forceinline__ float pm_bn_relu_gate(float g, float v, float mu, float is, float ga, float be) { return pm_bn_affine(v, mu, is, ga, be) > 0.f ? g : 0.f; }
+
 __device__ __forceinline__ float4 pm_maxpool_gather4(const float* __restrict__ dy, long dp, int Ho, int Wo, const uint8_t* __restrict__ arg, int H, int W, int C, long ip,
                                                      int ch) {
   const int ix = (int)(ip % W), iy = (int)((ip / W) % H), n = (int)(ip / ((long)W * H));
diff --git a/pinthememory_amd/csrc/winograd.hip b/pinthememory_amd/csrc/winograd.hip
--- a/pinthememory_amd/csrc/winograd.hip
+++ b/pinthememory_amd/csrc/winograd.hip
@@ -311,6 +311,83 @@
   }
 }
 
+struct WinoBnBwdArgs {
+  const float *dout, *y;
+  long dp, yp;
+  const float *mean, *invstd, *gamma, *beta, *sums;
+  float host_inv_n;
+  int C, Kp;
+  pm_wino_geom g;
+  float *V, *Z;
+};
+template <int MT, int W>
+__global__ __launch_bounds__(256) void wino_bn_bwd_kernel(const WinoBnBwdArgs a) {
+  constexpr int A = MT + 2;
+  const pm_wino_geom& g = a.g;
+  const unsigned kg = a.Kp / W;
+  const unsigned total = (unsigned)g.tiles * kg;
+  const long vplane = g.tiles * (long)a.Kp, zplane = g.tiles * (long)a.C;
+  const float inv_n = a.host_inv_n > 0.f ? a.host_inv_n : 1.f / a.sums[2 * a.C];
+  for (unsigned i = blockIdx.x * 256u + threadIdx.x; i < total; i += gridDim.x * 256u) {
+    const unsigned tile = i / kg;
+    const int c = (int)(i - tile * kg) * W;
+    const TileId t = decode_tile(tile, g);
+    const bool cok = c < a.C;
+    Vec<W> mu = vzero<W>(), is = mu, ga = mu, be = mu, s1 = mu, s2 = mu;
+    if (cok) mu = vload<W>(a.mean + c), is = vload<W>(a.invstd + c), ga = vload<W>(a.gamma + c), be = vload<W>(a.beta + c), s1 = vload<W>(a.sums + c), s2 = vload<W>(a.sums + a.C + c);
+    Vec<W> tt[A][A], r[A][MT];
+#pragma unroll
+    for (int b = 0; b < A; ++b) {
+      const int xx = t.rx + g.d * (MT * t.tx + b - 1);
+      const bool xok = cok && (unsigned)xx < (unsigned)g.W;
+      Vec<W> col[A], o[A];
+#pragma unroll
+      for (int aa = 0; aa < A; ++aa) {
+        const int yy = t.ry + g.d * (MT * t.ty + aa - 1);
+        col[aa] = vzero<W>();
+        if (xok && (unsigned)yy < (unsigned)g.H) {
+          const long pix = (long)(t.n * g.H + yy) * g.W + xx;
+          const Vec<W> gd = vload<W>(a.dout + pix * a.dp + c), v = vload<W>(a.y + pix * a.yp + c);
+#pragma unroll
+          for (int q = 0; q < W; ++q) {
+            float e = pm_bn_bwd_dx(pm_bn_relu_gate(gd.v[q], v.v[q], mu.v[q], is.v[q], ga.v[q], be.v[q]), v.v[q], mu.v[q], is.v[q], ga.v[q], s1.v[q], s2.v[q], inv_n);
+            asm("" : "+v"(e));
+            col[aa].v[q] = e;
+          }
+        }
+      }
+      mat_apply<MT, W_BT>(col, o);
+#pragma unroll
+      for (int aa = 0; aa < A; ++aa) tt[aa][b] = o[aa];
+      if (b >= 1 && b <= MT) {
+        Vec<W> in[MT], z[A];
+#pragma unroll
+        for (int aa = 0; aa < MT; ++aa) in[aa] = col[aa + 1];
+        mat_apply<MT, W_A>(in, z);
+#pragma unroll
+        for (int aa = 0; aa < A; ++aa) r[aa][b - 1] = z[aa];
+      }
+    }
+    float* vout = a.V + (long)tile * a.Kp + c;
+#pragma unroll
+    for (int aa = 0; aa < A; ++aa) {
+      Vec<W> o[A];
+      mat_apply<MT, W_BT>(tt[aa], o);
+#pragma unroll
+      for (int b = 0; b < A; ++b) vstore<W>(vout + (aa * A + b) * vplane, o[b]);
+    }
+    if (!cok) continue;
+    float* zout = a.Z + (long)tile * a.C + c;
+#pragma unroll
+    for (int aa = 0; aa < A; ++aa) {
+      Vec<W> o[A];
+      mat_apply<MT, W_A>(r[aa], o);
+#pragma unroll
+      for (int b = 0; b < A; ++b) vstore<W>(zout + (aa * A + b) * zplane, o[b]);
+    }
+  }
+}
+
 template <int MT>
 __global__ __launch_bounds__(256) void wino_dw_kernel(const float* __restrict__ slab, int ks, int Cout, int Cin, int Kp, float* __restrict__ dw) {
   constexpr int A = MT + 2, P = A * A;
@@ -565,6 +642,17 @@
   return pm_check_launch("wino_dy");
 }
 
+int pm_wino_bn_bwd_xf(const float* dout, long dpitch, const float* y, long ypitch, const float* mean, const float* invstd, const float* gamma, const float* beta,
+                      const float* sums, float count, int Cout, int Kp, const pm_wino_geom& g, float* V, float* Z, hipStream_t st) {
+  WinoBnBwdArgs a;
+  a.dout = dout, a.y = y, a.dp = dpitch, a.yp = ypitch, a.mean = mean, a.invstd = invstd, a.gamma = gamma, a.beta = beta, a.sums = sums;
+  a.host_inv_n = count > 0.f ? 1.f / count : 0.f;
+  a.C = Cout, a.Kp = Kp, a.g = g, a.V = V, a.Z = Z;
+  if (g.m == 4) hipLaunchKernelGGL((wino_bn_bwd_kernel<4, 2>), dim3(nblocks(g.tiles * (Kp / 2))), dim3(256), 0, st, a);
+  else hipLaunchKernelGGL((wino_bn_bwd_kernel<2, 4>), dim3(nblocks(g.tiles * (Kp / 4))), dim3(256), 0, st, a);
+  return pm_check_launch("wino_bn_bwd");
+}
+
 int pm_wino_dw_xf(const float* slab, int ks, int Cout, int Cin, int Kp, int m, float* dw, hipStream_t st) {
   const unsigned nb = (unsigned)std::min<long>(((long)Cout * Cin + 255) / 256, 1 << 16);
   if (m == 4) hipLaunchKernelGGL(wino_dw_kernel<4>, dim3(nb), dim3(256), 0, st, slab, ks, Cout, Cin, Kp, dw);
diff --git a/pinthememory_amd/hip/kernels.py b/pinthememory_amd/hip/kernels.py
--- a/pinthememory_amd/hip/kernels.py
+++ b/pinthememory_amd/hip/kernels.py
@@ -252,13 +252,18 @@
     return y
 
 
-def conv_bwd_data(dy, w_krsc, x_shape, stride, pad, dil, add=None, dtype=None, add_mask=None):
+def _xf_desc(buf, dy_shape):
+    n, h, w, c = dy_shape
+    return L.PmTensor(buf.data_ptr(), n, h, w, c, c, L.PM_F32, L.PM_TF_WINO_XF)
+
+
+def conv_bwd_data(dy, w_krsc, x_shape, stride, pad, dil, add=None, dtype=None, add_mask=None, dy_xf_shape=None):
     cout, kh, kw, cin = w_krsc.shape
     dx = new(x_shape, dy, dtype=dtype)
-    dyd, dxd = tdesc(dy), tdesc(dx)
+    dyd, dxd = (tdesc(dy) if dy_xf_shape is None else _xf_desc(dy, dy_xf_shape)), tdesc(dx)
     p = L.conv_params(kh, kw, stride, pad, dil, CONV_PREC)
     lib = _lib()
-    nb, nbu = _sizes(('d', dy.shape, dy.stride(), dy.dtype, dyd.flags, w_krsc.shape, dx.shape, dx.stride(), dx.dtype, stride, pad, dil, CONV_PREC, _GEN[0]),
+    nb, nbu = _sizes(('d', dy.shape, dy.stride(), dy.dtype, dyd.flags, dy_xf_shape, w_krsc.shape, dx.shape, dx.stride(), dx.dtype, stride, pad, dil, CONV_PREC, _GEN[0]),
                      lambda: (lib.pm_conv_workspace(byref(dxd), byref(dyd), byref(p), 1), lib.pm_conv_wxf_bytes_dgrad(byref(dyd), byref(dxd), byref(p))))
     ws = workspace(nb, dy.device) if nb else None
     ad = tdesc(add) if add is not None else None
@@ -275,21 +280,40 @@
     return dx
 
 
-def conv_bwd_weight(x, dy, w_shape_krsc, stride, pad, dil, want_bias=False, wino_v=None, on_stream=None):
+def conv_bwd_weight(x, dy, w_shape_krsc, stride, pad, dil, want_bias=False, wino_v=None, on_stream=None, dy_xf_shape=None):
     cout, kh, kw, cin = w_shape_krsc
     dw = torch.empty(w_shape_krsc, dtype=torch.float32, device=x.device)
     db = torch.empty(cout, dtype=torch.float32, device=x.device) if want_bias else None
-    xd, dyd = tdesc(x), tdesc(dy)
+    xd, dyd = tdesc(x), (tdesc(dy) if dy_xf_shape is None else _xf_desc(dy, dy_xf_shape))
     p = L.conv_params(kh, kw, stride, pad, dil, CONV_PREC)
     if wino_v is not None:
         p.wino_v, p.wino_v_bytes = wino_v.data_ptr(), wino_v.numel() * 4
     lib = _lib()
-    nb = _sizes(('w', x.shape, x.stride(), x.dtype, dy.shape, dy.stride(), dy.dtype, w_shape_krsc, stride, pad, dil, CONV_PREC, wino_v is not None, _GEN[0]),
+    nb = _sizes(('w', x.shape, x.stride(), x.dtype, dy.shape, dy.stride(), dy.dtype, w_shape_krsc, stride, pad, dil, CONV_PREC, wino_v is not None, dy_xf_shape, _GEN[0]),
                 lambda: lib.pm_conv_workspace(byref(xd), byref(dyd), byref(p), 2))
     raw = stream() if on_stream is None else on_stream.cuda_stream
     ws = workspace(nb, x.device, on_stream)
     check(lib.pm_conv_bwd_weight(byref(xd), byref(dyd), dw.data_ptr(), ptr(db), byref(p), ptr(ws), nb, raw), 'pm_conv_bwd_weight')
     return dw, db
+
+
+def conv_bn_bwd_winograd_bytes(x, y, w_shape_krsc, stride, pad, dil):
+    cout, kh, kw, cin = w_shape_krsc
+    xd, yd = tdesc(x), tdesc(y)
+    p = L.conv_params(kh, kw, stride, pad, dil, CONV_PREC)
+    lib = _lib()
+    return _sizes(('bnw', x.shape, x.stride(), x.dtype, y.shape, y.stride(), y.dtype, w_shape_krsc, stride, pad, dil, CONV_PREC, _GEN[0]),
+                  lambda: (lib.pm_conv_bn_bwd_winograd_bytes(byref(xd), byref(yd), byref(p), 0), lib.pm_conv_bn_bwd_winograd_bytes(byref(xd), byref(yd), byref(p), 1)))
+
+
+def conv_bn_bwd_winograd(dout, y, x, w_shape_krsc, stride, pad, dil, mean, invstd, gamma, beta, sums, count, nbytes):
+    cout, kh, kw, cin = w_shape_krsc
+    vdy = torch.empty(nbytes[0] // 4, dtype=torch.float32, device=y.device)
+    z = torch.empty(nbytes[1] // 4, dtype=torch.float32, device=y.device)
+    p = L.conv_params(kh, kw, stride, pad, dil, CONV_PREC)
+    check(_lib().pm_conv_bn_bwd_winograd(byref(tdesc(dout)), byref(tdesc(y)), byref(tdesc(x)), byref(p), mean.data_ptr(), invstd.data_ptr(), gamma.data_ptr(),
+                                         beta.data_ptr(), sums.data_ptr(), count, vdy.data_ptr(), nbytes[0], z.data_ptr(), nbytes[1], stream()), 'pm_conv_bn_bwd_winograd')
+    return vdy, z
 
 
 def bn_stats(x):
diff --git a/pinthememory_amd/hip/lib.py b/pinthememory_amd/hip/lib.py
--- a/pinthememory_amd/hip/lib.py
+++ b/pinthememory_amd/hip/lib.py
@@ -14,6 +14,7 @@
 
 PM_F32, PM_BF16 = 0, 1
 PM_TF_ZERO_PAD64 = 1
+PM_TF_WINO_XF = 2
 
 
 class PmSgdEntry(ctypes.Structure):
@@ -157,6 +158,8 @@
     'pm_sgd_momentum_multi': (_i, [_vp, _i, _f, _f, _f, _vp]),
     'pm_sgd_momentum_multi_dev': (_i, [_vp, _i, _f, _vp, _f, _f, _vp]),
     'pm_cast': (_i, [_T, _T, _vp]),
+    'pm_conv_bn_bwd_winograd_bytes': (_sz, [_T, _T, _P, _i]),
+    'pm_conv_bn_bwd_winograd': (_i, [_T, _T, _T, _P, _vp, _vp, _vp, _vp, _vp, _f, _vp, _sz, _vp, _sz, _vp]),
 }
 
 _lib = None
diff --git a/pinthememory_amd/hip/ops.py b/pinthememory_amd/hip/ops.py
--- a/pinthememory_amd/hip/ops.py
+++ b/pinthememory_amd/hip/ops.py
@@ -130,14 +130,14 @@
     return (p, True) if p is not None else (weight, False)
 
 
-def _wgrad(x, dy, wshape, geom, want_bias=False, deferred=False, wino_v=None):
+def _wgrad(x, dy, wshape, geom, want_bias=False, deferred=False, wino_v=None, dy_xf_shape=None):
     if not deferred:
-        return K.conv_bwd_weight(x, dy, wshape, *geom, want_bias=want_bias, wino_v=wino_v)
+        return K.conv_bwd_weight(x, dy, wshape, *geom, want_bias=want_bias, wino_v=wino_v, dy_xf_shape=dy_xf_shape)
     side, main = _side_stream(), L.stream_obj()
     ev = torch.cuda.Event()
     ev.record(main)
     side.wait_event(ev)
-    out = K.conv_bwd_weight(x, dy, wshape, *geom, want_bias=want_bias, wino_v=wino_v, on_stream=side)
+    out = K.conv_bwd_weight(x, dy, wshape, *geom, want_bias=want_bias, wino_v=wino_v, on_stream=side, dy_xf_shape=dy_xf_shape)
     if wino_v is not None:
         wino_v.record_stream(side)
     x.record_stream(side)
@@ -231,6 +231,40 @@
     else:
         dy, dres = K.bn_bwd_apply(dv, o, y, mean, invstd, gamma, sums, count, mode, want_dres, beta)
     return dy, dres, local[c:2 * c], local[:c]
+
+
+def _wino_bn_bwd_bytes(dv, y, x, wk, geom, mode, group, wino_v, want_bias):
+    if mode != 2 or group is not None or wino_v is None or want_bias or K.CONV_PREC != 0:
+        return None
+    if dv.dtype != torch.float32 or y.dtype != torch.float32 or x.dtype != torch.float32:
+        return None
+    nb = K.conv_bn_bwd_winograd_bytes(x, y, tuple(wk.shape), *geom)
+    return nb if nb[0] and nb[1] else None
+
+
+def _bn_conv_bwd(dv, o, y, mean, invstd, gamma, beta, relu, group, want_dres, has_res, x, wk, geom, deferred, wino_v, need_dx=True, need_dw=True, want_bias=False,
+                 dgrad_first=False):
+    mode = 0 if not relu else (1 if has_res else 2)
+    nb = _wino_bn_bwd_bytes(dv, y, x, wk, geom, mode, group, wino_v, want_bias) if (need_dx and need_dw) else None
+    wshape, dx, dwk, db = tuple(wk.shape), None, None, None
+    if nb is None:
+        dy, dres, dgamma, dbeta = _bn_train_bwd(dv, o, y, mean, invstd, gamma, beta, relu, group, want_dres, has_res)
+        if need_dx and dgrad_first:
+            dx = K.conv_bwd_data(dy, wk, tuple(x.shape), *geom, dtype=x.dtype)
+        if need_dw:
+            dwk, db = _wgrad(x, dy, wshape, geom, want_bias=want_bias, deferred=deferred, wino_v=wino_v)
+        if need_dx and not dgrad_first:
+            dx = K.conv_bwd_data(dy, wk, tuple(x.shape), *geom, dtype=x.dtype)
+        return dx, dwk, db, dres, dgamma, dbeta
+    c = y.shape[3]
+    sums, _ = K.bn_bwd_reduce(dv, o, y, mean, invstd, 2, gamma, beta, want_gmask=False, with_count=False)
+    vdy, z = K.conv_bn_bwd_winograd(dv, y, x, wshape, *geom, mean, invstd, gamma, beta, sums, float(y.shape[0] * y.shape[1] * y.shape[2]), nb)
+    if dgrad_first:
+        dx = K.conv_bwd_data(vdy, wk, tuple(x.shape), *geom, dtype=x.dtype, dy_xf_shape=tuple(y.shape))
+    dwk, _ = _wgrad(x, z, wshape, geom, deferred=deferred, wino_v=wino_v, dy_xf_shape=tuple(y.shape))
+    if not dgrad_first:
+        dx = K.conv_bwd_data(vdy, wk, tuple(x.shape), *geom, dtype=x.dtype, dy_xf_shape=tuple(y.shape))
+    return dx, dwk, None, None, sums[c:2 * c], sums[:c]
 
 
 def _bn_bwd_masked(dv, mask, y, mean, invstd, gamma, group):
@@ -312,9 +346,7 @@
             dy3, dres, dg3, db3 = _bn_train_bwd(dv, out, y3, m3, i3, g3, b3, True, gr[2], True, True, mask=mask3)
         dw3, _ = _wgrad(o2, dy3, tuple(k3.shape), ge[2], deferred=df[2])
         do2 = K.conv_bwd_data(dy3, k3, tuple(o2.shape), *ge[2])
-        dy2, _, dg2, db2 = _bn_train_bwd(do2, o2, y2, m2, i2, g2, b2, True, gr[1], False, False)
-        dw2, _ = _wgrad(o1, dy2, tuple(k2.shape), ge[1], deferred=df[1], wino_v=v2)
-        do1 = K.conv_bwd_data(dy2, k2, tuple(o1.shape), *ge[1])
+        do1, dw2, _, _, dg2, db2 = _bn_conv_bwd(do2, o2, y2, m2, i2, g2, b2, True, gr[1], False, False, o1, k2, ge[1], df[1], v2)
         dy1, _, dg1, db1 = _bn_train_bwd(do1, o1, y1, m1, i1, g1, b1, True, gr[0], False, False)
         dw1, _ = _wgrad(xv, dy1, tuple(k1.shape), ge[0], deferred=df[0])
         dwd = dgd = dbd = None
@@ -419,8 +451,12 @@
         stride, pad, dil = ctx.geom
         dv = _grad_view(dout)
         want_dres = ctx.has_res and ctx.needs_input_grad[5]
+        need_dw = ctx.needs_input_grad[1] or (ctx.has_bias and ctx.needs_input_grad[2])
         if ctx.train:
-            dy, dres, dgamma, dbeta = _bn_train_bwd(dv, o, y, mean, invstd, gamma, beta, ctx.relu, ctx.group, want_dres, ctx.has_res)
+            dxv, dwk, db, dres, dgamma, dbeta = _bn_conv_bwd(dv, o, y, mean, invstd, gamma, beta, ctx.relu, ctx.group, want_dres, ctx.has_res, xv, wk, ctx.geom, ctx.deferred,
+                                                             vk, need_dx=ctx.needs_input_grad[0], need_dw=need_dw, want_bias=ctx.has_bias, dgrad_first=True)
+            return (nchw(dxv) if dxv is not None else None, dwk.permute(0, 3, 1, 2) if dwk is not None else None, db, dgamma, dbeta,
+                    (nchw(dres) if dres is not None else None), None, None, None, None, None)
         else:
             c = y.shape[3]
             mode = 0 if not ctx.relu else (1 if ctx.has_res else 2)
@@ -430,7 +466,7 @@
             dres, dgamma, dbeta = (g if want_dres else None), sums[c:], sums[:c]
         dx = nchw(K.conv_bwd_data(dy, wk, tuple(xv.shape), stride, pad, dil, dtype=xv.dtype)) if ctx.needs_input_grad[0] else None
         dw = db = None
-        if ctx.needs_input_grad[1] or (ctx.has_bias and ctx.needs_input_grad[2]):
+        if need_dw:
             dwk, db = _wgrad(xv, dy, tuple(wk.shape), (stride, pad, dil), want_bias=ctx.has_bias, deferred=ctx.deferred, wino_v=vk)
             dw = dwk.permute(0, 3, 1, 2)
         return dx, dw, db, dgamma, dbeta, (nchw(dres) if dres is not None else None), None, None, None, None, None
```

Result: no change. 154.3, median of 6 (+0.4%).
